# rmontanana/semcode

Hardware: AMD Instinct MI355X
Metric: chunks/sec embed (256-tok) + top-k QPS over 10M x 768 (higher is better)
Workload: dtype bf16; 1 GPU; encoder forward, 256 chunks x 256 tokens per GPU per step, BERT-base shape (12x768, 12 heads, FFN 3072), bf16 MFMA / f32 accumulate, random-init weights; global_batch=256, seq_len=256, parallelism=dp1 (replicated weights, no collective), device=AMD Radeon Graphics (gfx950:sramecc+:xnack-)

## Files before the change

include/semcode_hip.h:

```cpp
#ifndef SEMCODE_HIP_H
#define SEMCODE_HIP_H

#include <stddef.h>
#include <stdint.h>

#ifdef __cplusplus
extern "C" {
#endif

typedef int32_t sc_status;

enum {
    SC_OK = 0,
    SC_ERR_INVALID = -1,
    SC_ERR_HIP = -2,
    SC_ERR_STATE = -3,
    SC_ERR_UNSUPPORTED = -4,
    SC_ERR_NOMEM = -5
};

typedef enum { SC_METRIC_IP = 0, SC_METRIC_L2 = 1, SC_METRIC_COSINE = 2 } sc_metric;
typedef enum { SC_INDEX_FLAT = 0, SC_INDEX_IVF_FLAT = 1 } sc_index_kind;

typedef struct sc_runtime sc_runtime;
typedef struct sc_index sc_index;
typedef struct sc_encoder sc_encoder;


typedef struct sc_runtime_cfg {
    int32_t device;
    void* stream;
    int32_t flags;
} sc_runtime_cfg;

const char* sc_version(void);
sc_status sc_last_error(char* buf, size_t n);

sc_status sc_runtime_create(const sc_runtime_cfg* cfg, sc_runtime** out);
sc_status sc_runtime_destroy(sc_runtime* rt);
sc_status sc_runtime_set_stream(sc_runtime* rt, void* stream);
sc_status sc_runtime_synchronize(sc_runtime* rt);
sc_status sc_runtime_device_info(sc_runtime* rt, char* name, size_t n, int32_t* cus, int64_t* hbm_bytes);
sc_status sc_runtime_set_profiling(sc_runtime* rt, int32_t enabled);
sc_status sc_runtime_profile_read(sc_runtime* rt, int32_t which, double* total_ms, int64_t* launches);
sc_status sc_runtime_profile_reset(sc_runtime* rt);

sc_status sc_synth_fill_dev(sc_runtime* rt, float* out, int64_t rows, int32_t dim, int32_t ld,
                            uint64_t seed, int64_t first_row);


typedef struct sc_encoder_cfg {
    int32_t vocab, hidden, layers, heads, ffn, max_pos, type_vocab;
    float ln_eps;
    int32_t normalize;
    uint64_t synth_seed;
    int32_t pos_type;
    int32_t ffn_type;
    float rope_theta;
    int32_t arch;
    int32_t local_window;
    int32_t global_every;
    float rope_theta_local;
    int32_t kv_heads;
    int32_t head_dim;
    int32_t qk_norm;
    int32_t rel_buckets;
    int32_t rel_max_distance;
} sc_encoder_cfg;

sc_status sc_encoder_blob_bytes(const sc_encoder_cfg* cfg, int64_t* out);
sc_status sc_encoder_create(sc_runtime* rt, const sc_encoder_cfg* cfg, const void* weights_blob, size_t nbytes, sc_encoder** out);
sc_status sc_encoder_destroy(sc_encoder* enc);
sc_status sc_encoder_info(sc_encoder* enc, sc_encoder_cfg* cfg_out);
sc_status sc_encoder_set_path(sc_encoder* enc, int32_t path);
sc_status sc_encoder_set_pooling(sc_encoder* enc, int32_t pooling);
sc_status sc_encoder_get_pooling(sc_encoder* enc, int32_t* out);
sc_status sc_encoder_set_output_proj(sc_encoder* enc, const float* W, const float* b, int32_t E);
sc_status sc_encoder_out_dim(sc_encoder* enc, int32_t* out);
sc_status sc_encoder_embed_ids(sc_encoder* enc, const int32_t* ids, const int32_t* lens, int32_t B, int32_t S, float* out);
sc_status sc_encoder_embed_ids_dev(sc_encoder* enc, const int32_t* ids_dev, const int32_t* lens_dev, int32_t B, int32_t S,
                                   float* out_dev);

sc_status sc_encoder_embed_ids_into(sc_encoder* enc, const int32_t* ids, const int32_t* lens, int32_t B, int32_t S, sc_index* ix,
                                    const int64_t* rows, float* out);

sc_status sc_encoder_embed_ids_into_async(sc_encoder* enc, const int32_t* ids, const int32_t* lens, int32_t B, int32_t S, sc_index* ix,
                                          const int64_t* rows);
sc_status sc_encoder_wait(sc_encoder* enc);

#define SC_ENCODER_PACKED_MAX_ROWS 524288
sc_status sc_encoder_packed_rows(sc_encoder* enc, const int64_t* offsets, int32_t B, int64_t* rows);
sc_status sc_encoder_embed_packed(sc_encoder* enc, const int32_t* ids, const int64_t* offsets, int32_t B, float* out);
sc_status sc_encoder_embed_packed_into(sc_encoder* enc, const int32_t* ids, const int64_t* offsets, int32_t B, sc_index* ix, const int64_t* rows,
                                       float* out);
sc_status sc_encoder_embed_packed_into_async(sc_encoder* enc, const int32_t* ids, const int64_t* offsets, int32_t B, sc_index* ix,
                                             const int64_t* rows);

sc_status sc_encoder_set_pair_head(sc_encoder* enc, const float* pooler_w , const float* pooler_b ,
                                   const float* cls_w , const float* cls_b , int32_t num_labels);
sc_status sc_encoder_score_pairs(sc_encoder* enc, const int32_t* ids, const int64_t* offsets, const int32_t* first_lens, int32_t B,
                                 float* out_logits, float* out_cls);

typedef struct sc_score_head {
    int32_t kind;
    int32_t pooling;
    int32_t num_labels;
    float   norm_eps;
    const float *dense_w , *dense_b , *norm_g , *norm_b ;
    const float *cls_w , *cls_b ;
} sc_score_head;
sc_status sc_encoder_set_score_head(sc_encoder* enc, const sc_score_head* head );
sc_status sc_encoder_score_seqs(sc_encoder* enc, const int32_t* ids, const int64_t* offsets, int32_t B, float* out_logits ,
                                float* out_rows );

sc_status sc_encoder_set_token_head(sc_encoder* enc, const float* w , int32_t W);
sc_status sc_encoder_embed_tokens(sc_encoder* enc, const int32_t* ids, const int64_t* offsets, int32_t B, int32_t expand_id, float* out ,
                                  int32_t* out_counts );
sc_status sc_encoder_score_late(sc_encoder* enc, const int32_t* q_ids, const int64_t* q_offsets, int32_t Bq, int32_t expand_id, const int32_t* d_ids,
                                const int64_t* d_offsets, int32_t Bd, const uint8_t* d_keep , const int32_t* pair_q, const int32_t* pair_d, int32_t P,
                                float* out_scores );
sc_status sc_diag_maxsim(sc_runtime* rt, const float* Q, const int32_t* q_off, int32_t Bq, const float* D, const int32_t* d_off, int32_t Bd, const uint8_t* keep,
                         const int32_t* pair_q, const int32_t* pair_d, int32_t P, int32_t W, float* out);
sc_status sc_diag_maxsim_host(const float* Q, const int32_t* q_off, int32_t Bq, const float* D, const int32_t* d_off, int32_t Bd, const uint8_t* keep,
                              const int32_t* pair_q, const int32_t* pair_d, int32_t P, int32_t W, float* out);

typedef struct sc_tokenizer sc_tokenizer;
sc_status sc_tokenizer_create(const char* vocab_utf8, size_t nbytes, int32_t lowercase, sc_tokenizer** out);
sc_status sc_tokenizer_destroy(sc_tokenizer* tok);
sc_status sc_tokenizer_info(sc_tokenizer* tok, int32_t* vocab_size, int32_t* pad, int32_t* unk, int32_t* cls, int32_t* sep);
sc_status sc_tokenizer_encode(sc_tokenizer* tok, const char* bytes, const int64_t* offsets, int32_t n, int32_t max_tokens, int32_t S,
                              int32_t* ids, int32_t* lens, uint8_t* needs_fallback, int32_t threads);

sc_status sc_diag_gemm_bf16(sc_runtime* rt, int32_t epi, const float* A, const float* W, const float* bias, const float* R,
                            int32_t M, int32_t N, int32_t K, float* out);
sc_status sc_diag_gemm_bench(sc_runtime* rt, int32_t epi, int32_t M, int32_t N, int32_t K, int32_t iters, int32_t variant,
                             double* ms_per_launch);
sc_status sc_diag_gemm_trace(sc_runtime* rt, int32_t epi, int32_t M, int32_t N, int32_t K, uint64_t* out, int64_t cap_words);
sc_status sc_diag_gemm_i8(sc_runtime* rt, const int8_t* A, const int8_t* W, int32_t M, int32_t N, int32_t K, int32_t* out);
sc_status sc_diag_encoder_read(sc_encoder* enc, int32_t which, void* out, size_t nbytes);
sc_status sc_diag_set_option(const char* name, int32_t value);
sc_status sc_diag_rope(sc_runtime* rt, float* qk, int32_t rows, int32_t S, int32_t heads, float theta);
sc_status sc_diag_rel_buckets(int32_t rel_buckets, int32_t max_distance, int32_t span, int32_t* out);
sc_status sc_diag_attention_bias(sc_runtime* rt, const float* qkv, const int32_t* lens, int32_t B, int32_t S, int32_t heads, int32_t blocked_rows,
                                 const float* rel_bias, int32_t buckets, int32_t max_distance, float* out);
sc_status sc_diag_attention_bias_packed(sc_runtime* rt, const float* qkv, const int32_t* starts, const int32_t* lens, int32_t B, int32_t heads,
                                        int32_t blocked_rows, const float* rel_bias, int32_t buckets, int32_t max_distance, float* out);
sc_status sc_diag_ffn_act(sc_runtime* rt, int32_t kind, const float* h, int32_t rows, int32_t F, float* out);
sc_status sc_diag_output_proj(sc_runtime* rt, const float* x, int32_t B, int32_t H, const float* W, const float* bias, int32_t E, int32_t normalize,
                              float* out);
sc_status sc_diag_swiglu(sc_runtime* rt, const float* h, int32_t rows, int32_t F, float* out);
sc_status sc_diag_attention(sc_runtime* rt, const float* qkv, const int32_t* lens, int32_t B, int32_t S, int32_t heads, float* out);

sc_status sc_diag_fold_ln(sc_runtime* rt, const float* W, const float* gamma, const float* beta, const float* bias, int32_t N, int32_t K,
                          float* Wf, float* c1, float* c2);
sc_status sc_diag_gemm_lna(sc_runtime* rt, int32_t epi, int32_t flags, const float* A, const float* Wf, const float* c1, const float* c2,
                           const float* stats_in, float eps, int32_t M, int32_t N, int32_t K, int32_t rope_S, float rope_theta,
                           int32_t rope_ncols, float* C, float* fin);
int32_t sc_diag_gemm_strip(int32_t M, int32_t N, int32_t K, int32_t cus);
sc_status sc_diag_gemm_resln(sc_runtime* rt, int32_t flags, const float* A, const float* W, const float* bias, const float* gam, const float* R,
                             const float* fin, float eps, int32_t M, int32_t N, int32_t K, float* C, float* stats_out);
sc_status sc_diag_attention_ex(sc_runtime* rt, const float* qkv, const int32_t* lens, int32_t B, int32_t S, int32_t heads, int32_t blocked_rows,
                               const float* slopes, float* out);
sc_status sc_diag_attention_packed(sc_runtime* rt, const float* qkv, const int32_t* starts, const int32_t* lens, int32_t B, int32_t heads,
                                   int32_t blocked_rows, const float* slopes, float* out);
sc_status sc_diag_attention_hd(sc_runtime* rt, const float* qkv, const int32_t* lens, int32_t B, int32_t S, int32_t heads, int32_t head_dim,
                               int32_t blocked_rows, const float* slopes, float* out);
sc_status sc_diag_attention_packed_hd(sc_runtime* rt, const float* qkv, const int32_t* starts, const int32_t* lens, int32_t B, int32_t heads,
                                      int32_t head_dim, int32_t blocked_rows, const float* slopes, float* out);
sc_status sc_diag_attention_cls(sc_runtime* rt, const float* qkv, const int32_t* lens, int32_t B, int32_t S, int32_t heads, int32_t head_dim,
                                const float* alibi, float* out);
sc_status sc_diag_attention_window(sc_runtime* rt, const float* qkv, const int32_t* starts, const int32_t* lens, int32_t B, int32_t S, int32_t heads,
                                   int32_t local_window, int32_t blocked_rows, float* out);
sc_status sc_diag_attention_causal(sc_runtime* rt, const float* qkv, const int32_t* starts, const int32_t* lens, int32_t B, int32_t S, int32_t heads,
                                   int32_t kv_heads, int32_t blocked_rows, float* out);
sc_status sc_diag_attention_causal_hd(sc_runtime* rt, const float* qkv, const int32_t* starts, const int32_t* lens, int32_t B, int32_t S, int32_t heads,
                                      int32_t kv_heads, int32_t head_dim, int32_t blocked_rows, float* out);
sc_status sc_diag_qknorm_rope(sc_runtime* rt, float* x, int32_t rows, int32_t S, const int32_t* pos, int32_t heads, int32_t kv_heads, int32_t head_dim,
                              float theta, const float* gamma_q, const float* gamma_k, float eps);
sc_status sc_diag_layernorm(sc_runtime* rt, const float* x, int32_t tokens, int32_t H, const float* gamma, const float* beta, float eps, float* out);
sc_status sc_diag_rmsnorm(sc_runtime* rt, const float* x, int32_t tokens, int32_t H, const float* gamma, float eps, float* out);
sc_status sc_diag_mean_pool(sc_runtime* rt, const float* x, const int32_t* lens, int32_t B, int32_t S, int32_t H, int32_t normalize, float* out);
sc_status sc_diag_mean_pool_ln(sc_runtime* rt, const float* y, const float* stats, int32_t slots, int32_t tokens_pad, const float* gamma,
                               const float* beta, float eps, const int32_t* lens, int32_t B, int32_t S, int32_t H, float* out);
sc_status sc_diag_geglu(sc_runtime* rt, const float* h, int32_t rows, int32_t F, float* out);
sc_status sc_diag_embed(sc_runtime* rt, int32_t ln, const int32_t* ids, int32_t tokens, int32_t S, int32_t H, int32_t vocab, int32_t max_pos,
                        const float* wemb, const float* pemb, const float* temb, const float* gamma, const float* beta, float eps,
                        int32_t tokens_pad, int32_t slots, float* rows, float* stats);
sc_status sc_diag_embed_pairs(sc_runtime* rt, int32_t ln, const int32_t* ids, const int32_t* pos, const int32_t* types, int32_t tokens, int32_t H,
                              int32_t vocab, int32_t max_pos, int32_t type_vocab, const float* wemb, const float* pemb, const float* temb,
                              const float* gamma, const float* beta, float eps, int32_t tokens_pad, int32_t slots, float* rows, float* stats);
sc_status sc_diag_pair_head(sc_runtime* rt, const float* cls, int32_t B, int32_t H, const float* pooler_w, const float* pooler_b,
                            const float* cls_w, const float* cls_b, int32_t num_labels, float* out_logits);
sc_status sc_diag_score_head(sc_runtime* rt, const float* rows, int32_t B, int32_t H, const sc_score_head* head, float* out_logits);


sc_status sc_index_create(sc_runtime* rt, int32_t dim, sc_metric metric, sc_index_kind kind,
                          int32_t nlist, int64_t row_base, sc_index** out);
sc_status sc_index_destroy(sc_index* ix);
sc_status sc_index_info(sc_index* ix, int64_t* rows, int32_t* dim, int32_t* ld);
sc_status sc_index_reserve(sc_index* ix, int64_t rows);
sc_status sc_index_add(sc_index* ix, const float* vecs, int64_t n);
sc_status sc_index_overwrite(sc_index* ix, const float* vecs, const int64_t* rows, int64_t n);
sc_status sc_index_put_rows(sc_index* ix, const float* vecs, const int64_t* rows, int64_t n);
sc_status sc_index_put_rows_dev(sc_index* ix, const float* vecs_dev, const int64_t* rows, int64_t n);
sc_status sc_index_delete_rows(sc_index* ix, const int64_t* rows, int64_t n);
sc_status sc_index_last_delete_stats(sc_index* ix, int64_t* rows_moved, int64_t* bytes_moved, int32_t* shadows_kept, int32_t* shadows_dropped);
sc_status sc_index_get_rows(sc_index* ix, int64_t first, int64_t n, float* out);
sc_status sc_index_fill_synthetic(sc_index* ix, int64_t n, uint64_t seed, int64_t first_row);

sc_status sc_index_fill_synthetic_clustered(sc_index* ix, int64_t n, uint64_t seed, int64_t first_row, int32_t nclusters, float spread);
sc_status sc_index_release_scratch(sc_index* ix);

sc_status sc_index_search(sc_index* ix, const float* q, int32_t Q, int32_t k, int32_t nprobe,
                          float* out_dist, int64_t* out_rows);
sc_status sc_index_search_dev(sc_index* ix, const float* q_dev, int32_t Q, int32_t k, int32_t nprobe,
                              float* out_dist_dev, int64_t* out_rows_dev);

sc_status sc_index_search_masked(sc_index* ix, const float* q, int32_t Q, int32_t k, const uint32_t* allow, int64_t allow_words,
                                 float* out_dist, int64_t* out_rows);
sc_status sc_index_search_masked_dev(sc_index* ix, const float* q_dev, int32_t Q, int32_t k, const uint32_t* allow_dev,
                                     int64_t allow_words, float* out_dist_dev, int64_t* out_rows_dev);
sc_status sc_index_last_mask_stats(sc_index* ix, int64_t* allowed_rows, int64_t* scanned_rows, int32_t* gathered);

sc_status sc_index_set_groups(sc_index* ix, const int32_t* labels, int64_t n);
sc_status sc_index_search_grouped(sc_index* ix, const float* q, int32_t Q, int32_t k, const uint32_t* allow, int64_t allow_words,
                                  float* out_dist, int64_t* out_rows);
sc_status sc_index_search_grouped_dev(sc_index* ix, const float* q_dev, int32_t Q, int32_t k, const uint32_t* allow_dev,
                                      int64_t allow_words, float* out_dist_dev, int64_t* out_rows_dev);
sc_status sc_index_last_group_stats(sc_index* ix, int32_t* first_width, int32_t* queries_continued, int32_t* rounds, int64_t* rows_scanned);

sc_status sc_index_search_mmr(sc_index* ix, const float* q, int32_t Q, int32_t k, int32_t fetch_k, float lambda, const uint32_t* allow,
                              int64_t allow_words, float* out_dist, int64_t* out_rows);
sc_status sc_index_search_mmr_dev(sc_index* ix, const float* q_dev, int32_t Q, int32_t k, int32_t fetch_k, float lambda,
                                  const uint32_t* allow_dev, int64_t allow_words, float* out_dist_dev, int64_t* out_rows_dev);
sc_status sc_index_last_mmr_stats(sc_index* ix, int32_t* fetch_k, int32_t* min_candidates, int64_t* rows_scanned);
sc_status sc_diag_mmr_select_host(const float* rel, const float* G, int32_t C, int32_t ldg, int32_t k, float lambda, int32_t* picked);

sc_status sc_lex_terms(const uint8_t* bytes, const int64_t* offsets, int64_t n, int32_t T, uint16_t* out_terms, int32_t* out_counts);
sc_status sc_index_set_terms(sc_index* ix, int64_t first_row, int64_t n, int32_t T, const uint16_t* terms);
sc_status sc_index_drop_terms(sc_index* ix);
sc_status sc_index_lex_stats(sc_index* ix, int64_t* rows, int64_t* sum_dl, uint32_t* df);
sc_status sc_index_search_lexical(sc_index* ix, int32_t Q, int32_t k, const uint16_t* qterms, const float* qweights, const int32_t* nterms, float k1, float b,
                                  float avgdl, const uint32_t* allow, int64_t allow_words, float* out_score, int64_t* out_rows);
sc_status sc_index_search_lexical_dev(sc_index* ix, int32_t Q, int32_t k, const uint16_t* qterms_dev, const float* qweights_dev, const int32_t* nterms_dev,
                                      float k1, float b, float avgdl, const uint32_t* allow_dev, int64_t allow_words, float* out_score_dev,
                                      int64_t* out_rows_dev);
sc_status sc_index_search_hybrid(sc_index* ix, const float* q, int32_t Q, int32_t k, int32_t fetch_k, const uint16_t* qterms, const float* qweights,
                                 const int32_t* nterms, float k1, float b, float avgdl, int32_t c, float wd, float wl, const uint32_t* allow,
                                 int64_t allow_words, float* out_score, int64_t* out_rows);
sc_status sc_index_search_hybrid_dev(sc_index* ix, const float* q_dev, int32_t Q, int32_t k, int32_t fetch_k, const uint16_t* qterms_dev,
                                     const float* qweights_dev, const int32_t* nterms_dev, float k1, float b, float avgdl, int32_t c, float wd, float wl,
                                     const uint32_t* allow_dev, int64_t allow_words, float* out_score_dev, int64_t* out_rows_dev);
sc_status sc_index_last_lex_stats(sc_index* ix, int64_t* rows_scanned, int64_t* bytes_per_pass, int32_t* passes);
sc_status sc_diag_lex_score_host(const uint16_t* terms, int64_t n, int32_t T, const uint16_t* qterms, const float* qweights, int32_t m, float k1, float b,
                                 float avgdl, float* out_score, uint8_t* out_hit);
sc_status sc_diag_rrf_host(const int64_t* dense_rows, const int64_t* lex_rows, int32_t F, int32_t k, int32_t c, float wd, float wl, float* out_score,
                           int64_t* out_rows);

sc_status sc_index_train(sc_index* ix, int32_t niter, uint64_t seed);
sc_status sc_index_ivf_assignments(sc_index* ix, int32_t* out);
sc_status sc_index_set_ivf(sc_index* ix, const float* centroids, const int32_t* assign, int32_t nlist);
sc_status sc_index_assign_lists(sc_index* ix, const float* centroids, int32_t nlist);
sc_status sc_index_ivf_info(sc_index* ix, int32_t* nlist, float* centroids, int64_t* list_sizes);

sc_status sc_index_set_search_mode(sc_index* ix, int32_t mode);
sc_status sc_index_last_search_stats(sc_index* ix, int32_t* path, int32_t* uncertified);

sc_status sc_index_set_coarse_stage(sc_index* ix, int32_t bits);
sc_status sc_index_last_coarse_stats(sc_index* ix, int32_t* first_stage_bits, int32_t* handed_to_bf16);
sc_status sc_index_last_collect_stats(sc_index* ix, int32_t* tried, int32_t* resolved);
sc_status sc_index_last_wide(sc_index* ix, int32_t* wide);
sc_status sc_index_last_tail_rows(sc_index* ix, int64_t* rows);

sc_status sc_index_last_probe_stats(sc_index* ix, int64_t* unique_rows, int64_t* streamed_rows, int32_t* groups);
sc_status sc_diag_ivf_plan(const char* path, const int64_t* probes, int32_t Q, int32_t nprobe, const int64_t* list_off, int32_t nlist,
                           int32_t k, int32_t ld, int32_t cus, int32_t wide, void* out, int64_t cap_bytes, int64_t* need_bytes);
sc_status sc_diag_ivf_exact_path(int32_t ld, int32_t R, int32_t k, int32_t nprobe, int32_t cus, int32_t* path);
sc_status sc_diag_encoder_plan(const int32_t* ids, const int64_t* offsets, int32_t B, int32_t kind, const int32_t* first_lens, int32_t expand_id,
                               int32_t query, int32_t max_pos, int32_t pos_type, int32_t vocab, int32_t type_vocab, int32_t arch, int32_t global_every,
                               int32_t local_window, void* out, int64_t cap_bytes, int64_t* need_bytes);

sc_status sc_topk_merge_host(sc_metric metric, int32_t lists, int32_t Q, int32_t k,
                             const float* dist, const int64_t* rows, float* out_dist, int64_t* out_rows);


typedef struct sc_comm sc_comm;
#define SC_COMM_ID_BYTES 128
sc_status sc_comm_unique_id(void* id_out, size_t nbytes);
sc_status sc_comm_create(sc_runtime* rt, int32_t rank, int32_t world, const void* unique_id, size_t nbytes, sc_comm** out);
sc_status sc_comm_destroy(sc_comm* comm);
sc_status sc_comm_info(sc_comm* comm, int32_t* rank, int32_t* world);
sc_status sc_comm_rccl_version(int32_t* version);
sc_status sc_comm_allgather_topk(sc_comm* comm, const float* dist_dev, const int64_t* rows_dev, int32_t Q, int32_t k,
                                 float* all_dist_dev, int64_t* all_rows_dev);
sc_status sc_comm_broadcast(sc_comm* comm, void* buf_dev, size_t nbytes, int32_t root);
sc_status sc_index_search_sharded(sc_index* ix, sc_comm* comm, const float* q, int32_t Q, int32_t k, int32_t nprobe,
                                  float* out_dist, int64_t* out_rows);
sc_status sc_index_search_sharded_dev(sc_index* ix, sc_comm* comm, const float* q_dev, int32_t Q, int32_t k, int32_t nprobe,
                                      float* all_dist_dev, int64_t* all_rows_dev);
sc_status sc_index_train_sharded(sc_index* ix, sc_comm* comm, int32_t niter, int32_t root);
sc_status sc_comm_allreduce_max(sc_comm* comm, double* value);

#ifdef __cplusplus
}
#endif
#endif
```

semcode_amd/_native.py:

```python
from __future__ import annotations

import ctypes as C
import sys
import threading
from pathlib import Path

import numpy as np

LIB_PATH = Path(__file__).resolve().parent / "_lib" / "libsemcode_hip.so"

METRICS = {"IP": 0, "L2": 1, "COSINE": 2}
KINDS = {"FLAT": 0, "IVF_FLAT": 1}


class ScError(RuntimeError):

    def __init__(self, status: int, message: str):
        super().__init__(f"libsemcode_hip error {status}: {message}")
        self.status = status


class _Cfg(C.Structure):
    _fields_ = [("device", C.c_int32), ("stream", C.c_void_p), ("flags", C.c_int32)]


class EncoderCfg(C.Structure):
    _fields_ = [("vocab", C.c_int32), ("hidden", C.c_int32), ("layers", C.c_int32), ("heads", C.c_int32), ("ffn", C.c_int32),
                ("max_pos", C.c_int32), ("type_vocab", C.c_int32), ("ln_eps", C.c_float), ("normalize", C.c_int32),
                ("synth_seed", C.c_uint64), ("pos_type", C.c_int32), ("ffn_type", C.c_int32), ("rope_theta", C.c_float),
                ("arch", C.c_int32), ("local_window", C.c_int32), ("global_every", C.c_int32), ("rope_theta_local", C.c_float),
                ("kv_heads", C.c_int32)]

    def __new__(cls, *args, **kw):
        real = EncoderCfgFull if cls is EncoderCfg else cls
        return real.from_buffer(bytearray(real.CFG_BYTES))


class EncoderCfgFull(EncoderCfg):
    _fields_ = [("head_dim", C.c_int32), ("qk_norm", C.c_int32)]
    TAIL_FIELDS = ("rel_buckets", "rel_max_distance")
    CFG_BYTES = 88 + 4 * len(TAIL_FIELDS)

    def _tail(self, name):
        return C.c_int32.from_address(C.addressof(self) + 88 + 4 * self.TAIL_FIELDS.index(name))

    rel_buckets = property(lambda self: self._tail("rel_buckets").value, lambda self, v: setattr(self._tail("rel_buckets"), "value", int(v)))
    rel_max_distance = property(lambda self: self._tail("rel_max_distance").value, lambda self, v: setattr(self._tail("rel_max_distance"), "value", int(v)))


class ScoreHead(C.Structure):
    _fields_ = [("kind", C.c_int32), ("pooling", C.c_int32), ("num_labels", C.c_int32), ("norm_eps", C.c_float),
                ("dense_w", C.c_void_p), ("dense_b", C.c_void_p), ("norm_g", C.c_void_p), ("norm_b", C.c_void_p), ("cls_w", C.c_void_p), ("cls_b", C.c_void_p)]


_lib = None
_lib_lock = threading.Lock()

_f32p = C.POINTER(C.c_float)
_i64p = C.POINTER(C.c_int64)

SIGNATURES = {
    "sc_version": (C.c_char_p, []),
    "sc_last_error": (C.c_int32, [C.c_char_p, C.c_size_t]),
    "sc_runtime_create": (C.c_int32, [C.POINTER(_Cfg), C.POINTER(C.c_void_p)]),
    "sc_runtime_destroy": (C.c_int32, [C.c_void_p]),
    "sc_runtime_set_stream": (C.c_int32, [C.c_void_p, C.c_void_p]),
    "sc_runtime_synchronize": (C.c_int32, [C.c_void_p]),
    "sc_runtime_device_info": (C.c_int32, [C.c_void_p, C.c_char_p, C.c_size_t, C.POINTER(C.c_int32), C.POINTER(C.c_int64)]),
    "sc_runtime_set_profiling": (C.c_int32, [C.c_void_p, C.c_int32]),
    "sc_runtime_profile_read": (C.c_int32, [C.c_void_p, C.c_int32, C.POINTER(C.c_double), C.POINTER(C.c_int64)]),
    "sc_runtime_profile_reset": (C.c_int32, [C.c_void_p]),
    "sc_synth_fill_dev": (C.c_int32, [C.c_void_p, C.c_void_p, C.c_int64, C.c_int32, C.c_int32, C.c_uint64, C.c_int64]),
    "sc_encoder_blob_bytes": (C.c_int32, [C.POINTER(EncoderCfg), C.POINTER(C.c_int64)]),
    "sc_encoder_create": (C.c_int32, [C.c_void_p, C.POINTER(EncoderCfg), C.c_void_p, C.c_size_t, C.POINTER(C.c_void_p)]),
    "sc_encoder_destroy": (C.c_int32, [C.c_void_p]),
    "sc_encoder_set_path": (C.c_int32, [C.c_void_p, C.c_int32]),
    "sc_encoder_set_pooling": (C.c_int32, [C.c_void_p, C.c_int32]),
    "sc_encoder_get_pooling": (C.c_int32, [C.c_void_p, C.POINTER(C.c_int32)]),
    "sc_encoder_info": (C.c_int32, [C.c_void_p, C.POINTER(EncoderCfg)]),
    "sc_encoder_embed_ids": (C.c_int32, [C.c_void_p, C.c_void_p, C.c_void_p, C.c_int32, C.c_int32, C.c_void_p]),
    "sc_encoder_embed_ids_dev": (C.c_int32, [C.c_void_p, C.c_void_p, C.c_void_p, C.c_int32, C.c_int32, C.c_void_p]),
    "sc_encoder_embed_ids_into": (C.c_int32, [C.c_void_p, C.c_void_p, C.c_void_p, C.c_int32, C.c_int32, C.c_void_p, C.c_void_p, C.c_void_p]),
    "sc_encoder_embed_ids_into_async": (C.c_int32, [C.c_void_p, C.c_void_p, C.c_void_p, C.c_int32, C.c_int32, C.c_void_p, C.c_void_p]),
    "sc_encoder_wait": (C.c_int32, [C.c_void_p]),
    "sc_encoder_packed_rows": (C.c_int32, [C.c_void_p, C.c_void_p, C.c_int32, C.POINTER(C.c_int64)]),
    "sc_encoder_embed_packed": (C.c_int32, [C.c_void_p, C.c_void_p, C.c_void_p, C.c_int32, C.c_void_p]),
    "sc_encoder_set_output_proj": (C.c_int32, [C.c_void_p, C.c_void_p, C.c_void_p, C.c_int32]),
    "sc_encoder_out_dim": (C.c_int32, [C.c_void_p, C.POINTER(C.c_int32)]),
    "sc_diag_output_proj": (C.c_int32, [C.c_void_p, C.c_void_p, C.c_int32, C.c_int32, C.c_void_p, C.c_void_p, C.c_int32, C.c_int32, C.c_void_p]),
    "sc_encoder_set_pair_head": (C.c_int32, [C.c_void_p] * 5 + [C.c_int32]),
    "sc_encoder_score_pairs": (C.c_int32, [C.c_void_p] * 4 + [C.c_int32, C.c_void_p, C.c_void_p]),
    "sc_encoder_set_score_head": (C.c_int32, [C.c_void_p, C.POINTER(ScoreHead)]),
    "sc_encoder_score_seqs": (C.c_int32, [C.c_void_p, C.c_void_p, C.c_void_p, C.c_int32, C.c_void_p, C.c_void_p]),
    "sc_encoder_set_token_head": (C.c_int32, [C.c_void_p, C.c_void_p, C.c_int32]),
    "sc_encoder_embed_tokens": (C.c_int32, [C.c_void_p, C.c_void_p, C.c_void_p, C.c_int32, C.c_int32, C.c_void_p, C.c_void_p]),
    "sc_encoder_score_late": (C.c_int32, [C.c_void_p, C.c_void_p, C.c_void_p, C.c_int32, C.c_int32, C.c_void_p, C.c_void_p, C.c_int32] + [C.c_void_p] * 3
                              + [C.c_int32, C.c_void_p]),
    "sc_diag_maxsim": (C.c_int32, [C.c_void_p, C.c_void_p, C.c_void_p, C.c_int32, C.c_void_p, C.c_void_p, C.c_int32] + [C.c_void_p] * 3
                       + [C.c_int32, C.c_int32, C.c_void_p]),
    "sc_diag_maxsim_host": (C.c_int32, [C.c_void_p, C.c_void_p, C.c_int32, C.c_void_p, C.c_void_p, C.c_int32] + [C.c_void_p] * 3 + [C.c_int32, C.c_int32, C.c_void_p]),
    "sc_diag_score_head": (C.c_int32, [C.c_void_p, C.c_void_p, C.c_int32, C.c_int32, C.POINTER(ScoreHead), C.c_void_p]),
    "sc_diag_embed_pairs": (C.c_int32, [C.c_void_p, C.c_int32] + [C.c_void_p] * 3 + [C.c_int32] * 5 + [C.c_void_p] * 5 + [C.c_float, C.c_int32, C.c_int32,
                                                                                                                       C.c_void_p, C.c_void_p]),
    "sc_diag_pair_head": (C.c_int32, [C.c_void_p, C.c_void_p, C.c_int32, C.c_int32] + [C.c_void_p] * 4 + [C.c_int32, C.c_void_p]),
    "sc_encoder_embed_packed_into": (C.c_int32, [C.c_void_p, C.c_void_p, C.c_void_p, C.c_int32, C.c_void_p, C.c_void_p, C.c_void_p]),
    "sc_encoder_embed_packed_into_async": (C.c_int32, [C.c_void_p, C.c_void_p, C.c_void_p, C.c_int32, C.c_void_p, C.c_void_p]),
    "sc_tokenizer_create": (C.c_int32, [C.c_char_p, C.c_size_t, C.c_int32, C.POINTER(C.c_void_p)]),
    "sc_tokenizer_destroy": (C.c_int32, [C.c_void_p]),
    "sc_tokenizer_info": (C.c_int32, [C.c_void_p] + [C.POINTER(C.c_int32)] * 5),
    "sc_tokenizer_encode": (C.c_int32, [C.c_void_p, C.c_char_p, C.c_void_p, C.c_int32, C.c_int32, C.c_int32, C.c_void_p, C.c_void_p, C.c_void_p, C.c_int32]),
    "sc_diag_gemm_bf16": (C.c_int32, [C.c_void_p, C.c_int32, C.c_void_p, C.c_void_p, C.c_void_p, C.c_void_p, C.c_int32, C.c_int32, C.c_int32, C.c_void_p]),
    "sc_diag_gemm_bench": (C.c_int32, [C.c_void_p, C.c_int32, C.c_int32, C.c_int32, C.c_int32, C.c_int32, C.c_int32, C.POINTER(C.c_double)]),
    "sc_diag_gemm_trace": (C.c_int32, [C.c_void_p, C.c_int32, C.c_int32, C.c_int32, C.c_int32, C.c_void_p, C.c_int64]),
    "sc_diag_set_option": (C.c_int32, [C.c_char_p, C.c_int32]),
    "sc_diag_gemm_i8": (C.c_int32, [C.c_void_p, C.c_void_p, C.c_void_p, C.c_int32, C.c_int32, C.c_int32, C.c_void_p]),
    "sc_diag_encoder_read": (C.c_int32, [C.c_void_p, C.c_int32, C.c_void_p, C.c_size_t]),
    "sc_diag_attention": (C.c_int32, [C.c_void_p, C.c_void_p, C.c_void_p, C.c_int32, C.c_int32, C.c_int32, C.c_void_p]),
    "sc_diag_rope": (C.c_int32, [C.c_void_p, C.c_void_p, C.c_int32, C.c_int32, C.c_int32, C.c_float]),
    "sc_diag_swiglu": (C.c_int32, [C.c_void_p, C.c_void_p, C.c_int32, C.c_int32, C.c_void_p]),
    "sc_diag_rel_buckets": (C.c_int32, [C.c_int32, C.c_int32, C.c_int32, C.c_void_p]),
    "sc_diag_attention_bias": (C.c_int32, [C.c_void_p, C.c_void_p, C.c_void_p, C.c_int32, C.c_int32, C.c_int32, C.c_int32, C.c_void_p, C.c_int32, C.c_int32, C.c_void_p]),
    "sc_diag_attention_bias_packed": (C.c_int32, [C.c_void_p, C.c_void_p, C.c_void_p, C.c_void_p, C.c_int32, C.c_int32, C.c_int32, C.c_void_p, C.c_int32, C.c_int32,
                                                  C.c_void_p]),
    "sc_diag_ffn_act": (C.c_int32, [C.c_void_p, C.c_int32, C.c_void_p, C.c_int32, C.c_int32, C.c_void_p]),
    "sc_diag_fold_ln": (C.c_int32, [C.c_void_p] * 5 + [C.c_int32, C.c_int32] + [C.c_void_p] * 3),
    "sc_diag_gemm_strip": (C.c_int32, [C.c_int32] * 4),
    "sc_diag_gemm_lna": (C.c_int32, [C.c_void_p, C.c_int32, C.c_int32] + [C.c_void_p] * 5 + [C.c_float, C.c_int32, C.c_int32, C.c_int32, C.c_int32,
                                     C.c_float, C.c_int32, C.c_void_p, C.c_void_p]),
    "sc_diag_gemm_resln": (C.c_int32, [C.c_void_p, C.c_int32] + [C.c_void_p] * 6 + [C.c_float, C.c_int32, C.c_int32, C.c_int32, C.c_void_p, C.c_void_p]),
    "sc_diag_attention_ex": (C.c_int32, [C.c_void_p, C.c_void_p, C.c_void_p, C.c_int32, C.c_int32, C.c_int32, C.c_int32, C.c_void_p, C.c_void_p]),
    "sc_diag_attention_packed": (C.c_int32, [C.c_void_p, C.c_void_p, C.c_void_p, C.c_void_p, C.c_int32, C.c_int32, C.c_int32, C.c_void_p, C.c_void_p]),
    "sc_diag_attention_hd": (C.c_int32, [C.c_void_p, C.c_void_p, C.c_void_p, C.c_int32, C.c_int32, C.c_int32, C.c_int32, C.c_int32, C.c_void_p, C.c_void_p]),
    "sc_diag_attention_cls": (C.c_int32, [C.c_void_p, C.c_void_p, C.c_void_p, C.c_int32, C.c_int32, C.c_int32, C.c_int32, C.c_void_p, C.c_void_p]),
    "sc_diag_attention_window": (C.c_int32, [C.c_void_p, C.c_void_p, C.c_void_p, C.c_void_p, C.c_int32, C.c_int32, C.c_int32, C.c_int32, C.c_int32, C.c_void_p]),
    "sc_diag_attention_packed_hd": (C.c_int32, [C.c_void_p, C.c_void_p, C.c_void_p, C.c_void_p, C.c_int32, C.c_int32, C.c_int32, C.c_int32, C.c_void_p, C.c_void_p]),
    "sc_diag_layernorm": (C.c_int32, [C.c_void_p, C.c_void_p, C.c_int32, C.c_int32, C.c_void_p, C.c_void_p, C.c_float, C.c_void_p]),
    "sc_diag_attention_causal": (C.c_int32, [C.c_void_p, C.c_void_p, C.c_void_p, C.c_void_p, C.c_int32, C.c_int32, C.c_int32, C.c_int32, C.c_int32, C.c_void_p]),
    "sc_diag_attention_causal_hd": (C.c_int32, [C.c_void_p, C.c_void_p, C.c_void_p, C.c_void_p, C.c_int32, C.c_int32, C.c_int32, C.c_int32, C.c_int32, C.c_int32,
                                                 C.c_void_p]),
    "sc_diag_qknorm_rope": (C.c_int32, [C.c_void_p, C.c_void_p, C.c_int32, C.c_int32, C.c_void_p, C.c_int32, C.c_int32, C.c_int32, C.c_float, C.c_void_p, C.c_void_p,
                                         C.c_float]),
    "sc_diag_rmsnorm": (C.c_int32, [C.c_void_p, C.c_void_p, C.c_int32, C.c_int32, C.c_void_p, C.c_float, C.c_void_p]),
    "sc_diag_mean_pool": (C.c_int32, [C.c_void_p, C.c_void_p, C.c_void_p, C.c_int32, C.c_int32, C.c_int32, C.c_int32, C.c_void_p]),
    "sc_diag_mean_pool_ln": (C.c_int32, [C.c_void_p, C.c_void_p, C.c_void_p, C.c_int32, C.c_int32, C.c_void_p, C.c_void_p, C.c_float, C.c_void_p,
                                         C.c_int32, C.c_int32, C.c_int32, C.c_void_p]),
    "sc_diag_geglu": (C.c_int32, [C.c_void_p, C.c_void_p, C.c_int32, C.c_int32, C.c_void_p]),
    "sc_diag_embed": (C.c_int32, [C.c_void_p, C.c_int32, C.c_void_p, C.c_int32, C.c_int32, C.c_int32, C.c_int32, C.c_int32] + [C.c_void_p] * 5 +
                                 [C.c_float, C.c_int32, C.c_int32, C.c_void_p, C.c_void_p]),
    "sc_index_create": (C.c_int32, [C.c_void_p, C.c_int32, C.c_int32, C.c_int32, C.c_int32, C.c_int64, C.POINTER(C.c_void_p)]),
    "sc_index_destroy": (C.c_int32, [C.c_void_p]),
    "sc_index_info": (C.c_int32, [C.c_void_p, C.POINTER(C.c_int64), C.POINTER(C.c_int32), C.POINTER(C.c_int32)]),
    "sc_index_reserve": (C.c_int32, [C.c_void_p, C.c_int64]),
    "sc_index_add": (C.c_int32, [C.c_void_p, C.c_void_p, C.c_int64]),
    "sc_index_overwrite": (C.c_int32, [C.c_void_p, C.c_void_p, C.c_void_p, C.c_int64]),
    "sc_index_put_rows": (C.c_int32, [C.c_void_p, C.c_void_p, C.c_void_p, C.c_int64]),
    "sc_index_put_rows_dev": (C.c_int32, [C.c_void_p, C.c_void_p, C.c_void_p, C.c_int64]),
    "sc_index_delete_rows": (C.c_int32, [C.c_void_p, C.c_void_p, C.c_int64]),
    "sc_index_last_delete_stats": (C.c_int32, [C.c_void_p, C.POINTER(C.c_int64), C.POINTER(C.c_int64), C.POINTER(C.c_int32), C.POINTER(C.c_int32)]),
    "sc_index_get_rows": (C.c_int32, [C.c_void_p, C.c_int64, C.c_int64, C.c_void_p]),
    "sc_index_fill_synthetic": (C.c_int32, [C.c_void_p, C.c_int64, C.c_uint64, C.c_int64]),
    "sc_index_fill_synthetic_clustered": (C.c_int32, [C.c_void_p, C.c_int64, C.c_uint64, C.c_int64, C.c_int32, C.c_float]),
    "sc_index_release_scratch": (C.c_int32, [C.c_void_p]),
    "sc_index_search": (C.c_int32, [C.c_void_p, C.c_void_p, C.c_int32, C.c_int32, C.c_int32, C.c_void_p, C.c_void_p]),
    "sc_index_search_dev": (C.c_int32, [C.c_void_p, C.c_void_p, C.c_int32, C.c_int32, C.c_int32, C.c_void_p, C.c_void_p]),
    "sc_index_search_masked": (C.c_int32, [C.c_void_p, C.c_void_p, C.c_int32, C.c_int32, C.c_void_p, C.c_int64, C.c_void_p, C.c_void_p]),
    "sc_index_search_masked_dev": (C.c_int32, [C.c_void_p, C.c_void_p, C.c_int32, C.c_int32, C.c_void_p, C.c_int64, C.c_void_p, C.c_void_p]),
    "sc_index_last_mask_stats": (C.c_int32, [C.c_void_p, C.POINTER(C.c_int64), C.POINTER(C.c_int64), C.POINTER(C.c_int32)]),
    "sc_index_set_groups": (C.c_int32, [C.c_void_p, C.c_void_p, C.c_int64]),
    "sc_index_search_grouped": (C.c_int32, [C.c_void_p, C.c_void_p, C.c_int32, C.c_int32, C.c_void_p, C.c_int64, C.c_void_p, C.c_void_p]),
    "sc_index_search_grouped_dev": (C.c_int32, [C.c_void_p, C.c_void_p, C.c_int32, C.c_int32, C.c_void_p, C.c_int64, C.c_void_p, C.c_void_p]),
    "sc_index_last_group_stats": (C.c_int32, [C.c_void_p, C.POINTER(C.c_int32), C.POINTER(C.c_int32), C.POINTER(C.c_int32), C.POINTER(C.c_int64)]),
    "sc_index_search_mmr": (C.c_int32, [C.c_void_p, C.c_void_p, C.c_int32, C.c_int32, C.c_int32, C.c_float, C.c_void_p, C.c_int64, C.c_void_p, C.c_void_p]),
    "sc_index_search_mmr_dev": (C.c_int32, [C.c_void_p, C.c_void_p, C.c_int32, C.c_int32, C.c_int32, C.c_float, C.c_void_p, C.c_int64, C.c_void_p, C.c_void_p]),
    "sc_index_last_mmr_stats": (C.c_int32, [C.c_void_p, C.POINTER(C.c_int32), C.POINTER(C.c_int32), C.POINTER(C.c_int64)]),
    "sc_diag_mmr_select_host": (C.c_int32, [C.c_void_p, C.c_void_p, C.c_int32, C.c_int32, C.c_int32, C.c_float, C.c_void_p]),
    "sc_lex_terms": (C.c_int32, [C.c_void_p, C.c_void_p, C.c_int64, C.c_int32, C.c_void_p, C.c_void_p]),
    "sc_index_set_terms": (C.c_int32, [C.c_void_p, C.c_int64, C.c_int64, C.c_int32, C.c_void_p]),
    "sc_index_drop_terms": (C.c_int32, [C.c_void_p]),
    "sc_index_lex_stats": (C.c_int32, [C.c_void_p, C.POINTER(C.c_int64), C.POINTER(C.c_int64), C.c_void_p]),
    "sc_index_search_lexical": (C.c_int32, [C.c_void_p, C.c_int32, C.c_int32, C.c_void_p, C.c_void_p, C.c_void_p, C.c_float, C.c_float, C.c_float, C.c_void_p, C.c_int64,
                                            C.c_void_p, C.c_void_p]),
    "sc_index_search_lexical_dev": (C.c_int32, [C.c_void_p, C.c_int32, C.c_int32, C.c_void_p, C.c_void_p, C.c_void_p, C.c_float, C.c_float, C.c_float, C.c_void_p, C.c_int64,
                                                C.c_void_p, C.c_void_p]),
    "sc_index_search_hybrid": (C.c_int32, [C.c_void_p, C.c_void_p, C.c_int32, C.c_int32, C.c_int32, C.c_void_p, C.c_void_p, C.c_void_p, C.c_float, C.c_float, C.c_float,
                                           C.c_int32, C.c_float, C.c_float, C.c_void_p, C.c_int64, C.c_void_p, C.c_void_p]),
    "sc_index_search_hybrid_dev": (C.c_int32, [C.c_void_p, C.c_void_p, C.c_int32, C.c_int32, C.c_int32, C.c_void_p, C.c_void_p, C.c_void_p, C.c_float, C.c_float, C.c_float,
                                               C.c_int32, C.c_float, C.c_float, C.c_void_p, C.c_int64, C.c_void_p, C.c_void_p]),
    "sc_index_last_lex_stats": (C.c_int32, [C.c_void_p, C.POINTER(C.c_int64), C.POINTER(C.c_int64), C.POINTER(C.c_int32)]),
    "sc_diag_lex_score_host": (C.c_int32, [C.c_void_p, C.c_int64, C.c_int32, C.c_void_p, C.c_void_p, C.c_int32, C.c_float, C.c_float, C.c_float, C.c_void_p, C.c_void_p]),
    "sc_diag_rrf_host": (C.c_int32, [C.c_void_p, C.c_void_p, C.c_int32, C.c_int32, C.c_int32, C.c_float, C.c_float, C.c_void_p, C.c_void_p]),
    "sc_index_train": (C.c_int32, [C.c_void_p, C.c_int32, C.c_uint64]),
    "sc_index_ivf_assignments": (C.c_int32, [C.c_void_p, C.c_void_p]),
    "sc_index_set_ivf": (C.c_int32, [C.c_void_p, C.c_void_p, C.c_void_p, C.c_int32]),
    "sc_index_assign_lists": (C.c_int32, [C.c_void_p, C.c_void_p, C.c_int32]),
    "sc_index_ivf_info": (C.c_int32, [C.c_void_p, C.POINTER(C.c_int32), C.c_void_p, C.c_void_p]),
    "sc_index_set_search_mode": (C.c_int32, [C.c_void_p, C.c_int32]),
    "sc_index_last_search_stats": (C.c_int32, [C.c_void_p, C.POINTER(C.c_int32), C.POINTER(C.c_int32)]),
    "sc_index_set_coarse_stage": (C.c_int32, [C.c_void_p, C.c_int32]),
    "sc_index_last_coarse_stats": (C.c_int32, [C.c_void_p, C.POINTER(C.c_int32), C.POINTER(C.c_int32)]),
    "sc_index_last_collect_stats": (C.c_int32, [C.c_void_p, C.POINTER(C.c_int32), C.POINTER(C.c_int32)]),
    "sc_index_last_wide": (C.c_int32, [C.c_void_p, C.POINTER(C.c_int32)]),
    "sc_index_last_tail_rows": (C.c_int32, [C.c_void_p, C.POINTER(C.c_int64)]),
    "sc_index_last_probe_stats": (C.c_int32, [C.c_void_p, C.POINTER(C.c_int64), C.POINTER(C.c_int64), C.POINTER(C.c_int32)]),
    "sc_diag_ivf_plan": (C.c_int32, [C.c_char_p, C.c_void_p, C.c_int32, C.c_int32, C.c_void_p, C.c_int32, C.c_int32, C.c_int32, C.c_int32, C.c_int32, C.c_void_p,
                                     C.c_int64, C.POINTER(C.c_int64)]),
    "sc_diag_ivf_exact_path": (C.c_int32, [C.c_int32, C.c_int32, C.c_int32, C.c_int32, C.c_int32, C.POINTER(C.c_int32)]),
    "sc_diag_encoder_plan": (C.c_int32, [C.c_void_p, C.c_void_p, C.c_int32, C.c_int32, C.c_void_p, C.c_int32] + [C.c_int32] * 8 + [C.c_void_p, C.c_int64,
                                         C.POINTER(C.c_int64)]),
    "sc_comm_unique_id": (C.c_int32, [C.c_void_p, C.c_size_t]),
    "sc_comm_create": (C.c_int32, [C.c_void_p, C.c_int32, C.c_int32, C.c_void_p, C.c_size_t, C.POINTER(C.c_void_p)]),
    "sc_comm_destroy": (C.c_int32, [C.c_void_p]),
    "sc_comm_info": (C.c_int32, [C.c_void_p, C.POINTER(C.c_int32), C.POINTER(C.c_int32)]),
    "sc_comm_rccl_version": (C.c_int32, [C.POINTER(C.c_int32)]),
    "sc_comm_allgather_topk": (C.c_int32, [C.c_void_p, C.c_void_p, C.c_void_p, C.c_int32, C.c_int32, C.c_void_p, C.c_void_p]),
    "sc_comm_broadcast": (C.c_int32, [C.c_void_p, C.c_void_p, C.c_size_t, C.c_int32]),
    "sc_index_search_sharded": (C.c_int32, [C.c_void_p, C.c_void_p, C.c_void_p, C.c_int32, C.c_int32, C.c_int32, C.c_void_p, C.c_void_p]),
    "sc_index_search_sharded_dev": (C.c_int32, [C.c_void_p, C.c_void_p, C.c_void_p, C.c_int32, C.c_int32, C.c_int32, C.c_void_p, C.c_void_p]),
    "sc_index_train_sharded": (C.c_int32, [C.c_void_p, C.c_void_p, C.c_int32, C.c_int32]),
    "sc_comm_allreduce_max": (C.c_int32, [C.c_void_p, C.POINTER(C.c_double)]),
    "sc_topk_merge_host": (C.c_int32, [C.c_int32, C.c_int32, C.c_int32, C.c_int32, C.c_void_p, C.c_void_p, C.c_void_p, C.c_void_p]),
}


def lib() -> C.CDLL:
    global _lib
    with _lib_lock:
        if _lib is None:
            if not LIB_PATH.exists():
                raise RuntimeError(
                    f"{LIB_PATH} is missing: build it with `python -m semcode_amd.csrc.build` "
                    "(needs hipcc); semcode_amd has no CPU fallback."
                )
            try:
                import torch
            except Exception:
                pass
            handle = C.CDLL(str(LIB_PATH))
            for name, (res, args) in SIGNATURES.items():
                fn = getattr(handle, name)
                fn.restype = res
                fn.argtypes = args
            _lib = handle
    return _lib


def _check(status: int) -> None:
    if status != 0:
        buf = C.create_string_buffer(512)
        lib().sc_last_error(buf, 512)
        raise ScError(status, buf.value.decode("utf-8", "replace"))


def pack_allow(allow, rows: int) -> np.ndarray:
    a = np.asarray(allow)
    if a.dtype == np.bool_:
        if a.shape != (rows,):
            raise ValueError(f"a boolean mask must have one entry per row ({rows}), got shape {a.shape}")
        bits = np.packbits(a, bitorder="little")
        words = np.zeros((rows + 31) // 32 * 4, dtype=np.uint8)
        words[: bits.size] = bits
        return words.view("<u4")
    if a.dtype != np.uint32 or a.ndim != 1:
        raise ValueError("allow must be a 1-d uint32 word array or a boolean array with one entry per row")
    return np.ascontiguousarray(a)


def _result_arrays(Q: int, k: int) -> "tuple[np.ndarray, np.ndarray]":
    return np.empty((Q, k), dtype=np.float32), np.empty((Q, k), dtype=np.int64)


LEX_MAX_QTERMS = 32
LEX_DF_SIZE = 65536
LEX_PAD = 0xFFFF


def lex_terms(texts, T: int = 128) -> "tuple[np.ndarray, np.ndarray]":
    raw = [t.encode("utf-8") if isinstance(t, str) else bytes(t) for t in texts]
    n = len(raw)
    offsets = np.zeros(n + 1, dtype=np.int64)
# ... 824 lines not shown
def diag_gemm_bench(rt: Runtime, M: int, N: int, K: int, epi: int = 0, iters: int = 20, variant: int = 0) -> float:
    ms = C.c_double()
    _check(lib().sc_diag_gemm_bench(rt.handle, epi, M, N, K, iters, variant, C.byref(ms)))
    return ms.value


def diag_gemm_trace(rt: Runtime, M: int, N: int, K: int, epi: int = 0, launches: int = 1) -> np.ndarray:
    nt = (M // 256) * (N // 256)
    out = np.zeros((launches, nt, 8), np.uint64)
    _check(lib().sc_diag_gemm_trace(rt.handle, epi, M, N, K, out.ctypes.data_as(C.c_void_p), out.size))
    return out


def diag_gemm_i8(rt: Runtime, A, W) -> np.ndarray:
    A = np.ascontiguousarray(A, np.int8)
    W = np.ascontiguousarray(W, np.int8)
    M, K = A.shape
    N = W.shape[0]
    out = np.empty((M, N), np.int32)
    _check(lib().sc_diag_gemm_i8(rt.handle, A.ctypes.data_as(C.c_void_p), W.ctypes.data_as(C.c_void_p), M, N, K, out.ctypes.data_as(C.c_void_p)))
    return out


def diag_attention(rt: Runtime, qkv, lens, B: int, S: int, heads: int, head_dim: int = 64, blocked_rows: int = 0) -> np.ndarray:
    if head_dim != 64 or blocked_rows:
        return diag_attention_ex(rt, qkv, lens, B, S, heads, blocked_rows=blocked_rows, head_dim=head_dim)
    qkv = np.ascontiguousarray(qkv, np.float32)
    lens = np.ascontiguousarray(lens, np.int32)
    out = np.empty((B * S, heads * 64), np.float32)
    _check(lib().sc_diag_attention(rt.handle, qkv.ctypes.data_as(C.c_void_p), lens.ctypes.data_as(C.c_void_p), B, S, heads,
                                   out.ctypes.data_as(C.c_void_p)))
    return out


def diag_rope(rt: Runtime, qk, S: int, heads: int, theta: float) -> np.ndarray:
    out = np.array(qk, dtype=np.float32, order="C")
    rows = out.shape[0]
    if out.shape != (rows, heads * 64):
        raise ValueError("qk must be [rows, heads * 64]")
    _check(lib().sc_diag_rope(rt.handle, out.ctypes.data_as(C.c_void_p), rows, int(S), int(heads), float(theta)))
    return out


def diag_rel_buckets(rel_buckets: int, max_distance: int, span: int) -> np.ndarray:
    out = np.empty(max(2 * int(span) - 1, 1), np.int32)
    _check(lib().sc_diag_rel_buckets(int(rel_buckets), int(max_distance), int(span), out.ctypes.data_as(C.c_void_p)))
    return out


def diag_ffn_act(rt: Runtime, kind: int, h) -> np.ndarray:
    h = np.ascontiguousarray(h, np.float32)
    rows, F = h.shape[0], h.shape[1] // (2 if kind == 4 else 1)
    out = np.empty((rows, F), np.float32)
    _check(lib().sc_diag_ffn_act(rt.handle, int(kind), h.ctypes.data_as(C.c_void_p), rows, F, out.ctypes.data_as(C.c_void_p)))
    return out


def diag_attention_bias(rt: Runtime, qkv, lens, B: int, S: int, heads: int, rel_bias, max_distance: int, blocked_rows: int = 0) -> np.ndarray:
    qkv = np.ascontiguousarray(qkv, np.float32)
    lens = np.ascontiguousarray(lens, np.int32)
    rb = np.ascontiguousarray(rel_bias, np.float32)
    H = heads * 64
    if blocked_rows:
        pad = np.zeros((blocked_rows, 3 * H), np.float32)
        pad[: B * S] = qkv
        qkv = block64(pad)
    out = np.empty((B * S, H), np.float32)
    _check(lib().sc_diag_attention_bias(rt.handle, qkv.ctypes.data_as(C.c_void_p), lens.ctypes.data_as(C.c_void_p), B, S, heads, int(blocked_rows),
                                        rb.ctypes.data_as(C.c_void_p), rb.shape[0], int(max_distance), out.ctypes.data_as(C.c_void_p)))
    return out


def diag_attention_bias_packed(rt: Runtime, qkv, starts, lens, heads: int, rel_bias, max_distance: int, blocked_rows: int = 0) -> np.ndarray:
    qkv = np.ascontiguousarray(qkv, np.float32)
    starts = np.ascontiguousarray(starts, np.int32)
    lens = np.ascontiguousarray(lens, np.int32)
    rb = np.ascontiguousarray(rel_bias, np.float32)
    H = heads * 64
    R = int(blocked_rows) if blocked_rows else (int((starts + (lens + 31) // 32 * 32).max()) + 255) // 256 * 256
    if qkv.shape != (R, 3 * H) or starts.shape != lens.shape:
        raise ValueError(f"diag_attention_bias_packed: qkv must be [{R}, {3 * H}], starts and lens [B]")
    if blocked_rows:
        qkv = block64(qkv)
    out = np.empty((R, H), np.float32)
    _check(lib().sc_diag_attention_bias_packed(rt.handle, qkv.ctypes.data_as(C.c_void_p), starts.ctypes.data_as(C.c_void_p), lens.ctypes.data_as(C.c_void_p),
                                               len(lens), heads, int(blocked_rows), rb.ctypes.data_as(C.c_void_p), rb.shape[0], int(max_distance),
                                               out.ctypes.data_as(C.c_void_p)))
    return out


def diag_output_proj(rt: Runtime, x, W, b=None, normalize: bool = True) -> np.ndarray:
    x, W = np.ascontiguousarray(x, np.float32), np.ascontiguousarray(W, np.float32)
    b = None if b is None else np.ascontiguousarray(b, np.float32)
    out = np.empty((x.shape[0], W.shape[0]), np.float32)
    _check(lib().sc_diag_output_proj(rt.handle, x.ctypes.data_as(C.c_void_p), x.shape[0], x.shape[1], W.ctypes.data_as(C.c_void_p),
                                     None if b is None else b.ctypes.data_as(C.c_void_p), W.shape[0], 1 if normalize else 0, out.ctypes.data_as(C.c_void_p)))
    return out


def diag_swiglu(rt: Runtime, h) -> np.ndarray:
    h = np.ascontiguousarray(h, np.float32)
    rows, F = h.shape[0], h.shape[1] // 2
    out = np.empty((rows, F), np.float32)
    _check(lib().sc_diag_swiglu(rt.handle, h.ctypes.data_as(C.c_void_p), rows, F, out.ctypes.data_as(C.c_void_p)))
    return out


EPI_LNA_BIAS, EPI_LNA_GELU, EPI_RESLN_STATS, EPI_LNA_BIAS_ROPE = 3, 4, 5, 6


def _f32(a):
    return np.ascontiguousarray(a, np.float32)


def _ptr(a):
    return None if a is None else a.ctypes.data_as(C.c_void_p)


def block64(a: np.ndarray) -> np.ndarray:
    M, N = a.shape
    return np.ascontiguousarray(a.reshape(M, N // 64, 64).transpose(1, 0, 2))


def unblock64(a: np.ndarray, M: int, N: int) -> np.ndarray:
    return np.ascontiguousarray(np.asarray(a).reshape(N // 64, M, 64).transpose(1, 0, 2).reshape(M, N))


def diag_fold_ln(rt: Runtime, W, gamma, beta, bias=None):
    W, gamma, beta = _f32(W), _f32(gamma), _f32(beta)
    bias = None if bias is None else _f32(bias)
    N, K = W.shape
    Wf, c1, c2 = np.empty((N, K), np.float32), np.empty(N, np.float32), np.empty(N, np.float32)
    _check(lib().sc_diag_fold_ln(rt.handle, _ptr(W), _ptr(gamma), _ptr(beta), _ptr(bias), N, K, _ptr(Wf), _ptr(c1), _ptr(c2)))
    return Wf, c1, c2


def diag_gemm_lna(rt: Runtime, epi: int, A, Wf, c1, c2, stats_in, eps: float, blocked: bool = False, rope_S: int = 0, rope_theta: float = 0.0,
                  rope_ncols: int = 0):
    A, Wf, c1, c2, stats_in = _f32(A), _f32(Wf), _f32(c1), _f32(c2), _f32(stats_in)
    M, K = A.shape
    N = Wf.shape[0]
    if stats_in.shape != (K // 256, M, 2) or Wf.shape != (N, K) or c1.shape != (N,) or c2.shape != (N,):
        raise ValueError("diag_gemm_lna: shapes")
    Cc, fin = np.empty((M, N), np.float32), np.empty((M, 2), np.float32)
    _check(lib().sc_diag_gemm_lna(rt.handle, epi, 1 if blocked else 0, _ptr(A), _ptr(Wf), _ptr(c1), _ptr(c2), _ptr(stats_in), float(eps), M, N, K,
                                  int(rope_S), float(rope_theta), int(rope_ncols), _ptr(Cc), _ptr(fin)))
    return (unblock64(Cc, M, N) if blocked else Cc), fin


def diag_gemm_strip(M: int = 0, N: int = 0, K: int = 0, cus: int = 0) -> int:
    return int(lib().sc_diag_gemm_strip(int(M), int(N), int(K), int(cus)))


def diag_gemm_resln(rt: Runtime, A, W, bias, gam, R, fin, eps: float, a_blocked: bool = False):
    A, W, bias, gam, R, fin = _f32(A), _f32(W), _f32(bias), _f32(gam), _f32(R), _f32(fin)
    M, K = A.shape
    N = W.shape[0]
    if W.shape != (N, K) or R.shape != (M, N) or fin.shape != (M, 2) or bias.shape != (N,) or gam.shape != (N,):
        raise ValueError("diag_gemm_resln: shapes")
    Ad = block64(A) if a_blocked else A
    Cc, st = np.empty((M, N), np.float32), np.empty((N // 256, M, 2), np.float32)
    _check(lib().sc_diag_gemm_resln(rt.handle, 1 if a_blocked else 0, _ptr(Ad), _ptr(W), _ptr(bias), _ptr(gam), _ptr(R), _ptr(fin), float(eps), M, N, K,
                                    _ptr(Cc), _ptr(st)))
    return Cc, st


def diag_attention_ex(rt: Runtime, qkv, lens, B: int, S: int, heads: int, blocked_rows: int = 0, slopes=None, head_dim: int = 64) -> np.ndarray:
    qkv = _f32(qkv)
    lens = np.ascontiguousarray(lens, np.int32)
    H = heads * head_dim
    if blocked_rows:
        pad = np.zeros((blocked_rows, 3 * H), np.float32)
        pad[: B * S] = qkv
        qkv = block64(pad)
    sl = None if slopes is None else _f32(slopes)
    out = np.empty((B * S, H), np.float32)
    if head_dim != 64:
        _check(lib().sc_diag_attention_hd(rt.handle, _ptr(qkv), _ptr(lens), B, S, heads, int(head_dim), int(blocked_rows), _ptr(sl), _ptr(out)))
    else:
        _check(lib().sc_diag_attention_ex(rt.handle, _ptr(qkv), _ptr(lens), B, S, heads, int(blocked_rows), _ptr(sl), _ptr(out)))
    return out


def diag_attention_cls(rt: Runtime, qkv, lens, B: int, S: int, heads: int, head_dim: int = 64, slopes=None) -> np.ndarray:
    qkv = _f32(qkv)
    lens = np.ascontiguousarray(lens, np.int32)
    H = heads * head_dim
    if qkv.shape != (B * S, 3 * H) or lens.shape != (B,):
        raise ValueError("qkv must be [B*S, 3*heads*head_dim] and lens [B]")
    sl = None if slopes is None else _f32(slopes)
    out = np.full((B, H), np.nan, np.float32)
    _check(lib().sc_diag_attention_cls(rt.handle, _ptr(qkv), _ptr(lens), B, S, heads, int(head_dim), _ptr(sl), _ptr(out)))
    return out


def diag_attention_packed(rt: Runtime, qkv, starts, lens, heads: int, blocked_rows: int = 0, slopes=None, head_dim: int = 64) -> np.ndarray:
    qkv = _f32(qkv)
    starts = np.ascontiguousarray(starts, np.int32)
    lens = np.ascontiguousarray(lens, np.int32)
    H = heads * head_dim
    R = int(blocked_rows) if blocked_rows else (int((starts + (lens + 31) // 32 * 32).max()) + 255) // 256 * 256
    if qkv.shape != (R, 3 * H) or starts.shape != lens.shape:
        raise ValueError(f"diag_attention_packed: qkv must be [{R}, {3 * H}], starts and lens [B]")
    if blocked_rows:
        qkv = block64(qkv)
    sl = None if slopes is None else _f32(slopes)
    out = np.empty((R, H), np.float32)
    if head_dim != 64:
        _check(lib().sc_diag_attention_packed_hd(rt.handle, _ptr(qkv), _ptr(starts), _ptr(lens), len(lens), heads, int(head_dim), int(blocked_rows), _ptr(sl),
                                                 _ptr(out)))
    else:
        _check(lib().sc_diag_attention_packed(rt.handle, _ptr(qkv), _ptr(starts), _ptr(lens), len(lens), heads, int(blocked_rows), _ptr(sl), _ptr(out)))
    return out


def diag_attention_window(rt: Runtime, qkv, lens, heads: int, local_window: int, S: int = 0, starts=None, blocked_rows: int = 0) -> np.ndarray:
    qkv = _f32(qkv)
    lens = np.ascontiguousarray(lens, np.int32)
    H = heads * 64
    if starts is None:
        rows = len(lens) * int(S)
        R = int(blocked_rows) if blocked_rows else rows
    else:
        starts = np.ascontiguousarray(starts, np.int32)
        R = rows = int(blocked_rows) if blocked_rows else (int((starts + (lens + 31) // 32 * 32).max()) + 255) // 256 * 256
    if qkv.shape != (R, 3 * H) or (starts is not None and starts.shape != lens.shape):
        raise ValueError(f"diag_attention_window: qkv must be [{R}, {3 * H}], starts (if given) and lens [B]")
    if blocked_rows:
        qkv = block64(qkv)
    out = np.empty((rows, H), np.float32)
    _check(lib().sc_diag_attention_window(rt.handle, _ptr(qkv), None if starts is None else _ptr(starts), _ptr(lens), len(lens), int(S), heads,
                                          int(local_window), int(blocked_rows), _ptr(out)))
    return out


def diag_attention_causal(rt: Runtime, qkv, lens, heads: int, kv_heads: int, S: int = 0, starts=None, blocked_rows: int = 0, head_dim: int = 64) -> np.ndarray:
    qkv = _f32(qkv)
    lens = np.ascontiguousarray(lens, np.int32)
    head_dim = int(head_dim)
    H, QN = heads * head_dim, (heads + 2 * kv_heads) * head_dim
    if starts is None:
        rows = len(lens) * int(S)
        R = int(blocked_rows) if blocked_rows else rows
    else:
        starts = np.ascontiguousarray(starts, np.int32)
        R = rows = int(blocked_rows) if blocked_rows else (int((starts + (lens + 31) // 32 * 32).max()) + 255) // 256 * 256
    if qkv.shape != (R, QN) or (starts is not None and starts.shape != lens.shape):
        raise ValueError(f"diag_attention_causal: qkv must be [{R}, {QN}], starts (if given) and lens [B]")
    if blocked_rows:
        qkv = block64(qkv)
    out = np.empty((rows, H), np.float32)
    if head_dim != 64:
        _check(lib().sc_diag_attention_causal_hd(rt.handle, _ptr(qkv), None if starts is None else _ptr(starts), _ptr(lens), len(lens), int(S), heads,
                                                 int(kv_heads), head_dim, int(blocked_rows), _ptr(out)))
        return out
    _check(lib().sc_diag_attention_causal(rt.handle, _ptr(qkv), None if starts is None else _ptr(starts), _ptr(lens), len(lens), int(S), heads,
                                          int(kv_heads), int(blocked_rows), _ptr(out)))
    return out


def diag_qknorm_rope(rt: Runtime, x, heads: int, kv_heads: int, head_dim: int, S: int, theta: float, pos=None, gamma_q=None, gamma_k=None,
                     eps: float = 1e-6) -> np.ndarray:
    out = np.array(x, dtype=np.float32, order="C")
    rows = out.shape[0]
    if out.shape != (rows, (heads + 2 * kv_heads) * head_dim):
        raise ValueError("x must be [rows, (heads + 2 kv_heads) * head_dim]")
    if pos is not None:
        pos = np.ascontiguousarray(pos, np.int32)
        if pos.shape != (rows,):
            raise ValueError("pos must be [rows]")
    gq = None if gamma_q is None else _f32(gamma_q)
    gk = None if gamma_k is None else _f32(gamma_k)
    _check(lib().sc_diag_qknorm_rope(rt.handle, _ptr(out), rows, int(S), None if pos is None else _ptr(pos), int(heads), int(kv_heads), int(head_dim),
                                     float(theta), None if gq is None else _ptr(gq), None if gk is None else _ptr(gk), float(eps)))
    return out


def diag_rmsnorm(rt: Runtime, x, gamma, eps: float) -> np.ndarray:
    x, gamma = _f32(x), _f32(gamma)
    out = np.empty_like(x)
    _check(lib().sc_diag_rmsnorm(rt.handle, _ptr(x), x.shape[0], x.shape[1], _ptr(gamma), float(eps), _ptr(out)))
    return out


def diag_layernorm(rt: Runtime, x, gamma, beta, eps: float) -> np.ndarray:
    x, gamma, beta = _f32(x), _f32(gamma), _f32(beta)
    out = np.empty_like(x)
    _check(lib().sc_diag_layernorm(rt.handle, _ptr(x), x.shape[0], x.shape[1], _ptr(gamma), _ptr(beta), float(eps), _ptr(out)))
    return out


def diag_mean_pool(rt: Runtime, x, lens, S: int, normalize: bool) -> np.ndarray:
    x = _f32(x)
    lens = np.ascontiguousarray(lens, np.int32)
    B, H = lens.size, x.shape[1]
    out = np.empty((B, H), np.float32)
    _check(lib().sc_diag_mean_pool(rt.handle, _ptr(x), _ptr(lens), B, int(S), H, 1 if normalize else 0, _ptr(out)))
    return out


def diag_mean_pool_ln(rt: Runtime, y, stats, gamma, beta, eps: float, lens, S: int) -> np.ndarray:
    y, stats, gamma, beta = _f32(y), _f32(stats), _f32(gamma), _f32(beta)
    lens = np.ascontiguousarray(lens, np.int32)
    B, (tp, H) = lens.size, y.shape
    if stats.shape[1:] != (tp, 2):
        raise ValueError("diag_mean_pool_ln: stats must be [slots, tokens_pad, 2]")
# ... 104 lines not shown
```

semcode_amd/csrc/sc_api.cpp:

```cpp
#include <algorithm>
#include <cmath>
#include <cstdarg>
#include <cstdio>
#include <cstring>
#include <mutex>
#include <new>
#include <string>
#include <vector>

#include "encoder_ops.h"
#include "sc_internal.h"

static thread_local std::string g_err;

sc_status sc_fail(sc_status code, const char* fmt, ...) {
    char buf[512];
    va_list ap;
    va_start(ap, fmt);
    vsnprintf(buf, sizeof buf, fmt, ap);
    va_end(ap);
    g_err = buf;
    return code;
}

extern "C" const char* sc_version(void) { return "semcode_hip 0.1 (gfx950)"; }

extern "C" sc_status sc_last_error(char* buf, size_t n) {
    if (!buf || n == 0) return SC_ERR_INVALID;
    snprintf(buf, n, "%s", g_err.c_str());
    return SC_OK;
}


extern "C" sc_status sc_runtime_create(const sc_runtime_cfg* cfg, sc_runtime** out) {
    if (!out) return sc_fail(SC_ERR_INVALID, "sc_runtime_create: out is NULL");
    *out = nullptr;
    int ndev = 0;
    hipError_t e = hipGetDeviceCount(&ndev);
    if (e != hipSuccess || ndev <= 0)
        return sc_fail(SC_ERR_HIP, "sc_runtime_create: no HIP device available (%s)", e == hipSuccess ? "count = 0" : hipGetErrorString(e));
    const int dev = cfg ? cfg->device : 0;
    if (dev < 0 || dev >= ndev) return sc_fail(SC_ERR_INVALID, "sc_runtime_create: device %d out of range [0,%d)", dev, ndev);
    SC_HIP(hipSetDevice(dev));
    sc_runtime* rt = new (std::nothrow) sc_runtime();
    if (!rt) return sc_fail(SC_ERR_NOMEM, "sc_runtime_create: out of host memory");
    rt->device = dev;
    if (cfg && cfg->stream) {
        rt->stream = (hipStream_t)cfg->stream;
        rt->own_stream = false;
    } else {
        e = hipStreamCreateWithFlags(&rt->stream, hipStreamNonBlocking);
        if (e != hipSuccess) {
            delete rt;
            return sc_fail(SC_ERR_HIP, "hipStreamCreate: %s", hipGetErrorString(e));
        }
        rt->own_stream = true;
    }
    hipDeviceProp_t prop;
    if (hipGetDeviceProperties(&prop, dev) == hipSuccess) {
        snprintf(rt->name, sizeof rt->name, "%s (%s)", prop.name, prop.gcnArchName);
        rt->cus = prop.multiProcessorCount;
        rt->hbm = (int64_t)prop.totalGlobalMem;
    }
    *out = rt;
    return SC_OK;
}

static void prof_clear(sc_runtime* rt) {
    for (int c = 0; c < SC_PROF_CLASSES; ++c) {
        for (auto& p : rt->prof[c]) {
            hipEventDestroy(p.first);
            hipEventDestroy(p.second);
        }
        rt->prof[c].clear();
    }
}

void sc_runtime_retain(sc_runtime* rt) { rt->refs.fetch_add(1, std::memory_order_relaxed); }

void sc_runtime_release(sc_runtime* rt) {
    if (rt->refs.fetch_sub(1, std::memory_order_acq_rel) != 1) return;
    hipSetDevice(rt->device);
    hipStreamSynchronize(rt->stream);
    prof_clear(rt);
    if (rt->own_stream) hipStreamDestroy(rt->stream);
    delete rt;
}

extern "C" sc_status sc_runtime_destroy(sc_runtime* rt) {
    if (!rt) return SC_OK;
    sc_runtime_release(rt);
    return SC_OK;
}

extern "C" sc_status sc_runtime_set_stream(sc_runtime* rt, void* stream) {
    if (!rt) return sc_fail(SC_ERR_INVALID, "runtime is NULL");
    std::lock_guard<std::mutex> g(rt->mu);
    if (rt->own_stream) {
        hipStreamSynchronize(rt->stream);
        hipStreamDestroy(rt->stream);
        rt->own_stream = false;
    }
    rt->stream = (hipStream_t)stream;
    return SC_OK;
}

extern "C" sc_status sc_runtime_synchronize(sc_runtime* rt) {
    if (!rt) return sc_fail(SC_ERR_INVALID, "runtime is NULL");
    SC_HIP(hipSetDevice(rt->device));
    SC_HIP(hipStreamSynchronize(rt->stream));
    return SC_OK;
}

extern "C" sc_status sc_runtime_device_info(sc_runtime* rt, char* name, size_t n, int32_t* cus, int64_t* hbm_bytes) {
    if (!rt) return sc_fail(SC_ERR_INVALID, "runtime is NULL");
    if (name && n) snprintf(name, n, "%s", rt->name);
    if (cus) *cus = rt->cus;
    if (hbm_bytes) *hbm_bytes = rt->hbm;
    return SC_OK;
}

extern "C" sc_status sc_runtime_set_profiling(sc_runtime* rt, int32_t enabled) {
    if (!rt) return sc_fail(SC_ERR_INVALID, "runtime is NULL");
    rt->profiling = enabled < 0 ? 0 : enabled;
    return SC_OK;
}

void sc_prof_begin(sc_runtime* rt, int which, hipEvent_t* a, hipEvent_t* b) {
    *a = *b = nullptr;
    if (!rt->profiling || rt->prof[which].size() >= 8192) return;
    if (which >= SC_PROF_GEMM && rt->profiling > 1 && (rt->prof_seen[which]++ % (unsigned)rt->profiling) != 0) return;
    if (hipEventCreate(a) != hipSuccess) { *a = nullptr; return; }
    if (hipEventCreate(b) != hipSuccess) { hipEventDestroy(*a); *a = *b = nullptr; return; }
    hipEventRecord(*a, rt->stream);
}
void sc_prof_end(sc_runtime* rt, int which, hipEvent_t a, hipEvent_t b) {
    if (!a) return;
    hipEventRecord(b, rt->stream);
    std::lock_guard<std::mutex> g(rt->mu);
    rt->prof[which].push_back({a, b});
}

extern "C" sc_status sc_runtime_profile_read(sc_runtime* rt, int32_t which, double* total_ms, int64_t* launches) {
    if (!rt || which < 0 || which >= SC_PROF_CLASSES) return sc_fail(SC_ERR_INVALID, "bad profile class");
    SC_HIP(hipSetDevice(rt->device));
    SC_HIP(hipStreamSynchronize(rt->stream));
    double t = 0;
    std::lock_guard<std::mutex> g(rt->mu);
    for (auto& p : rt->prof[which]) {
        float ms = 0;
        if (hipEventElapsedTime(&ms, p.first, p.second) == hipSuccess) t += ms;
    }
    if (total_ms) *total_ms = t;
    if (launches) *launches = (int64_t)rt->prof[which].size();
    return SC_OK;
}

extern "C" sc_status sc_runtime_profile_reset(sc_runtime* rt) {
    if (!rt) return sc_fail(SC_ERR_INVALID, "runtime is NULL");
    SC_HIP(hipSetDevice(rt->device));
    SC_HIP(hipStreamSynchronize(rt->stream));
    std::lock_guard<std::mutex> g(rt->mu);
    prof_clear(rt);
    for (unsigned& c : rt->prof_seen) c = 0;
    return SC_OK;
}

extern "C" sc_status sc_synth_fill_dev(sc_runtime* rt, float* out, int64_t rows, int32_t dim, int32_t ld, uint64_t seed,
                                       int64_t first_row) {
    if (!rt || !out) return sc_fail(SC_ERR_INVALID, "sc_synth_fill_dev: NULL argument");
    if (rows < 0 || dim <= 0 || ld < dim || (ld & 3)) return sc_fail(SC_ERR_INVALID, "sc_synth_fill_dev: need rows>=0, 0<dim<=ld, ld%%4==0");
    SC_HIP(hipSetDevice(rt->device));
    sc_launch_synth_fill(out, rows, dim, ld, seed, first_row, nullptr, rt->stream);
    SC_HIP(hipGetLastError());
    return SC_OK;
}

extern "C" sc_status sc_diag_set_option(const char* name, int32_t value) {
    if (!name) return sc_fail(SC_ERR_INVALID, "sc_diag_set_option: NULL name");
    static const struct { const char* name; void (*set)(int); } options[] = {
        {"coarse_workgroups", sc_scan_set_coarse_workgroups}, {"coarse_persistent", sc_scan_set_coarse_persistent},
        {"gemm_pp", sc_gemm_set_pp},                          {"gemm_nt", sc_gemm_set_nt},
        {"ivf_refresh_nomem", sc_ivf_set_refresh_nomem},      {"ivf_refine_cap", sc_ivf_set_refine_cap},
        {"ivf_coarse_nomem", sc_ivf_set_coarse_nomem},        {"collect_pass", sc_set_collect_pass},
        {"tighten", sc_set_tighten},                          {"wide_candidates", sc_set_wide_force},
        {"ivf_tail_rows", sc_set_ivf_tail_rows},              {"delete_chunk_rows", sc_set_delete_chunk_rows},
        {"rope_fused", sc_encoder_set_rope_fused},            {"mask_gather", sc_set_mask_gather},
        {"group_width0", sc_set_group_width0},                {"group_width1", sc_set_group_width1},
        {"mmr_chunk_q", sc_set_mmr_chunk_q},                  {"lex_chunk_q", sc_set_lex_chunk_q},
        {"gemm_strip", sc_gemm_set_strip},                    {"gemm_strip_n", sc_gemm_set_strip_n},
        {"cls_prune", sc_encoder_set_cls_prune},
    };
    for (const auto& o : options)
        if (!strcmp(name, o.name)) {
            o.set(value);
            return SC_OK;
        }
    return sc_fail(SC_ERR_INVALID, "sc_diag_set_option: unknown option '%s'", name);
}


static inline int round_up(int v, int a) { return (v + a - 1) / a * a; }

extern "C" sc_status sc_index_create(sc_runtime* rt, int32_t dim, sc_metric metric, sc_index_kind kind, int32_t nlist,
                                     int64_t row_base, sc_index** out) {
    if (!rt || !out) return sc_fail(SC_ERR_INVALID, "sc_index_create: NULL argument");
    *out = nullptr;
    if (dim <= 0 || dim > 65536) return sc_fail(SC_ERR_INVALID, "sc_index_create: dim %d out of range", dim);
    if (metric != SC_METRIC_IP && metric != SC_METRIC_L2 && metric != SC_METRIC_COSINE)
        return sc_fail(SC_ERR_INVALID, "sc_index_create: unknown metric %d", (int)metric);
    if (kind != SC_INDEX_FLAT && kind != SC_INDEX_IVF_FLAT) return sc_fail(SC_ERR_INVALID, "sc_index_create: unknown kind %d", (int)kind);
    if (kind == SC_INDEX_IVF_FLAT && nlist < 1) return sc_fail(SC_ERR_INVALID, "sc_index_create: IVF_FLAT needs nlist >= 1");
    sc_index* ix = new (std::nothrow) sc_index();
    if (!ix) return sc_fail(SC_ERR_NOMEM, "out of host memory");
    ix->rt = rt;
    sc_runtime_retain(rt);
    ix->dim = dim;
    ix->ld = round_up(dim, SC_LD_ALIGN);
    ix->metric = metric;
    ix->kind = kind;
    ix->nlist = nlist;
    ix->row_base = row_base;
    const size_t ld8 = (size_t)sc_ld8(ix);
    ix->sh_b16.row_bytes[0] = (size_t)ix->ld * 2;
    ix->sh_b16.stat_bit = 1;
    ix->sh_i8.row_bytes[0] = ix->sh_c8.row_bytes[0] = ld8;
    ix->sh_i8.row_bytes[1] = 4;
    ix->sh_i8.stat_bit = 2;
    ix->sh_c8.row_bytes[1] = 16;
    ix->sh_c8.tail_pad = 256;
    ix->sh_c8.stat_bit = 4;
    *out = ix;
    return SC_OK;
}

extern "C" sc_status sc_index_destroy(sc_index* ix) {
    if (!ix) return SC_OK;
    hipSetDevice(ix->rt->device);
    hipStreamSynchronize(ix->rt->stream);
    hipFree(ix->X);
    hipFree(ix->xnorm);
    hipFree(ix->perm);
    hipFree(ix->list_off);
    for (const sc_index_buf& b : SC_INDEX_BUFS) sc_buf_free(ix->*b.buf);
    for (sc_shadow* sh : ix->shadows) sc_shadow_release(*sh);
    if (ix->quant) sc_index_destroy(ix->quant);
    sc_runtime* rt = ix->rt;
    delete ix;
    sc_runtime_release(rt);
    return SC_OK;
}

extern "C" sc_status sc_index_info(sc_index* ix, int64_t* rows, int32_t* dim, int32_t* ld) {
    if (!ix) return sc_fail(SC_ERR_INVALID, "index is NULL");
    std::lock_guard<std::mutex> g(ix->mu);
    if (rows) *rows = ix->n;
    if (dim) *dim = ix->dim;
    if (ld) *ld = ix->ld;
    return SC_OK;
}

static sc_status ensure_rows(sc_index* ix, int64_t rows, bool exact) {
    if (rows <= ix->capacity) return SC_OK;
    int64_t cap = rows;
    if (!exact) cap = std::max<int64_t>(rows, std::max<int64_t>(ix->capacity * 2, 4096));
    float *nx = nullptr, *nn = nullptr;
    hipError_t e = hipMalloc((void**)&nx, (size_t)cap * ix->ld * sizeof(float));
    if (e != hipSuccess) return sc_fail(SC_ERR_NOMEM, "hipMalloc corpus (%lld rows x %d) failed: %s", (long long)cap, ix->ld, hipGetErrorString(e));
    e = hipMalloc((void**)&nn, (size_t)cap * sizeof(float));
    if (e != hipSuccess) {
        hipFree(nx);
        return sc_fail(SC_ERR_NOMEM, "hipMalloc norms failed: %s", hipGetErrorString(e));
    }
    hipStream_t s = ix->rt->stream;
    if (ix->n > 0) {
        SC_HIP(hipMemcpyAsync(nx, ix->X, (size_t)ix->n * ix->ld * sizeof(float), hipMemcpyDeviceToDevice, s));
        SC_HIP(hipMemcpyAsync(nn, ix->xnorm, (size_t)ix->n * sizeof(float), hipMemcpyDeviceToDevice, s));
    }
    SC_HIP(hipStreamSynchronize(s));
    hipFree(ix->X);
    hipFree(ix->xnorm);
    ix->X = nx;
    ix->xnorm = nn;
    ix->capacity = cap;
    return SC_OK;
}

extern "C" sc_status sc_index_reserve(sc_index* ix, int64_t rows) {
    if (!ix || rows < 0) return sc_fail(SC_ERR_INVALID, "sc_index_reserve: bad argument");
    std::lock_guard<std::mutex> g(ix->mu);
    SC_HIP(hipSetDevice(ix->rt->device));
    return ensure_rows(ix, rows, true);
}

static const int64_t STAGE_ROWS_BYTES = 64ll << 20;

extern "C" sc_status sc_index_add(sc_index* ix, const float* vecs, int64_t n) {
    if (!ix || n < 0 || (n > 0 && !vecs)) return sc_fail(SC_ERR_INVALID, "sc_index_add: bad argument");
    if (n == 0) return SC_OK;
    std::lock_guard<std::mutex> g(ix->mu);
    SC_HIP(hipSetDevice(ix->rt->device));
    if (ix->n + n > 0xFFFFFFF0ll) return sc_fail(SC_ERR_UNSUPPORTED, "sc_index_add: more than 2^32 rows per shard");
    sc_status st = ensure_rows(ix, ix->n + n, false);
    if (st) return st;
    const int64_t chunk = std::max<int64_t>(1, STAGE_ROWS_BYTES / ((int64_t)ix->dim * 4));
    hipStream_t s = ix->rt->stream;
    for (int64_t off = 0; off < n; off += chunk) {
        const int64_t m = std::min(chunk, n - off);
        st = sc_grow(ix, ix->stage, (size_t)m * ix->dim * 4);
        if (st) return st;
        SC_HIP(hipMemcpyAsync(ix->stage.p, vecs + off * ix->dim, (size_t)m * ix->dim * 4, hipMemcpyHostToDevice, s));
        sc_launch_ingest_rows(ix->stage.as<float>(), nullptr, ix->n + off, m, ix->dim, ix->X, ix->ld, ix->xnorm, s);
        SC_HIP(hipGetLastError());
        SC_HIP(hipStreamSynchronize(s));
    }
    ix->n += n;
    if (!ix->perm) ix->trained = false;
    return SC_OK;
}

extern "C" sc_status sc_index_overwrite(sc_index* ix, const float* vecs, const int64_t* rows, int64_t n) {
    if (!ix || n < 0 || (n > 0 && (!vecs || !rows))) return sc_fail(SC_ERR_INVALID, "sc_index_overwrite: bad argument");
    if (n == 0) return SC_OK;
    std::lock_guard<std::mutex> g(ix->mu);
    SC_HIP(hipSetDevice(ix->rt->device));
    for (int64_t i = 0; i < n; ++i)
        if (rows[i] < 0 || rows[i] >= ix->n) return sc_fail(SC_ERR_INVALID, "sc_index_overwrite: row %lld out of range [0,%lld)", (long long)rows[i], (long long)ix->n);
    return sc_index_put_rows_locked(ix, vecs, false, rows, n, "sc_index_overwrite");
}

sc_status sc_index_put_rows_locked(sc_index* ix, const float* vecs, bool vecs_on_device, const int64_t* rows, int64_t n, const char* who) {
    int64_t next = ix->n, min_old = INT64_MAX;
    const int64_t old_n = ix->n;
    for (int64_t i = 0; i < n; ++i) {
        const int64_t r = rows[i];
        if (r == next) ++next;
        else if (r >= 0 && r < ix->n) min_old = std::min(min_old, r);
        else return sc_fail(SC_ERR_INVALID, "%s: rows[%lld] = %lld is neither an existing row [0,%lld) nor the next free row %lld", who, (long long)i,
                            (long long)r, (long long)ix->n, (long long)next);
    }
    if (next > 0xFFFFFFF0ll) return sc_fail(SC_ERR_UNSUPPORTED, "%s: more than 2^32 rows per shard", who);
    {
        std::vector<int64_t> sorted(rows, rows + n);
        std::sort(sorted.begin(), sorted.end());
// ... 257 lines not shown
```

semcode_amd/csrc/sc_encoder_diag.cpp:

```cpp
#include <cstring>
#include <vector>

#include "encoder_ops.h"
#include "maxsim_rule.h"
#include "rel_bucket_rule.h"
#include "sc_diag_blob.h"
#include "sc_encoder_plan.h"
#include "sc_internal.h"

namespace {
#define SC_TRY(expr)              \
    do {                          \
        sc_status st_ = (expr);   \
        if (st_) return st_;      \
    } while (0)

sc_status dev_alloc(sc_devbuf& out, size_t bytes) {
    if (out.alloc(bytes) != hipSuccess) return sc_fail(SC_ERR_NOMEM, "diag: hipMalloc failed");
    return SC_OK;
}
sc_status upload(const void* host, size_t bytes, sc_devbuf& out, hipStream_t s) {
    SC_TRY(dev_alloc(out, bytes));
    if (host && bytes) SC_HIP(hipMemcpyAsync(out.p, host, bytes, hipMemcpyHostToDevice, s));
    return SC_OK;
// ... 73 lines not shown
    sc_launch_gemm_i8_diag(da.p, dw.p, dc.p, M, N, K, s);
    return download(dc.p, (size_t)M * N * 4, out, s);
}

namespace {
struct SynthGemm {
    int epi, M, N, K;
    sc_devbuf fa, da, fw, dw, db, dr, dc;
    sc_status init(hipStream_t s) {
        const int64_t na = (int64_t)M * K, nw = (int64_t)N * K, nc = (int64_t)M * N;
        SC_TRY(dev_alloc(fa, na * 4));
        SC_TRY(dev_alloc(da, na * 2));
        SC_TRY(dev_alloc(fw, nw * 4));
        SC_TRY(dev_alloc(dw, nw * 2));
        SC_TRY(dev_alloc(db, (size_t)N * 4));
        SC_TRY(dev_alloc(dr, nc * 2));
        SC_TRY(dev_alloc(dc, nc * 2));
        sc_launch_synth_scaled((float*)fa.p, na, 1, 1.0f, 0.0f, s);
        sc_launch_synth_scaled((float*)fw.p, nw, 2, 0.05f, 0.0f, s);
        sc_launch_f32_to_bf16((const float*)fa.p, da.p, na, s);
        sc_launch_f32_to_bf16((const float*)fw.p, dw.p, nw, s);
        SC_HIP(hipMemsetAsync(db.p, 0, (size_t)N * 4, s));
        SC_HIP(hipMemsetAsync(dr.p, 0, (size_t)nc * 2, s));
        return SC_OK;
    }
    void launch(hipStream_t s) const { sc_launch_gemm_bf16(epi, da.p, K, dw.p, K, (const float*)db.p, dr.p, N, dc.p, N, M, N, K, s); }
};
}

extern "C" sc_status sc_diag_gemm_trace(sc_runtime* rt, int32_t epi, int32_t M, int32_t N, int32_t K, uint64_t* out, int64_t cap_words) {
    if (!rt || !out) return sc_fail(SC_ERR_INVALID, "sc_diag_gemm_trace: bad argument");
    if (M <= 0 || N <= 0 || K <= 0 || (M % 256) || (N % 256) || (K % 64)) return sc_fail(SC_ERR_UNSUPPORTED, "sc_diag_gemm_trace: need M%%256==0, N%%256==0, K%%64==0");
    const int64_t ntiles = (int64_t)(M / 256) * (N / 256);
    const int64_t launches = cap_words / (ntiles * 8);
    if (launches < 1) return sc_fail(SC_ERR_INVALID, "sc_diag_gemm_trace: out too small (need 8 words per tile)");
    SC_HIP(hipSetDevice(rt->device));
    hipStream_t s = rt->stream;
    SynthGemm g{epi, M, N, K};
    sc_devbuf tr;
    const size_t trace_bytes = (size_t)launches * ntiles * 64;
    SC_TRY(dev_alloc(tr, trace_bytes));
    SC_TRY(g.init(s));
    SC_HIP(hipMemsetAsync(tr.p, 0, trace_bytes, s));
    static const int dbg = (int)sc_env_i64("SC_GEMM_TRACE_DBG", 0);
    sc_gemm_set_debug(dbg);
    for (int i = 0; i < 2; ++i) g.launch(s);
    for (int64_t l = 0; l < launches; ++l) {
        sc_gemm_set_trace((unsigned long long*)tr.p + l * ntiles * 8);
        g.launch(s);
    }
    sc_gemm_set_trace(nullptr);
    sc_gemm_set_debug(0);
    hipError_t he = hipStreamSynchronize(s);
    if (he != hipSuccess) return sc_fail(SC_ERR_HIP, "diag gemm trace failed: %s", hipGetErrorString(he));
    SC_HIP(hipMemcpy(out, tr.p, trace_bytes, hipMemcpyDeviceToHost));
    return SC_OK;
}

extern "C" sc_status sc_diag_gemm_bench(sc_runtime* rt, int32_t epi, int32_t M, int32_t N, int32_t K, int32_t iters, int32_t variant,
                                        double* ms_per_launch) {
    if (!rt || !ms_per_launch || iters < 1) return sc_fail(SC_ERR_INVALID, "sc_diag_gemm_bench: bad argument");
    if (!sc_gemm_bf16_supported(M, N, K)) return sc_fail(SC_ERR_UNSUPPORTED, "sc_diag_gemm_bench: need M%%128==0, N%%128==0, K%%64==0");
    SC_HIP(hipSetDevice(rt->device));
    hipStream_t s = rt->stream;
    SynthGemm g{epi, M, N, K};
    SC_TRY(g.init(s));
    const int pp = variant / 100000;
    variant %= 100000;
    sc_gemm_set_pp(pp == 0 ? -1 : pp == 1 ? 0 : pp);
    sc_gemm_force_tile128(variant == 128);
    sc_gemm_set_debug((variant == 128 || variant >= 1000) ? 0 : variant);
    sc_gemm_set_order(variant >= 1000 ? variant - 1000 : 16);
    hipEvent_t e0, e1;
    SC_HIP(hipEventCreate(&e0));
    SC_HIP(hipEventCreate(&e1));
    for (int i = 0; i < 2; ++i) g.launch(s);
    hipEventRecord(e0, s);
    for (int i = 0; i < iters; ++i) g.launch(s);
    hipEventRecord(e1, s);
    hipError_t he = hipStreamSynchronize(s);
    sc_gemm_force_tile128(false);
    sc_gemm_set_debug(0);
    sc_gemm_set_order(16);
    sc_gemm_set_pp(-1);
    float ms = 0;
    hipEventElapsedTime(&ms, e0, e1);
    hipEventDestroy(e0);
    hipEventDestroy(e1);
    if (he != hipSuccess) return sc_fail(SC_ERR_HIP, "diag gemm bench failed: %s", hipGetErrorString(he));
    *ms_per_launch = ms / iters;
    return SC_OK;
}


extern "C" sc_status sc_diag_fold_ln(sc_runtime* rt, const float* W, const float* gamma, const float* beta, const float* bias, int32_t N, int32_t K,
                                     float* Wf, float* c1, float* c2) {
    if (!rt || !W || !gamma || !beta || !Wf || !c1 || !c2) return sc_fail(SC_ERR_INVALID, "sc_diag_fold_ln: NULL argument");
    if (N < 1 || K < 4 || (K % 4)) return sc_fail(SC_ERR_UNSUPPORTED, "sc_diag_fold_ln: need N >= 1 and K a multiple of 4");
    SC_HIP(hipSetDevice(rt->device));
    hipStream_t s = rt->stream;
    sc_devbuf dw, dg, db, dbias, dwf, dc1, dc2;
    SC_TRY(upload(W, (size_t)N * K * 4, dw, s));
    SC_TRY(upload(gamma, (size_t)K * 4, dg, s));
    SC_TRY(upload(beta, (size_t)K * 4, db, s));
    if (bias) SC_TRY(upload(bias, (size_t)N * 4, dbias, s));
    SC_TRY(alloc_nan(dwf, (size_t)N * K * 2, s));
    SC_TRY(alloc_nan(dc1, (size_t)N * 4, s));
    SC_TRY(alloc_nan(dc2, (size_t)N * 4, s));
    sc_launch_fold_ln_weights((const float*)dw.p, (const float*)dg.p, (const float*)db.p, bias ? (const float*)dbias.p : nullptr, N, K, dwf.p, (float*)dc1.p,
                              (float*)dc2.p, s);
    SC_TRY(download(dc1.p, (size_t)N * 4, c1, s));
    SC_TRY(download(dc2.p, (size_t)N * 4, c2, s));
    return download_bf16(dwf.p, (int64_t)N * K, Wf, s);
}

extern "C" sc_status sc_diag_gemm_lna(sc_runtime* rt, int32_t epi, int32_t flags, const float* A, const float* Wf, const float* c1, const float* c2,
                                      const float* stats_in, float eps, int32_t M, int32_t N, int32_t K, int32_t rope_S, float rope_theta,
                                      int32_t rope_ncols, float* C, float* fin) {
    if (!rt || !A || !Wf || !c1 || !c2 || !stats_in || !C || !fin) return sc_fail(SC_ERR_INVALID, "sc_diag_gemm_lna: NULL argument");
    if (epi != EPI_LNA_BIAS && epi != EPI_LNA_GELU && epi != EPI_LNA_BIAS_ROPE) return sc_fail(SC_ERR_INVALID, "sc_diag_gemm_lna: epilogue must be 3, 4 or 6");
    if ((flags & ~1) || !(eps > 0.f)) return sc_fail(SC_ERR_INVALID, "sc_diag_gemm_lna: bad flags / eps");
    if (!sc_gemm_ln_supported(M, N, K) || K > 4096) return sc_fail(SC_ERR_UNSUPPORTED, "sc_diag_gemm_lna: need M%%256==0, N%%256==0, K%%256==0, K<=4096");
    const bool rope = epi == EPI_LNA_BIAS_ROPE;
    if (rope && (rope_S < 1 || rope_S > 65536 || (rope_S & (rope_S - 1)) || rope_ncols < 0 || rope_ncols > N || (rope_ncols % 64)))
        return sc_fail(SC_ERR_INVALID, "sc_diag_gemm_lna: rope_S must be a power of two, rope_ncols a multiple of 64 within N");
    SC_HIP(hipSetDevice(rt->device));
    hipStream_t s = rt->stream;
    sc_devbuf fa, da, fw, dw, dc1, dc2, dst, dfin, dc, dt;
    SC_TRY(upload_bf16(A, (int64_t)M * K, fa, da, s));
    SC_TRY(upload_bf16(Wf, (int64_t)N * K, fw, dw, s));
    SC_TRY(upload(c1, (size_t)N * 4, dc1, s));
    SC_TRY(upload(c2, (size_t)N * 4, dc2, s));
    SC_TRY(upload(stats_in, (size_t)(K / 256) * M * 8, dst, s));
    SC_TRY(alloc_nan(dfin, (size_t)M * 8, s));
    SC_TRY(alloc_nan(dc, (size_t)M * N * 2, s));
    const float *cos_t = nullptr, *sin_t = nullptr;
    std::vector<float> tab;
    if (rope) {
        tab = sc_rope_table(rope_S, rope_theta);
        SC_TRY(upload(tab.data(), tab.size() * 4, dt, s));
        cos_t = (const float*)dt.p;
        sin_t = cos_t + tab.size() / 2;
    }
    sc_launch_gemm_bf16_ln(epi, da.p, K, dw.p, K, (const float*)dc2.p, nullptr, 0, dc.p, (flags & 1) ? SC_LDC_BLOCKED64 : N, M, N, K, s, (const float*)dc1.p,
                           (const float*)dst.p, (float*)dfin.p, nullptr, nullptr, eps, cos_t, sin_t, rope ? rope_S : 0, rope ? rope_ncols : 0);
    SC_TRY(download(dfin.p, (size_t)M * 8, fin, s));
    return download_bf16(dc.p, (int64_t)M * N, C, s);
}

extern "C" int32_t sc_diag_gemm_strip(int32_t M, int32_t N, int32_t K, int32_t cus) {
    if (M == 0) return sc_gemm_last_strip();
    return sc_gemm_strip_tiles(M, N, K, cus > 0 ? cus : sc_device_cus());
}

extern "C" sc_status sc_diag_gemm_resln(sc_runtime* rt, int32_t flags, const float* A, const float* W, const float* bias, const float* gam, const float* R,
                                        const float* fin, float eps, int32_t M, int32_t N, int32_t K, float* C, float* stats_out) {
    if (!rt || !A || !W || !bias || !gam || !R || !fin || !C || !stats_out) return sc_fail(SC_ERR_INVALID, "sc_diag_gemm_resln: NULL argument");
    if ((flags & ~1) || !(eps > 0.f)) return sc_fail(SC_ERR_INVALID, "sc_diag_gemm_resln: bad flags / eps");
    if (!sc_gemm_ln_supported(M, N, K)) return sc_fail(SC_ERR_UNSUPPORTED, "sc_diag_gemm_resln: need M%%256==0, N%%256==0, K%%256==0");
    SC_HIP(hipSetDevice(rt->device));
    hipStream_t s = rt->stream;
    sc_devbuf fa, da, fw, dw, fr, dr, db, dg, dfin, dc, dso;
    SC_TRY(upload_bf16(A, (int64_t)M * K, fa, da, s));
    SC_TRY(upload_bf16(W, (int64_t)N * K, fw, dw, s));
    SC_TRY(upload_bf16(R, (int64_t)M * N, fr, dr, s));
    SC_TRY(upload(bias, (size_t)N * 4, db, s));
    SC_TRY(upload(gam, (size_t)N * 4, dg, s));
    SC_TRY(upload(fin, (size_t)M * 8, dfin, s));
    SC_TRY(alloc_nan(dc, (size_t)M * N * 2, s));
    SC_TRY(alloc_nan(dso, (size_t)(N / 256) * M * 8, s));
    sc_launch_gemm_bf16_ln(EPI_RESLN_STATS, da.p, (flags & 1) ? SC_LDC_BLOCKED64 : K, dw.p, K, (const float*)db.p, dr.p, N, dc.p, N, M, N, K, s, nullptr, nullptr,
                           (float*)dfin.p, (const float*)dg.p, (float*)dso.p, eps);
    SC_TRY(download(dso.p, (size_t)(N / 256) * M * 8, stats_out, s));
    return download_bf16(dc.p, (int64_t)M * N, C, s);
}

static sc_status diag_attention(const char* who, sc_runtime* rt, const float* qkv, const int32_t* lens, int32_t B, int32_t S, int32_t heads, int32_t blocked_rows,
                                const float* slopes, float* out, int32_t head_dim = 64, RelBiasArg rb = RelBiasArg()) {
    if (!rt || !qkv || !lens || !out || B < 1 || blocked_rows < 0) return sc_fail(SC_ERR_INVALID, "%s: bad argument", who);
    const int H = heads * head_dim;
    if (!sc_attention_supported(S, H, heads, head_dim))
        return sc_fail(SC_ERR_UNSUPPORTED, "%s: S must be one of 32,64,128,256,512,1024,2048, head_dim 64 or 32 (an even number of heads)", who);
    if (head_dim != 64 && slopes) return sc_fail(SC_ERR_UNSUPPORTED, "%s: head dimension %d has no ALiBi kernel", who, head_dim);
    const int64_t tokens = (int64_t)B * S;
    if (blocked_rows && blocked_rows < tokens) return sc_fail(SC_ERR_INVALID, "%s: blocked_rows < B*S", who);
    SC_HIP(hipSetDevice(rt->device));
    hipStream_t s = rt->stream;
    sc_devbuf fq, dq, dl, dsl, dc;
    SC_TRY(upload_bf16(qkv, (blocked_rows ? (int64_t)blocked_rows : tokens) * 3 * H, fq, dq, s));
    SC_TRY(upload(lens, (size_t)B * 4, dl, s));
    if (slopes) SC_TRY(upload(slopes, (size_t)heads * 4, dsl, s));
    SC_TRY(alloc_nan(dc, (size_t)tokens * H * 2, s));
    if (rb.rel_bias) {
        SC_TRY(upload_rel_table(who, rb, heads, dsl, s));
        sc_launch_attention_rel(dq.p, (const int32_t*)dl.p, B, S, H, (const float*)dsl.p, DIAG_REL_SPAN, dc.p, s, blocked_rows);
    } else {
        sc_launch_attention(dq.p, (const int32_t*)dl.p, B, S, H, slopes ? (const float*)dsl.p : nullptr, dc.p, s, blocked_rows, head_dim);
    }
    return download_bf16(dc.p, tokens * H, out, s);
}
extern "C" sc_status sc_diag_attention_bias(sc_runtime* rt, const float* qkv, const int32_t* lens, int32_t B, int32_t S, int32_t heads, int32_t blocked_rows,
                                            const float* rel_bias, int32_t buckets, int32_t max_distance, float* out) {
    if (!rel_bias) return sc_fail(SC_ERR_INVALID, "sc_diag_attention_bias: rel_bias is NULL");
    return diag_attention("sc_diag_attention_bias", rt, qkv, lens, B, S, heads, blocked_rows, nullptr, out, 64, RelBiasArg{rel_bias, buckets, max_distance});
}
extern "C" sc_status sc_diag_attention_hd(sc_runtime* rt, const float* qkv, const int32_t* lens, int32_t B, int32_t S, int32_t heads, int32_t head_dim,
                                          int32_t blocked_rows, const float* slopes, float* out) {
    return diag_attention("sc_diag_attention_hd", rt, qkv, lens, B, S, heads, blocked_rows, slopes, out, head_dim);
}
extern "C" sc_status sc_diag_attention_ex(sc_runtime* rt, const float* qkv, const int32_t* lens, int32_t B, int32_t S, int32_t heads, int32_t blocked_rows,
                                          const float* slopes, float* out) {
    return diag_attention("sc_diag_attention_ex", rt, qkv, lens, B, S, heads, blocked_rows, slopes, out);
}
extern "C" sc_status sc_diag_attention(sc_runtime* rt, const float* qkv, const int32_t* lens, int32_t B, int32_t S, int32_t heads, float* out) {
    return diag_attention("sc_diag_attention", rt, qkv, lens, B, S, heads, 0, nullptr, out);
}

extern "C" sc_status sc_diag_attention_cls(sc_runtime* rt, const float* qkv, const int32_t* lens, int32_t B, int32_t S, int32_t heads, int32_t head_dim,
                                           const float* alibi, float* out) {
    const char* who = "sc_diag_attention_cls";
    if (!rt || !qkv || !lens || !out || B < 1 || B > 65536 || heads < 1) return sc_fail(SC_ERR_INVALID, "%s: bad argument", who);
    if (head_dim != 64 && !(head_dim == 32 && heads % 2 == 0)) return sc_fail(SC_ERR_UNSUPPORTED, "%s: head_dim must be 64, or 32 with an even number of heads", who);
    const int H = heads * head_dim;
    if (S < 1 || S > 2048 || H > 2048) return sc_fail(SC_ERR_INVALID, "%s: S and heads*head_dim must be at most 2048", who);
    const int64_t tokens = (int64_t)B * S, M = (tokens + 255) / 256 * 256, nblk = 3 * H / 64;
    std::vector<float> blocked((size_t)nblk * M * 64, 0.f);
    for (int64_t r = 0; r < tokens; ++r)
        for (int64_t cb = 0; cb < nblk; ++cb) memcpy(&blocked[(size_t)(cb * M + r) * 64], qkv + r * 3 * H + cb * 64, 64 * sizeof(float));
    SC_HIP(hipSetDevice(rt->device));
    hipStream_t s = rt->stream;
    sc_devbuf fq, dq, dl, dsl, dc;
    SC_TRY(upload_bf16(blocked.data(), nblk * M * 64, fq, dq, s));
    SC_TRY(upload(lens, (size_t)B * 4, dl, s));
    if (alibi) SC_TRY(upload(alibi, (size_t)heads * 4, dsl, s));
    SC_TRY(alloc_nan(dc, (size_t)B * H * 2, s));
    sc_launch_attention_cls(dq.p, nullptr, (const int32_t*)dl.p, B, S, (int)M, H, head_dim, alibi ? (const float*)dsl.p : nullptr, dc.p, B, s);
    return download_bf16(dc.p, (int64_t)B * H, out, s);
}

static sc_status diag_attention_packed(const char* who, sc_runtime* rt, const float* qkv, const int32_t* starts, const int32_t* lens, int32_t B, int32_t heads,
                                       int32_t head_dim, int32_t blocked_rows, const float* slopes, float* out, RelBiasArg rb = RelBiasArg()) {
    if (!rt || !qkv || !starts || !lens || !out || B < 1 || B > 65536 || blocked_rows < 0 || heads < 1) return sc_fail(SC_ERR_INVALID, "%s: bad argument", who);
    if (head_dim != 64 && !(head_dim == 32 && heads % 2 == 0 && !slopes))
        return sc_fail(SC_ERR_UNSUPPORTED, "%s: head_dim must be 64, or 32 with an even number of heads and no ALiBi slopes (got %d, %d heads)", who, head_dim, heads);
    if (heads * head_dim > 2048) return sc_fail(SC_ERR_INVALID, "%s: bad argument", who);
    const int H = heads * head_dim;
    int64_t end = 0;
    for (int32_t b = 0; b < B; ++b) {
        if (lens[b] < 1 || lens[b] > 2048 || starts[b] < 0 || (starts[b] % 32) || starts[b] > (1 << 24))
            return sc_fail(SC_ERR_INVALID, "%s: sequence %d: start %d (multiple of 32) / length %d (1..2048) out of range", who, b, starts[b], lens[b]);
        const int64_t e = (int64_t)starts[b] + (lens[b] + 31) / 32 * 32;
        if (e > end) end = e;
    }
    const int64_t R = blocked_rows ? (int64_t)blocked_rows : (end + 255) / 256 * 256;
    if (R < end) return sc_fail(SC_ERR_INVALID, "%s: blocked_rows %d < the last sequence's end %lld", who, blocked_rows, (long long)end);
    SC_HIP(hipSetDevice(rt->device));
    hipStream_t s = rt->stream;
    std::vector<int32_t> items((size_t)B * 8 * 4);
    int nitems[3];
    sc_packed_items(starts, lens, B, items.data(), nitems);
    sc_devbuf fq, dq, di, dsl, dc;
    SC_TRY(upload_bf16(qkv, R * 3 * H, fq, dq, s));
    SC_TRY(upload(items.data(), items.size() * 4, di, s));
    if (slopes) SC_TRY(upload(slopes, (size_t)heads * 4, dsl, s));
    SC_TRY(alloc_nan(dc, (size_t)R * H * 2, s));
    if (rb.rel_bias) {
        SC_TRY(upload_rel_table(who, rb, heads, dsl, s));
        sc_launch_attention_rel_packed(dq.p, (const int32_t*)di.p, nitems, H, (const float*)dsl.p, DIAG_REL_SPAN, dc.p, s, blocked_rows);
    } else {
        sc_launch_attention_packed(dq.p, (const int32_t*)di.p, nitems, H, slopes ? (const float*)dsl.p : nullptr, dc.p, s, blocked_rows, head_dim);
    }
    return download_bf16(dc.p, R * H, out, s);
}
extern "C" sc_status sc_diag_attention_bias_packed(sc_runtime* rt, const float* qkv, const int32_t* starts, const int32_t* lens, int32_t B, int32_t heads,
                                                   int32_t blocked_rows, const float* rel_bias, int32_t buckets, int32_t max_distance, float* out) {
    if (!rel_bias) return sc_fail(SC_ERR_INVALID, "sc_diag_attention_bias_packed: rel_bias is NULL");
    return diag_attention_packed("sc_diag_attention_bias_packed", rt, qkv, starts, lens, B, heads, 64, blocked_rows, nullptr, out,
                                 RelBiasArg{rel_bias, buckets, max_distance});
}
extern "C" sc_status sc_diag_rel_buckets(int32_t rel_buckets, int32_t max_distance, int32_t span, int32_t* out) {
    if (!out || span < 1 || span > (1 << 20)) return sc_fail(SC_ERR_INVALID, "sc_diag_rel_buckets: bad argument (span 1 .. 2^20)");
    if (!sc_rel_buckets_valid(rel_buckets, max_distance))
        return sc_fail(SC_ERR_INVALID, "sc_diag_rel_buckets: rel_buckets must be even, 4 .. 256, and max_distance beyond rel_buckets / 4, got %d / %d", rel_buckets,
                       max_distance);
    sc_rel_buckets(rel_buckets, max_distance, span, out);
    return SC_OK;
}
extern "C" sc_status sc_diag_attention_packed(sc_runtime* rt, const float* qkv, const int32_t* starts, const int32_t* lens, int32_t B, int32_t heads,
                                              int32_t blocked_rows, const float* slopes, float* out) {
    return diag_attention_packed("sc_diag_attention_packed", rt, qkv, starts, lens, B, heads, 64, blocked_rows, slopes, out);
}
extern "C" sc_status sc_diag_attention_packed_hd(sc_runtime* rt, const float* qkv, const int32_t* starts, const int32_t* lens, int32_t B, int32_t heads,
                                                 int32_t head_dim, int32_t blocked_rows, const float* slopes, float* out) {
    return diag_attention_packed("sc_diag_attention_packed_hd", rt, qkv, starts, lens, B, heads, head_dim, blocked_rows, slopes, out);
}

extern "C" sc_status sc_diag_attention_window(sc_runtime* rt, const float* qkv, const int32_t* starts, const int32_t* lens, int32_t B, int32_t S, int32_t heads,
                                              int32_t local_window, int32_t blocked_rows, float* out) {
    const char* who = "sc_diag_attention_window";
    if (!rt || !qkv || !lens || !out || B < 1 || B > 65536 || blocked_rows < 0 || heads < 1 || heads * 64 > 2048) return sc_fail(SC_ERR_INVALID, "%s: bad argument", who);
    if (!sc_attention_window_supported(local_window)) return sc_fail(SC_ERR_UNSUPPORTED, "%s: local_window must be even and within 2 .. 128, got %d", who, local_window);
    const int H = heads * 64;
    int64_t R = 0, rows_out = 0;
    std::vector<int32_t> items;
    int nitems[3] = {0, 0, 0};
    if (starts) {
// ... 424 lines not shown
```

semcode_amd/csrc/sc_encoder_forward.cpp:

```cpp
#include "sc_encoder_state.h"

static void launch_gate(const sc_encoder_cfg& c, const void* h, int64_t tokens, int F, void* out, hipStream_t s) {
    if (c.ffn_type == 2) sc_launch_swiglu(h, tokens, F, out, s);
    else if (c.ffn_type == 4) sc_launch_geglu_tanh(h, tokens, F, out, s);
    else sc_launch_geglu(h, tokens, F, out, s);
}
static int g_rope_fused = -1;
static const int ROPE_FUSED_DEFAULT = 1;
void sc_encoder_set_rope_fused(int v) { g_rope_fused = v < 0 ? -1 : (v ? 1 : 0); }
static int g_cls_prune = -1;
static const int CLS_PRUNE_DEFAULT = 1;
void sc_encoder_set_cls_prune(int v) { g_cls_prune = v < 0 ? -1 : (v ? 1 : 0); }
static bool cls_prune_enabled() { return (g_cls_prune < 0 ? CLS_PRUNE_DEFAULT : g_cls_prune) != 0; }
static bool ffn_blocked_enabled() { static const bool on = sc_env_flag("SC_FFN_BLOCKED", true); return on; }

static void launch_rope(sc_encoder* e, int M, int S, const PackedLayout* pk, hipStream_t s, bool local = false) {
    const float *cos_t = local ? e->rope_cos_l : e->rope_cos, *sin_t = local ? e->rope_sin_l : e->rope_sin;
    const int nblocks = e->cfg.arch == 2 ? e->cfg.heads + e->cfg.kv_heads : 2 * e->cfg.heads;
    if (pk) sc_launch_rope_qk_packed(e->qkv, M, nblocks, pk->pos, e->cfg.max_pos, cos_t, sin_t, s);
    else sc_launch_rope_qk(e->qkv, M, nblocks, S, cos_t, sin_t, s);
}
static void launch_attention(sc_encoder* e, const int32_t* lens_dev, int B, int S, int M, const PackedLayout* pk, hipStream_t s) {
    const int hd = e->cfg.hidden / e->cfg.heads;
    if (pk) sc_launch_attention_packed(e->qkv, pk->items, pk->nitems, e->cfg.hidden, e->slopes, e->ctx, s, M, hd);
    else sc_launch_attention(e->qkv, lens_dev, B, S, e->cfg.hidden, e->slopes, e->ctx, s, M, hd);
}
static void launch_norm(const sc_encoder_cfg& c, const void* in, int tokens, const float* g, const float* b, void* out, hipStream_t s) {
    if (c.arch >= 2) sc_launch_rmsnorm(in, tokens, c.hidden, g, c.ln_eps, out, s);
    else sc_launch_layernorm(in, tokens, c.hidden, g, b, c.ln_eps, out, s);
}
static void launch_layer_rotation(sc_encoder* e, const LayerW& w, int l, int M, int S, const PackedLayout* pk, hipStream_t s) {
    const sc_encoder_cfg& c = e->cfg;
    if (c.arch == 3) return;
    if (c.arch == 2 && (head_width(c) == 128 || c.qk_norm))
        sc_launch_qknorm_rope(e->qkv, M, c.heads, c.kv_heads, head_width(c), S, pk ? pk->pos : nullptr, c.max_pos, e->rope_cos, e->rope_sin, w.qng, w.kng, c.ln_eps, s);
    else launch_rope(e, M, S, pk, s, layer_is_local(c, l));
}
static void launch_layer_attention(sc_encoder* e, int l, const int32_t* lens_dev, int B, int S, int M, const PackedLayout* pk, hipStream_t s) {
    const sc_encoder_cfg& c = e->cfg;
    if (c.arch == 2) {
        if (pk) sc_launch_attention_causal_packed(e->qkv, pk->items, pk->nitems, c.heads, c.kv_heads, head_width(c), e->ctx, s, M);
        else sc_launch_attention_causal(e->qkv, lens_dev, B, S, c.heads, c.kv_heads, head_width(c), e->ctx, s, M);
    } else if (c.arch == 3) {
        if (pk) sc_launch_attention_rel_packed(e->qkv, pk->items, pk->nitems, (int)attn_width(c), e->rel_tbl, c.max_pos, e->ctx, s, M);
        else sc_launch_attention_rel(e->qkv, lens_dev, B, S, (int)attn_width(c), e->rel_tbl, c.max_pos, e->ctx, s, M);
    } else if (layer_is_local(c, l)) {
        if (pk) sc_launch_attention_window_packed(e->qkv, pk->items, pk->nitems, c.hidden, c.local_window, e->ctx, s, M);
        else sc_launch_attention_window(e->qkv, lens_dev, B, S, c.hidden, c.local_window, e->ctx, s, M);
    } else {
        launch_attention(e, lens_dev, B, S, M, pk, s);
    }
}
static sc_status launch_token_head(sc_encoder* e, const void* x, const PackedLayout* pk, hipStream_t s) {
    sc_launch_token_head(x, pk->rows, e->cfg.hidden, e->token.w, e->token.W, pk->per_row, pk->call.tok_out, s);
    SC_HIP(hipGetLastError());
    return SC_OK;
}
static sc_status splitk_scratch(sc_encoder* e, int M, bool batch_invariant, void** sk, size_t* bytes) {
    *sk = nullptr;
    *bytes = 0;
    if (M > 1024 || e->path == 1 || batch_invariant) return SC_OK;
    if (!e->splitk) SC_HIP(hipMalloc(&e->splitk, sc_encoder::SPLITK_BYTES));
    *sk = e->splitk;
    *bytes = sc_encoder::SPLITK_BYTES;
    return SC_OK;
}
static sc_status cls_last_layer(sc_encoder* e, const LayerW& w, const int32_t* lens_dev, int B, int S, int M, const PackedLayout* pk, const float* res_g,
                                const float* res_b, float* out_dev) {
    const sc_encoder_cfg& c = e->cfg;
    sc_runtime* rt = e->rt;
    hipStream_t s = rt->stream;
    const int H = c.hidden, F = c.ffn, Mc = (int)ceil256(B);
    const int32_t* starts = pk ? pk->starts : nullptr;
    void* sk;
    size_t skb;
    if (sc_status st = splitk_scratch(e, Mc, false, &sk, &skb)) return st;
    sc_with_prof(rt, SC_PROF_ATTN, [&] { sc_launch_attention_cls(e->qkv, starts, lens_dev, B, S, M, H, H / c.heads, e->slopes, e->ctx, Mc, s); });
    sc_launch_cls_gather(e->x, starts, B, S, H, res_g, res_b, c.ln_eps, e->x1, Mc, s);
    sc_with_prof(rt, SC_PROF_GEMM, [&] { sc_launch_gemm_bf16(EPI_BIAS_RES, e->ctx, H, w.wo, H, w.bo, e->x1, H, e->y, H, Mc, H, H, s, sk, skb); });
    sc_launch_layernorm(e->y, Mc, H, w.ln1g, w.ln1b, c.ln_eps, e->x1, s);
    const void* ffn_in = e->hm;
    sc_with_prof(rt, SC_PROF_GEMM, [&] {
        if (ffn_gated(c)) sc_launch_gemm_bf16(EPI_BIAS, e->x1, H, w.w1, H, w.b1, nullptr, 0, e->hm, 2 * F, Mc, 2 * F, H, s, sk, skb);
        else sc_launch_gemm_bf16(EPI_BIAS_GELU, e->x1, H, w.w1, H, w.b1, nullptr, 0, e->hm, F, Mc, F, H, s, sk, skb);
    });
    if (ffn_gated(c)) {
        launch_gate(c, e->hm, Mc, F, e->hg, s);
        ffn_in = e->hg;
    }
    sc_with_prof(rt, SC_PROF_GEMM, [&] { sc_launch_gemm_bf16(EPI_BIAS_RES, ffn_in, F, w.w2, F, w.b2, e->x1, H, e->y, H, Mc, H, F, s, sk, skb); });
    sc_launch_cls_pool(e->y, nullptr, B, 1, H, w.ln2g, w.ln2b, c.ln_eps, out_normalize(e, pk), out_dev, s);
    SC_HIP(hipGetLastError());
    return SC_OK;
}
static void launch_mean_pool(sc_encoder* e, const void* x, const int32_t* lens_dev, int B, int S, const PackedLayout* pk, float* out_dev, hipStream_t s) {
    if (pk) sc_launch_mean_pool_packed(x, pk->starts, lens_dev, B, e->cfg.hidden, out_normalize(e, pk), out_dev, s);
    else sc_launch_mean_pool(x, lens_dev, B, S, e->cfg.hidden, out_normalize(e, pk), out_dev, s);
}

static sc_status forward_folded_locked(sc_encoder* e, const int32_t* ids_dev, const int32_t* lens_dev, int32_t B, int32_t S, float* out_dev,
                                       const PackedLayout* pk) {
    const sc_encoder_cfg& c = e->cfg;
    sc_runtime* rt = e->rt;
    hipStream_t s = rt->stream;
    const int H = c.hidden, F = c.ffn;
    const int tokens = pk ? pk->rows : B * S;
    const int M = (int)ceil256(tokens);
    const int slots = H / 256;
    const bool gated = ffn_gated(c);
    const bool ffn_blocked = !gated && ffn_blocked_enabled();
    const bool rope = c.pos_type == 2, rope_fused = rope && !pk && (g_rope_fused < 0 ? ROPE_FUSED_DEFAULT : g_rope_fused) != 0;
    const bool cls = cls_pooling(e, pk), prune = cls && cls_prune_enabled();
    if (pair_call(pk))
        sc_launch_embed_raw_pairs(ids_dev, pk->pos, pk->per_row, tokens, M, H, c.vocab, c.max_pos, c.type_vocab, e->wemb, e->pemb, e->temb, e->x, e->stat_b, slots, s);
    else if (pk) sc_launch_embed_raw_packed(ids_dev, pk->pos, tokens, M, H, c.vocab, c.max_pos, e->wemb, e->pemb, e->temb, e->x, e->stat_b, slots, s);
    else sc_launch_embed_raw(ids_dev, tokens, M, S, H, c.vocab, c.max_pos, e->wemb, e->pemb, e->temb, e->x, e->stat_b, slots, s);
    for (int l = 0; l < c.layers; ++l) {
        const LayerW& w = e->layers[l];
        sc_with_prof(rt, SC_PROF_GEMM, [&] {
            if (rope_fused)
                sc_launch_gemm_bf16_ln(EPI_LNA_BIAS_ROPE, e->x, H, w.wqkv_f, H, w.c2q, nullptr, 0, e->qkv, SC_LDC_BLOCKED64, M, 3 * H, H, s, w.c1q, e->stat_b, e->fin_b,
                                       nullptr, nullptr, c.ln_eps, e->rope_cos, e->rope_sin, S, 2 * H);
            else
                sc_launch_gemm_bf16_ln(EPI_LNA_BIAS, e->x, H, w.wqkv_f, H, w.c2q, nullptr, 0, e->qkv, SC_LDC_BLOCKED64, M, 3 * H, H, s, w.c1q, e->stat_b, e->fin_b, nullptr,
                                       nullptr, c.ln_eps);
        });
        if (rope && !rope_fused) launch_rope(e, M, S, pk, s);
        if (prune && l == c.layers - 1)
            return cls_last_layer(e, w, lens_dev, B, S, M, pk, w.g_prev, l == 0 ? e->embb : e->layers[l - 1].ln2b, out_dev);
        sc_with_prof(rt, SC_PROF_ATTN, [&] { launch_attention(e, lens_dev, B, S, M, pk, s); });
        sc_with_prof(rt, SC_PROF_GEMM, [&] {
            sc_launch_gemm_bf16_ln(EPI_RESLN_STATS, e->ctx, H, w.wo, H, w.bb_o, e->x, H, e->y, H, M, H, H, s, nullptr, nullptr, e->fin_b, w.g_prev, e->stat_a, c.ln_eps);
        });
        const void* ffn_in = e->hm;
        sc_with_prof(rt, SC_PROF_GEMM, [&] {
            if (gated)
                sc_launch_gemm_bf16_ln(EPI_LNA_BIAS, e->y, H, w.w1_f, H, w.c2f, nullptr, 0, e->hm, 2 * F, M, 2 * F, H, s, w.c1f, e->stat_a, e->fin_a, nullptr, nullptr, c.ln_eps);
            else
                sc_launch_gemm_bf16_ln(EPI_LNA_GELU, e->y, H, w.w1_f, H, w.c2f, nullptr, 0, e->hm, ffn_blocked ? SC_LDC_BLOCKED64 : F, M, F, H, s, w.c1f, e->stat_a,
                                       e->fin_a, nullptr, nullptr, c.ln_eps);
        });
        if (gated) {
            launch_gate(c, e->hm, M, F, e->hg, s);
            ffn_in = e->hg;
        }
        sc_with_prof(rt, SC_PROF_GEMM, [&] {
            sc_launch_gemm_bf16_ln(EPI_RESLN_STATS, ffn_in, ffn_blocked ? SC_LDC_BLOCKED64 : F, w.w2, F, w.bb_2, e->y, H, e->x, H, M, H, F, s, nullptr,
                                   nullptr, e->fin_a, w.ln1g, e->stat_b, c.ln_eps);
        });
    }
    const LayerW& last = e->layers[c.layers - 1];
    if (token_call(pk)) {
        sc_launch_layernorm(e->x, tokens, H, last.ln2g, last.ln2b, c.ln_eps, e->x1, s);
        return launch_token_head(e, e->x1, pk, s);
    }
    if (cls) {
        sc_launch_cls_pool(e->x, pk ? pk->starts : nullptr, B, S, H, last.ln2g, last.ln2b, c.ln_eps, out_normalize(e, pk), out_dev, s);
    } else if (out_normalize(e, pk)) {
        sc_launch_layernorm(e->x, tokens, H, last.ln2g, last.ln2b, c.ln_eps, e->x1, s);
        launch_mean_pool(e, e->x1, lens_dev, B, S, pk, out_dev, s);
    } else if (pk) {
        sc_launch_mean_pool_ln_packed(e->x, e->stat_b, slots, M, last.ln2g, last.ln2b, c.ln_eps, pk->starts, lens_dev, B, H, out_dev, s);
    } else {
        sc_launch_mean_pool_ln(e->x, e->stat_b, slots, M, last.ln2g, last.ln2b, c.ln_eps, lens_dev, B, S, H, out_dev, s);
    }
    SC_HIP(hipGetLastError());
    return SC_OK;
}

static sc_status forward_raw_locked(sc_encoder* e, const int32_t* ids_dev, const int32_t* lens_dev, int32_t B, int32_t S, float* out_dev,
                                    const PackedLayout* pk) {
    const sc_encoder_cfg& c = e->cfg;
    sc_runtime* rt = e->rt;
    hipStream_t s = rt->stream;
    const bool causal = c.arch == 2, raw_emb = c.arch >= 2;
    const int H = c.hidden, F = c.ffn, AW = (int)attn_width(c), QN = AW + 2 * (int)kv_width(c);
    const int tokens = pk ? pk->rows : B * S;
    const int M = (int)ceil256(tokens);
    const bool scored = scored_call(pk);
    void* sk;
    size_t skb;
    if (sc_status st = splitk_scratch(e, M, scored || token_call(pk), &sk, &skb)) return st;
    if (raw_emb && pk) sc_launch_embed_raw_packed(ids_dev, pk->pos, tokens, M, H, c.vocab, c.max_pos, e->wemb, nullptr, e->temb, e->x, nullptr, 0, s);
    else if (raw_emb) sc_launch_embed_raw(ids_dev, tokens, M, S, H, c.vocab, c.max_pos, e->wemb, nullptr, e->temb, e->x, nullptr, 0, s);
    else if (pk) sc_launch_embed_ln_packed(ids_dev, pk->pos, tokens, H, c.vocab, c.max_pos, e->wemb, nullptr, e->temb, e->embg, e->embb, c.ln_eps, e->x, s);
    else sc_launch_embed_ln(ids_dev, tokens, S, H, c.vocab, c.max_pos, e->wemb, nullptr, e->temb, e->embg, e->embb, c.ln_eps, e->x, s);
    for (int l = 0; l < c.layers; ++l) {
        const LayerW& w = e->layers[l];
        const void* a = e->x;
        if (raw_emb || l > 0) {
            launch_norm(c, e->x, tokens, w.ln1g, w.ln1b, e->x1, s);
            a = e->x1;
        }
        sc_with_prof(rt, SC_PROF_GEMM, [&] { sc_launch_gemm_bf16(EPI_BIAS, a, H, w.wqkv, H, w.bqkv, nullptr, 0, e->qkv, SC_LDC_BLOCKED64, M, QN, H, s, sk, skb); });
        launch_layer_rotation(e, w, l, M, S, pk, s);
        sc_with_prof(rt, SC_PROF_ATTN, [&] { launch_layer_attention(e, l, lens_dev, B, S, M, pk, s); });
        sc_with_prof(rt, SC_PROF_GEMM, [&] { sc_launch_gemm_bf16(EPI_BIAS_RES, e->ctx, AW, w.wo, AW, w.bo, e->x, H, e->y, H, M, H, AW, s, sk, skb); });
        launch_norm(c, e->y, tokens, w.ln2g, w.ln2b, e->x1, s);
        const void* ffn_in = e->hg;
        if (c.ffn_type == 3) {
            sc_with_prof(rt, SC_PROF_GEMM, [&] { sc_launch_gemm_bf16(EPI_BIAS, e->x1, H, w.w1, H, w.b1, nullptr, 0, e->hm, F, M, F, H, s, sk, skb); });
            sc_launch_relu(e->hm, (int64_t)M * F, s);
            ffn_in = e->hm;
        } else {
            sc_with_prof(rt, SC_PROF_GEMM, [&] { sc_launch_gemm_bf16(EPI_BIAS, e->x1, H, w.w1, H, w.b1, nullptr, 0, e->hm, 2 * F, M, 2 * F, H, s, sk, skb); });
            launch_gate(c, e->hm, M, F, e->hg, s);
        }
        sc_with_prof(rt, SC_PROF_GEMM, [&] { sc_launch_gemm_bf16(EPI_BIAS_RES, ffn_in, F, w.w2, F, w.b2, e->y, H, e->x, H, M, H, F, s, sk, skb); });
    }
    const int32_t* starts = pk ? pk->starts : nullptr;
    if (causal && (scored || e->pooling == 2)) {
        sc_launch_last_pool(e->x, starts, lens_dev, B, S, H, e->fing, c.ln_eps, out_normalize(e, pk), out_dev, s);
    } else if (c.arch == 3 && cls_pooling(e, pk)) {
        sc_launch_last_pool(e->x, starts, e->ones, B, S, H, e->fing, c.ln_eps, out_normalize(e, pk), out_dev, s);
    } else if (!causal && (scored ? pk->call.head_pool == 1 : cls_pooling(e, pk))) {
        sc_launch_cls_pool(e->x, starts, B, S, H, e->fing, e->finb, c.ln_eps, out_normalize(e, pk), out_dev, s);
    } else {
        launch_norm(c, e->x, tokens, e->fing, e->finb, e->x1, s);
        if (token_call(pk)) return launch_token_head(e, e->x1, pk, s);
        launch_mean_pool(e, e->x1, lens_dev, B, S, pk, out_dev, s);
    }
    SC_HIP(hipGetLastError());
    return SC_OK;
}

sc_status forward_locked(sc_encoder* e, const int32_t* ids_dev, const int32_t* lens_dev, int32_t B, int32_t S, float* out_dev, const PackedLayout* pk) {
    const sc_encoder_cfg& c = e->cfg;
    sc_runtime* rt = e->rt;
    hipStream_t s = rt->stream;
    const int H = c.hidden, F = c.ffn;
    const int tokens = pk ? pk->rows : B * S;
    const int M = (int)ceil256(tokens);
    if (c.arch != 0) return forward_raw_locked(e, ids_dev, lens_dev, B, S, out_dev, pk);
    static const bool env_fold = sc_env_flag("SC_ENC_FOLD", true);
    const bool tok = token_call(pk);
    if (e->foldable && e->path != 2 && (M > 1024 || e->path == 1 || tok) && env_fold) return forward_folded_locked(e, ids_dev, lens_dev, B, S, out_dev, pk);
    void* sk;
    size_t skb;
    if (sc_status st = splitk_scratch(e, M, tok, &sk, &skb)) return st;
    const bool gated = ffn_gated(c);
    const bool ffn_blocked = !sk && !gated && (F % 256) == 0 && (H % 256) == 0 && ffn_blocked_enabled();
    const bool cls = cls_pooling(e, pk), prune = cls && cls_prune_enabled();
    if (pair_call(pk))
        sc_launch_embed_ln_pairs(ids_dev, pk->pos, pk->per_row, tokens, H, c.vocab, c.max_pos, c.type_vocab, e->wemb, e->pemb, e->temb, e->embg, e->embb, c.ln_eps, e->x, s);
    else if (pk) sc_launch_embed_ln_packed(ids_dev, pk->pos, tokens, H, c.vocab, c.max_pos, e->wemb, e->pemb, e->temb, e->embg, e->embb, c.ln_eps, e->x, s);
    else sc_launch_embed_ln(ids_dev, tokens, S, H, c.vocab, c.max_pos, e->wemb, e->pemb, e->temb, e->embg, e->embb, c.ln_eps, e->x, s);
    for (int l = 0; l < c.layers; ++l) {
        const LayerW& w = e->layers[l];
        sc_with_prof(rt, SC_PROF_GEMM, [&] {
            sc_launch_gemm_bf16(EPI_BIAS, e->x, H, w.wqkv, H, w.bqkv, nullptr, 0, e->qkv, SC_LDC_BLOCKED64, M, 3 * H, H, s, sk, skb);
        });
        if (c.pos_type == 2) launch_rope(e, M, S, pk, s);
        if (prune && l == c.layers - 1) return cls_last_layer(e, w, lens_dev, B, S, M, pk, nullptr, nullptr, out_dev);
        sc_with_prof(rt, SC_PROF_ATTN, [&] { launch_attention(e, lens_dev, B, S, M, pk, s); });
        sc_with_prof(rt, SC_PROF_GEMM, [&] { sc_launch_gemm_bf16(EPI_BIAS_RES, e->ctx, H, w.wo, H, w.bo, e->x, H, e->y, H, M, H, H, s, sk, skb); });
        sc_launch_layernorm(e->y, tokens, H, w.ln1g, w.ln1b, c.ln_eps, e->x1, s);
        const void* ffn_in = e->hm;
        sc_with_prof(rt, SC_PROF_GEMM, [&] {
            if (gated) sc_launch_gemm_bf16(EPI_BIAS, e->x1, H, w.w1, H, w.b1, nullptr, 0, e->hm, 2 * F, M, 2 * F, H, s, sk, skb);
            else sc_launch_gemm_bf16(EPI_BIAS_GELU, e->x1, H, w.w1, H, w.b1, nullptr, 0, e->hm, ffn_blocked ? SC_LDC_BLOCKED64 : F, M, F, H, s, sk, skb);
        });
        if (gated) {
            launch_gate(c, e->hm, M, F, e->hg, s);
            ffn_in = e->hg;
        }
        sc_with_prof(rt, SC_PROF_GEMM, [&] { sc_launch_gemm_bf16(EPI_BIAS_RES, ffn_in, ffn_blocked ? SC_LDC_BLOCKED64 : F, w.w2, F, w.b2, e->x1, H, e->y, H, M, H, F, s, sk, skb); });
        sc_launch_layernorm(e->y, tokens, H, w.ln2g, w.ln2b, c.ln_eps, e->x, s);
    }
    if (tok) return launch_token_head(e, e->x, pk, s);
    if (cls) sc_launch_cls_pool(e->x, pk ? pk->starts : nullptr, B, S, H, nullptr, nullptr, c.ln_eps, out_normalize(e, pk), out_dev, s);
    else launch_mean_pool(e, e->x, lens_dev, B, S, pk, out_dev, s);
    SC_HIP(hipGetLastError());
    return SC_OK;
}
```

semcode_amd/csrc/sc_encoder_model.cpp:

```cpp
#include <cmath>
#include <new>

#include "rel_bucket_rule.h"
#include "sc_encoder_state.h"

static int64_t blob_floats(const sc_encoder_cfg& c) {
    const int64_t H = c.hidden, F = c.ffn, F1 = ffn_gated(c) ? 2 * F : F;
    const int64_t KV = kv_width(c), AW = attn_width(c);
    int64_t n = (int64_t)c.vocab * H + (c.pos_type != 0 ? 0 : (int64_t)c.max_pos * H) + (c.arch != 0 ? 0 : (int64_t)c.type_vocab * H) + (c.arch >= 2 ? 0 : 2 * H);
    if (c.pos_type == 3) n += (int64_t)c.rel_buckets * c.heads;
    n += (int64_t)c.layers * ((AW * H + AW) + (H * AW + H) + 2 * (KV * H + KV) + 2 * H + (F1 * H + F1) + (H * F + H) + 2 * H);
    if (c.arch == 2 && c.qk_norm) n += (int64_t)c.layers * 2 * head_width(c);
    if (c.arch != 0) n += 2 * H;
    return n;
}
extern "C" sc_status sc_encoder_blob_bytes(const sc_encoder_cfg* cfg, int64_t* out) {
    if (!cfg || !out) return sc_fail(SC_ERR_INVALID, "sc_encoder_blob_bytes: NULL argument");
    *out = blob_floats(*cfg) * 4;
    return SC_OK;
}

static sc_status check_cfg(const sc_encoder_cfg& c) {
    if (c.vocab < 1 || c.hidden < 1 || c.layers < 1 || c.heads < 1 || c.ffn < 1 || c.max_pos < 1 || c.type_vocab < 1)
        return sc_fail(SC_ERR_INVALID, "sc_encoder_create: non-positive model dimension");
// ... 121 lines not shown
    e->rel_tbl = c.pos_type == 3 ? a.f32((size_t)c.heads * (2 * (size_t)c.max_pos - 1)) : nullptr;
    e->temb = a.f32(c.arch != 0 ? H : (size_t)c.type_vocab * H);
    e->fing = c.arch != 0 ? a.f32(H) : nullptr;
    e->finb = c.arch != 0 ? a.f32(H) : nullptr;
    e->embg = a.f32(H);
    e->embb = a.f32(H);
    for (LayerW& w : e->layers) {
        w.wqkv = a.bf16(QN * H);    w.bqkv = a.f32(QN);
        w.wo = a.bf16(H * AW);      w.bo = a.f32(H);
        w.qng = c.arch == 2 && c.qk_norm ? a.f32((size_t)head_width(c)) : nullptr;
        w.kng = c.arch == 2 && c.qk_norm ? a.f32((size_t)head_width(c)) : nullptr;
        w.ln1g = a.f32(H);          w.ln1b = a.f32(H);
        w.w1 = a.bf16(F1 * H);      w.b1 = a.f32(F1);
        w.w2 = a.bf16(H * F);       w.b2 = a.f32(H);
        w.ln2g = a.f32(H);          w.ln2b = a.f32(H);
        if (!e->foldable) continue;
        w.wqkv_f = a.bf16(3 * H * H); w.c1q = a.f32(3 * H); w.c2q = a.f32(3 * H);
        w.w1_f = a.bf16(F1 * H);      w.c1f = a.f32(F1);    w.c2f = a.f32(F1);
        w.bb_o = a.f32(H);            w.bb_2 = a.f32(H);
    }
}

extern "C" sc_status sc_encoder_create(sc_runtime* rt, const sc_encoder_cfg* cfg, const void* weights_blob, size_t nbytes, sc_encoder** out) {
    if (!rt || !cfg || !out) return sc_fail(SC_ERR_INVALID, "sc_encoder_create: NULL argument");
    *out = nullptr;
    sc_status st = check_cfg(*cfg);
    if (st) return st;
    const int64_t nfl = blob_floats(*cfg);
    if (weights_blob && (int64_t)nbytes != nfl * 4)
        return sc_fail(SC_ERR_INVALID, "sc_encoder_create: weight blob is %zu bytes, config needs %lld", nbytes, (long long)(nfl * 4));
    SC_HIP(hipSetDevice(rt->device));
    hipStream_t s = rt->stream;
    sc_encoder* e = new (std::nothrow) sc_encoder();
    if (!e) return sc_fail(SC_ERR_NOMEM, "out of host memory");
    e->rt = rt;
    sc_runtime_retain(rt);
    e->cfg = *cfg;
    if (e->cfg.arch == 2 && e->cfg.kv_heads == 0) e->cfg.kv_heads = e->cfg.heads;
    if (e->cfg.arch == 2) e->cfg.head_dim = head_width(*cfg);
    const int64_t H = cfg->hidden, F = cfg->ffn, L = cfg->layers, F1 = ffn_gated(*cfg) ? 2 * F : F, KV = kv_width(*cfg), AW = attn_width(*cfg), HD = head_width(*cfg);

    float* blob = nullptr;
    hipError_t he = hipMalloc((void**)&blob, (size_t)nfl * 4);
    if (he != hipSuccess) {
        delete e;
        sc_runtime_release(rt);
        return sc_fail(SC_ERR_NOMEM, "hipMalloc weight staging (%lld B) failed: %s", (long long)nfl * 4, hipGetErrorString(he));
    }
    auto fail = [&](sc_status code) {
        hipFree(blob);
        hipFree(e->params);
        delete e;
        sc_runtime_release(rt);
        return code;
    };
    e->foldable = cfg->arch == 0 && (H % 256) == 0 && (F % 256) == 0 && (F1 % 256) == 0 && ((3 * H) % 256) == 0;
    e->layers.resize(L);
    Arena arena;
    layout_params(e, arena);
    he = hipMalloc((void**)&e->params, arena.used);
    if (he != hipSuccess) return fail(sc_fail(SC_ERR_NOMEM, "hipMalloc parameters (%zu B) failed: %s", arena.used, hipGetErrorString(he)));
    arena = Arena{e->params};
    layout_params(e, arena);

    if (weights_blob) {
        he = hipMemcpyAsync(blob, weights_blob, (size_t)nfl * 4, hipMemcpyHostToDevice, s);
        if (he != hipSuccess) return fail(sc_fail(SC_ERR_HIP, "weight upload failed: %s", hipGetErrorString(he)));
    } else {
        sc_launch_synth_scaled(blob, nfl, cfg->synth_seed, 0.02f, 0.0f, s);
    }
    int64_t off = 0;
    auto take = [&](int64_t n) { float* p = blob + off; off += n; return p; };
    enum { COPY, ONES, ZEROS };
    auto put_f32 = [&](float* d, const float* src, int64_t n, int synth) {
        if (!weights_blob && synth == ONES) sc_launch_synth_scaled(d, n, 0, 0.0f, 1.0f, s);
        else if (!weights_blob && synth == ZEROS) hipMemsetAsync(d, 0, (size_t)n * 4, s);
        else hipMemcpyAsync(d, src, (size_t)n * 4, hipMemcpyDeviceToDevice, s);
    };
    auto put_bf16 = [&](void* d, const float* src, int64_t n) { sc_launch_f32_to_bf16(src, d, n, s); };
    auto put_host = [&](float* d, const std::vector<float>& v) {
        hipMemcpyAsync(d, v.data(), v.size() * 4, hipMemcpyHostToDevice, s);
        hipStreamSynchronize(s);
    };
    put_f32(e->wemb, take((int64_t)cfg->vocab * H), (int64_t)cfg->vocab * H, COPY);
    if (e->pemb) put_f32(e->pemb, take((int64_t)cfg->max_pos * H), (int64_t)cfg->max_pos * H, COPY);
    if (e->slopes) put_host(e->slopes, alibi_slopes(cfg->heads));
    if (e->rope_cos) put_host(e->rope_cos, sc_rope_table(cfg->max_pos, cfg->rope_theta, (int)HD));
    if (e->rope_cos_l) put_host(e->rope_cos_l, sc_rope_table(cfg->max_pos, cfg->rope_theta_local));
    if (e->rel_tbl) {
        const int64_t nb = (int64_t)cfg->rel_buckets * cfg->heads;
        std::vector<float> rb((size_t)nb);
        he = hipMemcpyAsync(rb.data(), take(nb), (size_t)nb * 4, hipMemcpyDeviceToHost, s);
        if (he == hipSuccess) he = hipStreamSynchronize(s);
        if (he != hipSuccess) return fail(sc_fail(SC_ERR_HIP, "relative bias download failed: %s", hipGetErrorString(he)));
        put_host(e->rel_tbl, sc_rel_bias_table(rb.data(), cfg->rel_buckets, cfg->heads, cfg->rel_max_distance, cfg->max_pos));
    }
    if (cfg->arch != 0) hipMemsetAsync(e->temb, 0, (size_t)H * 4, s);
    else put_f32(e->temb, take((int64_t)cfg->type_vocab * H), (int64_t)cfg->type_vocab * H, COPY);
    if (cfg->arch < 2) {
        put_f32(e->embg, take(H), H, ONES);
        put_f32(e->embb, take(H), H, ZEROS);
    }
    for (int64_t l = 0; l < L; ++l) {
        LayerW& w = e->layers[l];
        const float* wqkv_f32[3];
        for (int p = 0; p < 3; ++p) {
            const int64_t rows = p == 0 ? AW : KV, row0 = p == 0 ? 0 : AW + (p - 1) * KV;
            wqkv_f32[p] = take(rows * H);
            put_bf16((char*)w.wqkv + (size_t)row0 * H * 2, wqkv_f32[p], rows * H);
            put_f32(w.bqkv + row0, take(rows), rows, ZEROS);
        }
        put_bf16(w.wo, take(H * AW), H * AW);
        put_f32(w.bo, take(H), H, ZEROS);
        put_f32(w.ln1g, take(H), H, ONES);
        put_f32(w.ln1b, take(H), H, ZEROS);
        const float* w1_f32 = take(F1 * H);
        put_bf16(w.w1, w1_f32, F1 * H);
        put_f32(w.b1, take(F1), F1, ZEROS);
        put_bf16(w.w2, take(H * F), H * F);
        put_f32(w.b2, take(H), H, ZEROS);
        put_f32(w.ln2g, take(H), H, ONES);
        put_f32(w.ln2b, take(H), H, ZEROS);
        if (w.qng) {
            put_f32(w.qng, take(HD), HD, ONES);
            put_f32(w.kng, take(HD), HD, ONES);
        }
        if (e->foldable) {
            const float* gp = l == 0 ? e->embg : e->layers[l - 1].ln2g;
            const float* bp = l == 0 ? e->embb : e->layers[l - 1].ln2b;
            w.g_prev = gp;
            for (int p = 0; p < 3; ++p)
                sc_launch_fold_ln_weights(wqkv_f32[p], gp, bp, w.bqkv + p * H, (int)H, (int)H, (char*)w.wqkv_f + (size_t)p * H * H * 2, w.c1q + p * H, w.c2q + p * H, s);
            sc_launch_fold_ln_weights(w1_f32, w.ln1g, w.ln1b, w.b1, (int)F1, (int)H, w.w1_f, w.c1f, w.c2f, s);
            sc_launch_add_vectors(w.bo, bp, w.bb_o, (int)H, s);
            sc_launch_add_vectors(w.b2, w.ln1b, w.bb_2, (int)H, s);
        }
    }
    if (e->fing) {
        put_f32(e->fing, take(H), H, ONES);
        put_f32(e->finb, take(H), H, ZEROS);
    }
    he = hipStreamSynchronize(s);
    if (he == hipSuccess) he = hipGetLastError();
    if (he != hipSuccess) return fail(sc_fail(SC_ERR_HIP, "encoder parameter setup failed: %s", hipGetErrorString(he)));
    hipFree(blob);
    *out = e;
    return SC_OK;
}

extern "C" sc_status sc_encoder_destroy(sc_encoder* e) {
    if (!e) return SC_OK;
    hipSetDevice(e->rt->device);
    hipStreamSynchronize(e->rt->stream);
    hipFree(e->params);
    hipFree(e->ws);
    hipFree(e->splitk);
    hipFree(e->pair.mem);
    hipFree(e->proj.mem);
    hipFree(e->score.mem);
    hipFree(e->token.mem);
    hipFree(e->tok[0].p);
    hipFree(e->tok[1].p);
    hipFree(e->late_aux.p);
    for (auto& slot : e->pin) {
        if (slot.host) hipHostFree(slot.host);
        if (slot.done) hipEventDestroy(slot.done);
    }
    sc_runtime* rt = e->rt;
    delete e;
    sc_runtime_release(rt);
    return SC_OK;
}

static void layout_ws(sc_encoder* e, Arena& a, size_t tokens, size_t nb) {
    const size_t H = e->cfg.hidden, F = e->cfg.ffn, F1 = ffn_gated(e->cfg) ? 2 * F : F, slots = H / 256;
    const size_t AW = (size_t)attn_width(e->cfg), QN = AW + 2 * (size_t)kv_width(e->cfg);
    e->x = a.bf16(tokens * H);
    e->x1 = a.bf16(tokens * H);
    e->y = a.bf16(tokens * H);
    e->qkv = a.bf16(tokens * (QN > 3 * H ? QN : 3 * H));
    e->ctx = a.bf16(tokens * (AW > H ? AW : H));
    e->hm = a.bf16(tokens * F1);
    e->hg = ffn_gated(e->cfg) ? a.bf16(tokens * F) : nullptr;
    e->ids = (int32_t*)a.take(tokens * 4);
    e->lens = (int32_t*)a.take(nb * 4);
    e->ones = e->cfg.arch == 3 ? (int32_t*)a.take(nb * 4) : nullptr;
    e->plan = (char*)a.take(PlanOffsets(tokens, nb, PackedCall::PAIRS).total);
    e->pooled = a.f32(nb * H);
    e->projected = e->proj.mem ? a.f32(nb * (size_t)e->proj.E) : nullptr;
    e->logits = a.f32(nb * 2);
    e->stat_a = e->foldable ? a.f32(slots * tokens * 2) : nullptr;
    e->stat_b = e->foldable ? a.f32(slots * tokens * 2) : nullptr;
    e->fin_a = e->foldable ? a.f32(tokens * 2) : nullptr;
    e->fin_b = e->foldable ? a.f32(tokens * 2) : nullptr;
}

sc_status ensure_ws(sc_encoder* e, int64_t rows, int64_t B) {
    const int64_t tokens = ceil256(rows);
    if (tokens <= e->ws_tokens && B <= e->ws_batch) return SC_OK;
    SC_HIP(hipStreamSynchronize(e->rt->stream));
    hipFree(e->ws);
    e->ws = nullptr;
    e->ws_tokens = 0;
    e->ws_batch = 0;
    Arena arena;
    layout_ws(e, arena, (size_t)tokens, (size_t)B);
    hipError_t he = hipMalloc((void**)&e->ws, arena.used);
    if (he != hipSuccess) return sc_fail(SC_ERR_NOMEM, "hipMalloc encoder workspace (%zu B) failed: %s", arena.used, hipGetErrorString(he));
    SC_HIP(hipMemsetAsync(e->ws, 0, arena.used, e->rt->stream));
    arena = Arena{e->ws};
    layout_ws(e, arena, (size_t)tokens, (size_t)B);
    if (e->ones) SC_HIP(hipMemsetD32Async((hipDeviceptr_t)e->ones, 1, (size_t)B, e->rt->stream));
    e->ws_tokens = tokens;
    e->ws_batch = B;
    return SC_OK;
}

extern "C" sc_status sc_encoder_info(sc_encoder* e, sc_encoder_cfg* cfg_out) {
    if (!e || !cfg_out) return sc_fail(SC_ERR_INVALID, "sc_encoder_info: NULL argument");
    *cfg_out = e->cfg;
    return SC_OK;
}
```

semcode_amd/csrc/sc_encoder_plan.cpp:

```cpp
#include "sc_encoder_plan.h"

#include <cstring>

void sc_packed_items(const int32_t* starts, const int32_t* lens, int64_t B, int32_t* items, int nitems[3]) {
    int32_t* w = items;
    for (int cls = 0; cls < 3; ++cls) {
        const int32_t* w0 = w;
        for (int64_t i = 0; i < B; ++i) {
            if (sc_packed_attention_class(lens[i]) != cls) continue;
            const int nqb = (int)(ceil32(lens[i]) / 32);
            for (int qb = 0; qb < (cls == 0 ? nqb : 1); qb += 8, w += 4) { w[0] = starts[i]; w[1] = lens[i]; w[2] = qb; w[3] = 0; }
        }
        nitems[cls] = (int)((w - w0) / 4);
    }
}

sc_status sc_plan_check_offsets(const int64_t* offsets, int32_t B, const PlanBounds& mb, const char* who, int64_t* rows) {
    if (!offsets) return sc_fail(SC_ERR_INVALID, "%s: NULL argument", who);
    if (B < 1 || B > 65536) return sc_fail(SC_ERR_INVALID, "%s: batch %d out of range", who, B);
    if (offsets[0] != 0) return sc_fail(SC_ERR_INVALID, "%s: offsets[0] must be 0 (got %lld)", who, (long long)offsets[0]);
    const int64_t max_len = mb.pos_type != 1 && mb.max_pos < 2048 ? mb.max_pos : 2048;
    int64_t used = 0;
    for (int32_t i = 0; i < B; ++i) {
        const int64_t len = offsets[i + 1] - offsets[i];
        if (len < 1) return sc_fail(SC_ERR_INVALID, "%s: text %d has length %lld (every text needs at least one token)", who, i, (long long)len);
        if (len > max_len)
            return sc_fail(SC_ERR_INVALID, "%s: text %d has %lld tokens, more than %lld (the smaller of 2048 and the model's max_pos)", who, i, (long long)len, (long long)max_len);
        used += ceil32(len);
    }
    if (ceil256(used) > SC_ENCODER_PACKED_MAX_ROWS)
        return sc_fail(SC_ERR_UNSUPPORTED, "%s: %lld token rows, more than SC_ENCODER_PACKED_MAX_ROWS = %d (split the batch)", who, (long long)used, SC_ENCODER_PACKED_MAX_ROWS);
    *rows = used;
    return SC_OK;
}

sc_status sc_plan_check_pairs(const int64_t* offsets, const int32_t* first_lens, int32_t B, const PlanBounds& mb, const char* who) {
    for (int32_t i = 0; i < B; ++i) {
        const int64_t len = offsets[i + 1] - offsets[i];
        if (len < 2) return sc_fail(SC_ERR_INVALID, "%s: pair %d has %lld token(s) (a pair needs at least 2)", who, i, (long long)len);
        if (first_lens[i] < 1 || first_lens[i] > len)
            return sc_fail(SC_ERR_INVALID, "%s: first_lens[%d] = %d outside 1 .. %lld (the pair's length)", who, i, first_lens[i], (long long)len);
        if (first_lens[i] < len && mb.type_vocab < 2)
            return sc_fail(SC_ERR_INVALID, "%s: pair %d has a second segment, the model's type_vocab is %d (needs 2)", who, i, mb.type_vocab);
    }
    return SC_OK;
}

sc_status sc_plan_check_tokens(const int64_t* offsets, int32_t B, int32_t expand_id, bool query, const PlanBounds& mb, const char* who, int64_t* used,
                               int64_t* nrows) {
    sc_status st = sc_plan_check_offsets(offsets, B, mb, who, used);
    if (st) return st;
    if (expand_id >= mb.vocab) return sc_fail(SC_ERR_INVALID, "%s: expand_id %d outside the vocabulary (%d tokens)", who, expand_id, mb.vocab);
    *nrows = expand_id >= 0 ? *used : offsets[B];
    if (!query) return SC_OK;
    const bool local_layers = mb.arch == 1 && mb.global_every > 1;
    for (int32_t i = 0; i < B; ++i) {
        const int64_t len = offsets[i + 1] - offsets[i];
        if (len > mb.max_query) return sc_fail(SC_ERR_INVALID, "%s: query %d has %lld tokens, more than %d", who, i, (long long)len, mb.max_query);
        if (expand_id >= 0 && local_layers && ceil32(len) - len > mb.local_window / 2)
            return sc_fail(SC_ERR_INVALID, "%s: query %d has %lld tokens: its last expansion row would see no key within local_window %d", who, i, (long long)len,
                           mb.local_window);
    }
    return SC_OK;
}

int64_t sc_plan_fill(const int32_t* ids, const int64_t* offsets, int32_t B, const PackedCall& call, const PlanOffsets& po, int64_t M, char* buf, int nitems[3]) {
    int32_t* h_ids = (int32_t*)(buf + po.ids);
    int32_t* h_pos = (int32_t*)(buf + po.pos);
    int32_t* h_starts = (int32_t*)(buf + po.starts);
    int32_t* h_lens = (int32_t*)(buf + po.lens);
    memset(h_ids, 0, (size_t)M * 4);
    memset(h_pos, 0, (size_t)M * 4);
    int64_t row = 0;
    for (int32_t i = 0; i < B; ++i) {
        const int64_t len = offsets[i + 1] - offsets[i], span = ceil32(len);
        h_starts[i] = (int32_t)row;
        h_lens[i] = (int32_t)len;
        memcpy(h_ids + row, ids + offsets[i], (size_t)len * 4);
        for (int64_t j = 0; j < span; ++j) h_pos[row + j] = (int32_t)j;
        row += span;
    }
    if (call.kind == PackedCall::PAIRS) {
        int32_t* h_types = (int32_t*)(buf + po.types);
        int32_t* h_ones = (int32_t*)(buf + po.ones);
        memset(h_types, 0, (size_t)M * 4);
        for (int32_t i = 0; i < B; ++i) {
            for (int32_t j = call.first_lens[i]; j < h_lens[i]; ++j) h_types[h_starts[i] + j] = 1;
            h_ones[i] = 1;
        }
    }
    if (call.kind == PackedCall::TOKENS) {
        int32_t* h_dst = (int32_t*)(buf + po.dst);
        memset(h_dst, 0xFF, (size_t)M * 4);
        int32_t at = 0;
        for (int32_t i = 0; i < B; ++i) {
            const int32_t n = call.expand_id >= 0 ? (int32_t)ceil32(h_lens[i]) : h_lens[i];
            for (int32_t j = h_lens[i]; j < n; ++j) h_ids[h_starts[i] + j] = call.expand_id;
            for (int32_t j = 0; j < n; ++j) h_dst[h_starts[i] + j] = at++;
        }
    }
    sc_packed_items(h_starts, h_lens, B, (int32_t*)(buf + po.items), nitems);
    return row;
}
```

semcode_amd/csrc/sc_encoder_plan.h:

```cpp
#pragma once
#include <cstddef>
#include <cstdint>

#include "../../include/semcode_hip.h"

sc_status sc_fail(sc_status code, const char* fmt, ...);
int sc_packed_attention_class(int len);

static inline int64_t ceil32(int64_t v) { return (v + 31) & ~(int64_t)31; }
static inline int64_t ceil256(int64_t v) { return (v + 255) & ~(int64_t)255; }

struct PackedCall {
    enum Kind {
        TEXTS,
        PAIRS,
        SCORED,
        TOKENS
    } kind = TEXTS;
    const int32_t* first_lens = nullptr;
    int head_pool = -1;
    int32_t expand_id = -1;
    float* tok_out = nullptr;
    static PackedCall pairs(const int32_t* first_lens) { PackedCall c; c.kind = PAIRS; c.first_lens = first_lens; return c; }
    static PackedCall scored(int head_pool) { PackedCall c; c.kind = SCORED; c.head_pool = head_pool; return c; }
    static PackedCall tokens(int32_t expand_id, float* out) { PackedCall c; c.kind = TOKENS; c.expand_id = expand_id; c.tok_out = out; return c; }
};

inline int64_t sc_packed_items_cap(int64_t rows, int64_t B) { return B + rows / 256; }
void sc_packed_items(const int32_t* starts, const int32_t* lens, int64_t B, int32_t* items, int nitems[3]);

struct PlanOffsets {
    size_t ids, pos, starts, lens, items, types = 0, ones = 0, dst = 0, total;
    PlanOffsets(size_t M, size_t B, PackedCall::Kind kind = PackedCall::TEXTS) {
        size_t u = 0;
        auto take = [&](size_t bytes) { const size_t at = u; u += (size_t)ceil256((int64_t)bytes); return at; };
        ids = take(M * 4);
        pos = take(M * 4);
        starts = take(B * 4);
        lens = take(B * 4);
        items = take((size_t)sc_packed_items_cap((int64_t)M, (int64_t)B) * 16);
        if (kind == PackedCall::PAIRS) {
            types = take(M * 4);
            ones = take(B * 4);
        }
        if (kind == PackedCall::TOKENS) dst = take(M * 4);
        total = u;
    }
};

struct PlanBounds {
    int max_pos, pos_type, vocab, type_vocab, arch, global_every, local_window;
    int max_query;
};

sc_status sc_plan_check_offsets(const int64_t* offsets, int32_t B, const PlanBounds& mb, const char* who, int64_t* rows);
sc_status sc_plan_check_pairs(const int64_t* offsets, const int32_t* first_lens, int32_t B, const PlanBounds& mb, const char* who);
sc_status sc_plan_check_tokens(const int64_t* offsets, int32_t B, int32_t expand_id, bool query, const PlanBounds& mb, const char* who, int64_t* used,
                               int64_t* nrows);

int64_t sc_plan_fill(const int32_t* ids, const int64_t* offsets, int32_t B, const PackedCall& call, const PlanOffsets& po, int64_t M, char* buf, int nitems[3]);
```

semcode_amd/csrc/sc_encoder_state.h:

```cpp
#pragma once
#include <vector>

#include "encoder_ops.h"
#include "maxsim_rule.h"
#include "sc_encoder_plan.h"
#include "sc_internal.h"

struct LayerW {
    void* wqkv;
    float* bqkv;
    void* wo;
    float* bo;
    float *qng = nullptr, *kng = nullptr;
    float *ln1g, *ln1b;
    void* w1;
    float* b1;
    void* w2;
    float* b2;
    float *ln2g, *ln2b;
    void *wqkv_f = nullptr, *w1_f = nullptr;
    float *c1q = nullptr, *c2q = nullptr, *c1f = nullptr, *c2f = nullptr;
    const float* g_prev = nullptr;
    float *bb_o = nullptr, *bb_2 = nullptr;
};

struct PairHead {
    char* mem = nullptr;
    float *wp = nullptr, *bp = nullptr, *wc = nullptr, *bc = nullptr;
    int labels = 0;
};
struct ScoreHead {
    char* mem = nullptr;
    float *wd = nullptr, *bd = nullptr, *g = nullptr, *b = nullptr, *wc = nullptr, *bc = nullptr;
    int kind = 0, pooling = 0, labels = 0;
    float eps = 0.f;
};
struct TokenHead {
    char* mem = nullptr;
    void* w = nullptr;
    int W = 0;
};

struct OutProj {
    char* mem = nullptr;
    float *w = nullptr, *b = nullptr;
    int E = 0;
};

struct sc_encoder {
    sc_runtime* rt = nullptr;
    sc_encoder_cfg cfg{};
    char* params = nullptr;
    float *wemb = nullptr, *pemb = nullptr, *temb = nullptr, *embg = nullptr, *embb = nullptr;
    float* slopes = nullptr;
    float *rope_cos = nullptr, *rope_sin = nullptr;
    float *rope_cos_l = nullptr, *rope_sin_l = nullptr;
    float *fing = nullptr, *finb = nullptr;
    float* rel_tbl = nullptr;
    std::vector<LayerW> layers;
    int64_t ws_tokens = 0;
    char* ws = nullptr;
    void *x = nullptr, *x1 = nullptr, *y = nullptr, *qkv = nullptr, *ctx = nullptr, *hm = nullptr, *hg = nullptr;
    int32_t* ids = nullptr;
    int32_t* lens = nullptr;
    int32_t* ones = nullptr;
    char* plan = nullptr;
    float* pooled = nullptr;
    float* logits = nullptr;
    int64_t ws_batch = 0;
    float *stat_a = nullptr, *stat_b = nullptr;
    float *fin_a = nullptr, *fin_b = nullptr;
    bool foldable = false;
    int path = 0;
    int pooling = 0;
    void* splitk = nullptr;
    static constexpr size_t SPLITK_BYTES = 64u << 20;
    struct PinSlot {
        char* host = nullptr;
        size_t cap = 0;
        hipEvent_t done = nullptr;
        bool busy = false;
    } pin[2];
    int pin_next = 0;
    PairHead pair;
    OutProj proj;
    float* projected = nullptr;
    ScoreHead score;
    TokenHead token;
    struct Grown {
        char* p = nullptr;
        size_t cap = 0;
    } tok[2], late_aux;
    std::mutex mu;
};

struct PackedLayout {
    const int32_t *pos, *starts, *items;
    int nitems[3];
    int rows;
    PackedCall call;
    const int32_t* per_row;
};
static inline bool pair_call(const PackedLayout* pk) { return pk && pk->call.kind == PackedCall::PAIRS; }
static inline bool scored_call(const PackedLayout* pk) { return pk && pk->call.kind == PackedCall::SCORED; }
static inline bool token_call(const PackedLayout* pk) { return pk && pk->call.kind == PackedCall::TOKENS; }
static inline bool cls_pooling(const sc_encoder* e, const PackedLayout* pk) { return e->pooling == 1 && (!pk || pk->call.kind == PackedCall::TEXTS); }
static inline int out_normalize(const sc_encoder* e, const PackedLayout* pk) {
    return pair_call(pk) || scored_call(pk) || (e->proj.mem && (!pk || pk->call.kind == PackedCall::TEXTS)) ? 0 : e->cfg.normalize;
}
static inline int out_width(const sc_encoder* e) { return e->proj.mem ? e->proj.E : e->cfg.hidden; }

struct Arena {
    char* base = nullptr;
    size_t used = 0;
    void* take(size_t bytes) { const size_t o = used; used += sc_align256(bytes); return base ? base + o : nullptr; }
    float* f32(size_t n) { return (float*)take(n * 4); }
    void* bf16(size_t n) { return take(n * 2); }
};

static inline bool ffn_gated(const sc_encoder_cfg& c) { return c.ffn_type == 1 || c.ffn_type == 2 || c.ffn_type == 4; }
static inline bool t5_stated_heads(const sc_encoder_cfg& c) { return c.arch == 3 && c.head_dim == 64; }
static inline int head_width(const sc_encoder_cfg& c) { return c.arch == 2 && c.head_dim == 128 ? 128 : 64; }
static inline int64_t attn_width(const sc_encoder_cfg& c) { return c.arch == 2 || t5_stated_heads(c) ? (int64_t)c.heads * head_width(c) : (int64_t)c.hidden; }
static inline int64_t kv_width(const sc_encoder_cfg& c) { return c.arch == 2 ? (int64_t)(c.kv_heads > 0 ? c.kv_heads : c.heads) * head_width(c) : attn_width(c); }
static inline bool layer_is_local(const sc_encoder_cfg& c, int l) { return c.arch == 1 && c.global_every > 1 && (l % c.global_every) != 0; }
static inline PlanBounds plan_bounds(const sc_encoder* e) {
    const sc_encoder_cfg& c = e->cfg;
    return PlanBounds{c.max_pos, c.pos_type, c.vocab, c.type_vocab, c.arch, c.global_every, c.local_window, MAXSIM_MAX_NQ};
}

sc_status ensure_ws(sc_encoder* e, int64_t rows, int64_t B);
sc_status forward_locked(sc_encoder* e, const int32_t* ids_dev, const int32_t* lens_dev, int32_t B, int32_t S, float* out_dev, const PackedLayout* pk = nullptr);
sc_status check_packed_offsets(sc_encoder* e, const int64_t* offsets, int32_t B, const char* who, int64_t* rows);
sc_status pin_slot_wait(sc_encoder::PinSlot& slot);
sc_status embed_packed_locked(sc_encoder* e, const int32_t* ids, const int64_t* offsets, int32_t B, int64_t used, sc_encoder::PinSlot& slot, const PackedCall& call,
                              const int64_t* index_rows = nullptr, const int64_t** rows_out = nullptr);

template <class Tail>
static sc_status packed_call_locked(sc_encoder* e, const int32_t* ids, const int64_t* offsets, int32_t B, int64_t used, const PackedCall& call,
                                    const int64_t* index_rows, bool in_flight, Tail&& tail) {
    SC_HIP(hipSetDevice(e->rt->device));
    sc_encoder::PinSlot& slot = e->pin[e->pin_next];
    sc_status st = pin_slot_wait(slot);
    if (st) return st;
    hipStream_t s = e->rt->stream;
    const int64_t* h_rows = nullptr;
    st = embed_packed_locked(e, ids, offsets, B, used, slot, call, index_rows, &h_rows);
    if (!st) st = tail(h_rows);
    if (st) {
        hipStreamSynchronize(s);
        return st;
    }
    if (!in_flight) {
        SC_HIP(hipStreamSynchronize(s));
        return SC_OK;
    }
    SC_HIP(hipEventRecord(slot.done, s));
    slot.busy = true;
    e->pin_next ^= 1;
    return SC_OK;
}
```

semcode_amd/csrc/sc_internal.h:

```cpp
#pragma once
#include <atomic>
#include <cstdlib>
#include <mutex>
#include <utility>
#include <vector>

#include "sc_common.h"

#define SC_PROF_SCAN 0
#define SC_PROF_MERGE 1
#define SC_PROF_GEMM 2
#define SC_PROF_ATTN 3
#define SC_PROF_CLASSES 4

sc_status sc_fail(sc_status code, const char* fmt, ...);

#define SC_HIP(expr)                                                                                  \
    do {                                                                                              \
        hipError_t _e = (expr);                                                                       \
        if (_e != hipSuccess) return sc_fail(SC_ERR_HIP, "%s failed: %s", #expr, hipGetErrorString(_e)); \
    } while (0)

struct sc_runtime {
    std::atomic<int> refs{1};
    int device = 0;
    hipStream_t stream = nullptr;
    bool own_stream = false;
    int profiling = 0;
    unsigned prof_seen[8] = {0, 0, 0, 0, 0, 0, 0, 0};
    char name[256] = {0};
    int cus = 256;
    int64_t hbm = 0;
    std::mutex mu;
    std::vector<std::pair<hipEvent_t, hipEvent_t>> prof[SC_PROF_CLASSES];
};

void sc_runtime_retain(sc_runtime* rt);
void sc_runtime_release(sc_runtime* rt);
void sc_prof_begin(sc_runtime* rt, int which, hipEvent_t* a, hipEvent_t* b);
void sc_prof_end(sc_runtime* rt, int which, hipEvent_t a, hipEvent_t b);
template <class F>
static inline void sc_with_prof(sc_runtime* rt, int which, F&& launch) {
    hipEvent_t a, b;
    sc_prof_begin(rt, which, &a, &b);
    launch();
    sc_prof_end(rt, which, a, b);
}

struct sc_buf {
    void* p = nullptr;
    size_t cap = 0;
    template <class T> T* as() const { return (T*)p; }
};

struct sc_devbuf {
    void* p = nullptr;
    ~sc_devbuf() { hipFree(p); }
    hipError_t alloc(size_t n) { return hipMalloc(&p, n ? n : 16); }
    template <class T> T* take() { T* q = (T*)p; p = nullptr; return q; }
};

struct sc_shadow {
    sc_buf arr[2];
    size_t row_bytes[2] = {0, 0};
    int64_t rows = 0;
    int64_t tail_pad = 0;
    unsigned* maxima = nullptr;
    std::vector<int64_t> dirty;
    int stat_bit = 0;
};

struct sc_index {
    sc_runtime* rt = nullptr;
    int dim = 0, ld = 0;
    sc_metric metric = SC_METRIC_IP;
    sc_index_kind kind = SC_INDEX_FLAT;
    int nlist = 0;
    int64_t row_base = 0;
    int64_t n = 0, capacity = 0;
    float* X = nullptr;
    float* xnorm = nullptr;
    bool trained = false;
    sc_buf stage, qpad, qnorm, partial, io;
    sc_shadow sh_b16;
    sc_shadow sh_i8;
    int coarse_mode = 0;
    bool i8_off = false;
    int last_coarse_bits = 0;
    int last_uncert_i8 = 0;
    bool wide_i8 = false;
    int last_wide = 0;
    bool i8_sticky = false;
    double cost_i8_first = 0.0;
    bool collect_off8 = false, collect_off16 = false;
    int last_collect_tried = 0, last_collect_resolved = 0;
    sc_buf bscratch;
    sc_buf fb, fb2;
    sc_buf tailbuf;
    int64_t last_tail_rows = 0;
    sc_buf mask_words, mask_cnt, mask_sel;
    int64_t last_mask_allowed = 0, last_mask_scanned = 0;
    int last_mask_gathered = 0;
    sc_buf groups, group_scratch;
    int64_t group_rows = -1;
    int last_group_width0 = 0, last_group_continued = 0, last_group_rounds = 0;
    int64_t last_group_scanned = 0;
    sc_buf mmr_scratch, mmr_stat;
    int last_mmr_fetch = 0;
    bool mmr_stat_pending = false;
    int64_t last_mmr_scanned = 0;
    sc_buf terms, lex_stat, lex_scratch;
    int64_t term_rows = -1, term_cap = 0;
    int term_T = 0;
    bool lex_stat_dirty = true;
    int64_t last_lex_rows = 0, last_lex_bytes = 0;
    int last_lex_passes = 0;
    sc_index* quant = nullptr;
    uint32_t* perm = nullptr;
    int64_t* list_off = nullptr;
    std::vector<uint32_t> inv_h;
    std::vector<int64_t> list_off_h;
    std::vector<int32_t> assign_h;
    int nlist_trained = 0;
    int64_t ivf_rows = 0;
    int64_t perm_rows = 0;
    std::vector<int64_t> dirty_rows;
    sc_buf ivf_scratch;
    sc_shadow sh_c8;
    sc_shadow* const shadows[3] = {&sh_b16, &sh_i8, &sh_c8};
    static constexpr int64_t SC_SHADOW_DIRTY_MAX = 8192;
    sc_buf ivfc_scratch;
    bool ivfc_off = false;
    int last_ivfc_uncertified = 0;
    int last_probed_lists = 0;
    int64_t last_unique_rows = 0, last_streamed_rows = 0;
    int last_groups = 0;
    int search_mode = 0;
    int last_path = 0;
    int last_uncertified = 0;
    int64_t last_del_rows_moved = 0, last_del_bytes_moved = 0;
    int last_del_kept = 0, last_del_dropped = 0;
    double uncert_frac = -1.0;
    std::mutex mu;
};

struct sc_index_buf { sc_buf sc_index::*buf; bool released; };
inline constexpr sc_index_buf SC_INDEX_BUFS[] = {
    {&sc_index::stage, true},   {&sc_index::partial, true},     {&sc_index::bscratch, true},     {&sc_index::fb, true},
    {&sc_index::fb2, true},     {&sc_index::tailbuf, true},     {&sc_index::ivf_scratch, true},  {&sc_index::ivfc_scratch, true},
    {&sc_index::mask_words, true}, {&sc_index::mask_cnt, true}, {&sc_index::mask_sel, true}, {&sc_index::group_scratch, true},
    {&sc_index::mmr_scratch, true}, {&sc_index::lex_scratch, true},
    {&sc_index::qpad, false},   {&sc_index::qnorm, false},      {&sc_index::io, false},          {&sc_index::groups, false},
    {&sc_index::mmr_stat, false},   {&sc_index::terms, false},      {&sc_index::lex_stat, false},
};

static inline int sc_ld8(const sc_index* ix) { return (ix->ld + 127) / 128 * 128; }
static inline size_t sc_ivfc_stats_words(int nlist_trained) { return (size_t)nlist_trained * 2 + 4; }
static inline unsigned* sc_ivfc_xmax_slot(const sc_index* ix) { return ix->sh_c8.maxima + (size_t)ix->nlist_trained * 2; }
static inline size_t sc_align256(size_t v) { return (v + 255) & ~(size_t)255; }
struct sc_carver {
    size_t off = 0;
    size_t operator()(size_t bytes) { const size_t o = off; off += sc_align256(bytes); return o; }
};
template <class T>
struct sc_scoped_set {
    T& ref;
    const T saved;
    sc_scoped_set(T& r, T v) : ref(r), saved(r) { r = v; }
    ~sc_scoped_set() { ref = saved; }
    sc_scoped_set(const sc_scoped_set&) = delete;
};
static inline int64_t sc_env_i64(const char* name, int64_t dflt) { const char* e = getenv(name); return e ? (int64_t)atoll(e) : dflt; }
static inline bool sc_env_flag(const char* name, bool dflt) { const char* e = getenv(name); return !e ? dflt : dflt ? e[0] != '0' : e[0] == '1'; }

sc_status sc_grow(sc_index* ix, sc_buf& b, size_t need);
void sc_buf_free(sc_buf& b);
void sc_shadow_invalidate(sc_shadow& sh);
void sc_shadow_release(sc_shadow& sh);
void sc_shadow_free_maxima(sc_shadow& sh);
void sc_invalidate_shadows(sc_index* ix);
void sc_shadow_note_overwritten(sc_shadow& sh, const int64_t* rows, const int64_t* pos, int64_t n, int64_t old_n);
sc_status sc_ensure_shadow_b16(sc_index* ix);
sc_status sc_ensure_shadow_i8(sc_index* ix);
sc_status sc_prep_queries(sc_index* ix, const float* q_dev, int32_t Q);
struct sc_subbatch { float* q; float* d; int64_t* r; int32_t* idx; int R; };
sc_status sc_subbatch_stage(sc_index* ix, sc_buf& buf, const float* q_dev, const std::vector<int>& which, int k, sc_subbatch* sb);
sc_status sc_subbatch_scatter(sc_index* ix, const sc_subbatch& sb, int k, float* out_dist, int64_t* out_rows);

sc_status sc_check_query_args(const char* who, bool any_null, int32_t Q, int32_t k, int32_t k_max);
sc_status sc_check_allow_null(const char* who, const void* allow, int64_t allow_words);
sc_status sc_check_allow_words(const char* who, const sc_index* ix, const void* allow, int64_t allow_words);
struct sc_host_io { float* q; float* dist; int64_t* rows; const uint32_t* allow; char* extra; };
sc_status sc_stage_host_locked(sc_index* ix, const float* q, int32_t Q, int32_t k, const uint32_t* allow, size_t extra_bytes, sc_host_io* io);
sc_status sc_fetch_host_locked(sc_index* ix, const sc_host_io& io, int32_t Q, int32_t k, float* out_dist, int64_t* out_rows);
sc_status sc_search_exhaustive_locked(sc_index* ix, const float* q_dev, int32_t Q, int32_t k, float* out_dist, int64_t* out_rows);
sc_status sc_candidates_locked(sc_index* ix, const float* q_dev, int32_t Q, int32_t W, const uint32_t* allow_dev, float* cand_dist, int64_t* cand_rows, int64_t* scanned,
                               int64_t* allowed);

sc_status sc_search_dev_locked(sc_index* ix, const float* q_dev, int32_t Q, int32_t k, int32_t nprobe, float* out_dist, int64_t* out_rows);
sc_status sc_search_flat_locked(sc_index* ix, const float* q_dev, int32_t Q, int32_t k, float* out_dist, int64_t* out_rows);
sc_status sc_ivf_search_locked(sc_index* ix, const float* q_dev, int32_t Q, int32_t k, int32_t nprobe, float* out_dist, int64_t* out_rows);
bool sc_ivf_listmajor_applicable(const sc_index* ix, int Q, int k, int nprobe, bool flat_is_batched);
sc_status sc_ivf_search_listmajor_locked(sc_index* ix, const float* q_dev, int32_t Q, int32_t k, int32_t nprobe, float* out_dist, int64_t* out_rows);
bool sc_ivf_coarse_applicable(const sc_index* ix, int Q, int k, int nprobe);
sc_status sc_ivf_search_coarse_locked(sc_index* ix, const float* q_dev, int32_t Q, int32_t k, int32_t nprobe, float* out_dist, int64_t* out_rows, int chunk = 0);
int sc_ivf_exact_probe_path(int ld, int R, int k, int nprobe, int cus);
sc_status sc_ivf_untrain_locked(sc_index* ix);
void sc_ivf_drop_lists_locked(sc_index* ix);
sc_status sc_ivf_cover_tail_locked(sc_index* ix);
sc_status sc_ivf_refresh_locked(sc_index* ix, bool keep_tail = false);
static inline int64_t sc_perm_entries(const sc_index* ix) { return ix->perm ? (ix->perm_rows > 0 ? ix->perm_rows : ix->ivf_rows) : 0; }
static inline int64_t sc_ivf_pos(const sc_index* ix, int64_t r) { return r < ix->ivf_rows ? (int64_t)ix->inv_h[(size_t)r] : r; }
sc_status sc_index_put_rows_locked(sc_index* ix, const float* vecs, bool vecs_on_device, const int64_t* rows, int64_t n, const char* who);
bool sc_ivf_applicable(const sc_index* ix, int Q, int nprobe);
sc_status sc_search_masked_locked(sc_index* ix, const float* q_dev, int32_t Q, int32_t k, const uint32_t* allow_dev, float* out_dist, int64_t* out_rows);
void sc_lex_drop_locked(sc_index* ix);
struct sc_ivf_probes { float* dist; int64_t* lists; char* extra; };
sc_status sc_ivf_probe_quantizer_locked(sc_index* ix, const float* q_dev, int Q, int nprobe, size_t extra_bytes, sc_ivf_probes* out,
                                        std::vector<int64_t>* host = nullptr);
struct IvfPlanParams;
bool sc_ivf_plan_params(int ld, int k, int nprobe, int cus, IvfPlanParams* pp, ScanPlan* plan = nullptr, ScanPlan* plan_res = nullptr);

void sc_ivf_set_refresh_nomem(int v);
void sc_ivf_set_refine_cap(int v);
void sc_ivf_set_coarse_nomem(int v);
void sc_set_collect_pass(int v);
void sc_set_tighten(int v);
void sc_set_wide_force(int v);
void sc_set_ivf_tail_rows(int v);
void sc_set_delete_chunk_rows(int v);
void sc_set_mask_gather(int v);
void sc_set_group_width0(int v);
void sc_set_group_width1(int v);
void sc_set_mmr_chunk_q(int v);
void sc_set_lex_chunk_q(int v);
void sc_encoder_set_rope_fused(int v);
void sc_encoder_set_cls_prune(int v);
```

Before: 22770 chunks/s.

## Split encoder batch into two halves run concurrently on two streams

The folded encoder forward now divides the batch into two halves, each with its own row-offset view of the workspace buffers, and issues every layer's kernels for both halves alternately on the main stream and a second non-blocking stream, joined with events. The aim is to let kernels of different kinds (attention, GEMMs, elementwise work) from the two halves overlap on the GPU and fill CUs left idle by individual launches. By default the split applies when the per-half tile count covers the device CUs; it can be forced on or off by option or environment variable. The trade-off is more kernel launches, smaller GEMMs per launch, and contention between concurrent kernels for cache and bandwidth. Profiling events are extended to record per-stream parts.

```diff
diff --git a/include/semcode_hip.h b/include/semcode_hip.h
--- a/include/semcode_hip.h
+++ b/include/semcode_hip.h
@@ -157,6 +157,8 @@
                            const float* stats_in, float eps, int32_t M, int32_t N, int32_t K, int32_t rope_S, float rope_theta,
                            int32_t rope_ncols, float* C, float* fin);
 int32_t sc_diag_gemm_strip(int32_t M, int32_t N, int32_t K, int32_t cus);
+int32_t sc_diag_enc_split(int32_t B, int32_t S, int32_t H, int32_t cus, int32_t by_options);
+int32_t sc_diag_enc_split_last(void);
 sc_status sc_diag_gemm_resln(sc_runtime* rt, int32_t flags, const float* A, const float* W, const float* bias, const float* gam, const float* R,
                              const float* fin, float eps, int32_t M, int32_t N, int32_t K, float* C, float* stats_out);
 sc_status sc_diag_attention_ex(sc_runtime* rt, const float* qkv, const int32_t* lens, int32_t B, int32_t S, int32_t heads, int32_t blocked_rows,
diff --git a/semcode_amd/_native.py b/semcode_amd/_native.py
--- a/semcode_amd/_native.py
+++ b/semcode_amd/_native.py
@@ -125,6 +125,8 @@
     "sc_diag_ffn_act": (C.c_int32, [C.c_void_p, C.c_int32, C.c_void_p, C.c_int32, C.c_int32, C.c_void_p]),
     "sc_diag_fold_ln": (C.c_int32, [C.c_void_p] * 5 + [C.c_int32, C.c_int32] + [C.c_void_p] * 3),
     "sc_diag_gemm_strip": (C.c_int32, [C.c_int32] * 4),
+    "sc_diag_enc_split": (C.c_int32, [C.c_int32] * 5),
+    "sc_diag_enc_split_last": (C.c_int32, []),
     "sc_diag_gemm_lna": (C.c_int32, [C.c_void_p, C.c_int32, C.c_int32] + [C.c_void_p] * 5 + [C.c_float, C.c_int32, C.c_int32, C.c_int32, C.c_int32,
                                      C.c_float, C.c_int32, C.c_void_p, C.c_void_p]),
     "sc_diag_gemm_resln": (C.c_int32, [C.c_void_p, C.c_int32] + [C.c_void_p] * 6 + [C.c_float, C.c_int32, C.c_int32, C.c_int32, C.c_void_p, C.c_void_p]),
@@ -1255,6 +1257,14 @@
     return int(lib().sc_diag_gemm_strip(int(M), int(N), int(K), int(cus)))
 
 
+def diag_enc_split(B: int, S: int, H: int, cus: int = 0, by_options: bool = True) -> int:
+    return int(lib().sc_diag_enc_split(int(B), int(S), int(H), int(cus), 1 if by_options else 0))
+
+
+def diag_enc_split_last() -> int:
+    return int(lib().sc_diag_enc_split_last())
+
+
 def diag_gemm_resln(rt: Runtime, A, W, bias, gam, R, fin, eps: float, a_blocked: bool = False):
     A, W, bias, gam, R, fin = _f32(A), _f32(W), _f32(bias), _f32(gam), _f32(R), _f32(fin)
     M, K = A.shape
diff --git a/semcode_amd/csrc/sc_api.cpp b/semcode_amd/csrc/sc_api.cpp
--- a/semcode_amd/csrc/sc_api.cpp
+++ b/semcode_amd/csrc/sc_api.cpp
@@ -68,10 +68,12 @@
 
 static void prof_clear(sc_runtime* rt) {
     for (int c = 0; c < SC_PROF_CLASSES; ++c) {
-        for (auto& p : rt->prof[c]) {
-            hipEventDestroy(p.first);
-            hipEventDestroy(p.second);
-        }
+        for (auto& p : rt->prof[c])
+            for (int i = 0; i < sc_prof_sample::MAX_PARTS; ++i)
+                if (p.a[i]) {
+                    hipEventDestroy(p.a[i]);
+                    hipEventDestroy(p.b[i]);
+                }
         rt->prof[c].clear();
     }
 }
@@ -126,19 +128,39 @@
     return SC_OK;
 }
 
-void sc_prof_begin(sc_runtime* rt, int which, hipEvent_t* a, hipEvent_t* b) {
-    *a = *b = nullptr;
+void sc_prof_open(sc_runtime* rt, int which, int parts, sc_prof_sample* p) {
+    *p = sc_prof_sample{};
     if (!rt->profiling || rt->prof[which].size() >= 8192) return;
     if (which >= SC_PROF_GEMM && rt->profiling > 1 && (rt->prof_seen[which]++ % (unsigned)rt->profiling) != 0) return;
-    if (hipEventCreate(a) != hipSuccess) { *a = nullptr; return; }
-    if (hipEventCreate(b) != hipSuccess) { hipEventDestroy(*a); *a = *b = nullptr; return; }
-    hipEventRecord(*a, rt->stream);
+    for (int i = 0; i < parts && i < sc_prof_sample::MAX_PARTS; ++i)
+        if (hipEventCreate(&p->a[i]) != hipSuccess || hipEventCreate(&p->b[i]) != hipSuccess) {
+            for (int j = 0; j <= i; ++j) {
+                if (p->a[j]) hipEventDestroy(p->a[j]);
+                if (p->b[j]) hipEventDestroy(p->b[j]);
+            }
+            *p = sc_prof_sample{};
+            return;
+        }
+}
+void sc_prof_close(sc_runtime* rt, int which, const sc_prof_sample& p) {
+    if (!p.a[0]) return;
+    std::lock_guard<std::mutex> g(rt->mu);
+    rt->prof[which].push_back(p);
+}
+void sc_prof_begin(sc_runtime* rt, int which, hipEvent_t* a, hipEvent_t* b) {
+    sc_prof_sample p;
+    sc_prof_open(rt, which, 1, &p);
+    *a = p.a[0];
+    *b = p.b[0];
+    if (*a) hipEventRecord(*a, rt->stream);
 }
 void sc_prof_end(sc_runtime* rt, int which, hipEvent_t a, hipEvent_t b) {
     if (!a) return;
     hipEventRecord(b, rt->stream);
-    std::lock_guard<std::mutex> g(rt->mu);
-    rt->prof[which].push_back({a, b});
+    sc_prof_sample p;
+    p.a[0] = a;
+    p.b[0] = b;
+    sc_prof_close(rt, which, p);
 }
 
 extern "C" sc_status sc_runtime_profile_read(sc_runtime* rt, int32_t which, double* total_ms, int64_t* launches) {
@@ -147,10 +169,11 @@
     SC_HIP(hipStreamSynchronize(rt->stream));
     double t = 0;
     std::lock_guard<std::mutex> g(rt->mu);
-    for (auto& p : rt->prof[which]) {
-        float ms = 0;
-        if (hipEventElapsedTime(&ms, p.first, p.second) == hipSuccess) t += ms;
-    }
+    for (auto& p : rt->prof[which])
+        for (int i = 0; i < sc_prof_sample::MAX_PARTS && p.a[i]; ++i) {
+            float ms = 0;
+            if (hipEventElapsedTime(&ms, p.a[i], p.b[i]) == hipSuccess) t += ms;
+        }
     if (total_ms) *total_ms = t;
     if (launches) *launches = (int64_t)rt->prof[which].size();
     return SC_OK;
@@ -189,7 +212,7 @@
         {"group_width0", sc_set_group_width0},                {"group_width1", sc_set_group_width1},
         {"mmr_chunk_q", sc_set_mmr_chunk_q},                  {"lex_chunk_q", sc_set_lex_chunk_q},
         {"gemm_strip", sc_gemm_set_strip},                    {"gemm_strip_n", sc_gemm_set_strip_n},
-        {"cls_prune", sc_encoder_set_cls_prune},
+        {"cls_prune", sc_encoder_set_cls_prune},              {"enc_split", sc_encoder_set_split},
     };
     for (const auto& o : options)
         if (!strcmp(name, o.name)) {
diff --git a/semcode_amd/csrc/sc_encoder_diag.cpp b/semcode_amd/csrc/sc_encoder_diag.cpp
--- a/semcode_amd/csrc/sc_encoder_diag.cpp
+++ b/semcode_amd/csrc/sc_encoder_diag.cpp
@@ -249,6 +249,15 @@
     if (M == 0) return sc_gemm_last_strip();
     return sc_gemm_strip_tiles(M, N, K, cus > 0 ? cus : sc_device_cus());
 }
+
+extern "C" int32_t sc_diag_enc_split(int32_t B, int32_t S, int32_t H, int32_t cus, int32_t by_options) {
+    if (cus <= 0) cus = sc_device_cus();
+    if (by_options) return sc_encoder_split_chunks(B, S, H, cus);
+    int B0 = 0;
+    sc_encoder_split_rule(B, S, H, cus, &B0);
+    return B0;
+}
+extern "C" int32_t sc_diag_enc_split_last(void) { return sc_encoder_split_last(); }
 
 extern "C" sc_status sc_diag_gemm_resln(sc_runtime* rt, int32_t flags, const float* A, const float* W, const float* bias, const float* gam, const float* R,
                                         const float* fin, float eps, int32_t M, int32_t N, int32_t K, float* C, float* stats_out) {
diff --git a/semcode_amd/csrc/sc_encoder_forward.cpp b/semcode_amd/csrc/sc_encoder_forward.cpp
--- a/semcode_amd/csrc/sc_encoder_forward.cpp
+++ b/semcode_amd/csrc/sc_encoder_forward.cpp
@@ -14,16 +14,19 @@
 static bool cls_prune_enabled() { return (g_cls_prune < 0 ? CLS_PRUNE_DEFAULT : g_cls_prune) != 0; }
 static bool ffn_blocked_enabled() { static const bool on = sc_env_flag("SC_FFN_BLOCKED", true); return on; }
 
-static void launch_rope(sc_encoder* e, int M, int S, const PackedLayout* pk, hipStream_t s, bool local = false) {
+static void launch_rope(sc_encoder* e, int M, int S, const PackedLayout* pk, hipStream_t s, bool local = false, void* qkv = nullptr) {
     const float *cos_t = local ? e->rope_cos_l : e->rope_cos, *sin_t = local ? e->rope_sin_l : e->rope_sin;
     const int nblocks = e->cfg.arch == 2 ? e->cfg.heads + e->cfg.kv_heads : 2 * e->cfg.heads;
-    if (pk) sc_launch_rope_qk_packed(e->qkv, M, nblocks, pk->pos, e->cfg.max_pos, cos_t, sin_t, s);
-    else sc_launch_rope_qk(e->qkv, M, nblocks, S, cos_t, sin_t, s);
-}
-static void launch_attention(sc_encoder* e, const int32_t* lens_dev, int B, int S, int M, const PackedLayout* pk, hipStream_t s) {
+    if (!qkv) qkv = e->qkv;
+    if (pk) sc_launch_rope_qk_packed(qkv, M, nblocks, pk->pos, e->cfg.max_pos, cos_t, sin_t, s);
+    else sc_launch_rope_qk(qkv, M, nblocks, S, cos_t, sin_t, s);
+}
+static void launch_attention(sc_encoder* e, const int32_t* lens_dev, int B, int S, int M, const PackedLayout* pk, hipStream_t s, const void* qkv = nullptr,
+                             void* ctx = nullptr) {
     const int hd = e->cfg.hidden / e->cfg.heads;
-    if (pk) sc_launch_attention_packed(e->qkv, pk->items, pk->nitems, e->cfg.hidden, e->slopes, e->ctx, s, M, hd);
-    else sc_launch_attention(e->qkv, lens_dev, B, S, e->cfg.hidden, e->slopes, e->ctx, s, M, hd);
+    if (!qkv) qkv = e->qkv, ctx = e->ctx;
+    if (pk) sc_launch_attention_packed(qkv, pk->items, pk->nitems, e->cfg.hidden, e->slopes, ctx, s, M, hd);
+    else sc_launch_attention(qkv, lens_dev, B, S, e->cfg.hidden, e->slopes, ctx, s, M, hd);
 }
 static void launch_norm(const sc_encoder_cfg& c, const void* in, int tokens, const float* g, const float* b, void* out, hipStream_t s) {
     if (c.arch >= 2) sc_launch_rmsnorm(in, tokens, c.hidden, g, c.ln_eps, out, s);
@@ -98,73 +101,142 @@
     else sc_launch_mean_pool(x, lens_dev, B, S, e->cfg.hidden, out_normalize(e, pk), out_dev, s);
 }
 
-static sc_status forward_folded_locked(sc_encoder* e, const int32_t* ids_dev, const int32_t* lens_dev, int32_t B, int32_t S, float* out_dev,
-                                       const PackedLayout* pk) {
+struct FoldView {
+    hipStream_t s;
+    const int32_t *ids, *lens;
+    float* out;
+    int B, tokens, M;
+    void *x, *x1, *y, *qkv, *ctx, *hm, *hg;
+    float *stat_a, *stat_b, *fin_a, *fin_b;
+};
+static FoldView fold_view(const sc_encoder* e, hipStream_t s, const int32_t* ids, const int32_t* lens, float* out, int b0, int B, int S, int tokens, int rows,
+                          int64_t row0) {
+    const sc_encoder_cfg& c = e->cfg;
+    const int64_t H = c.hidden, F = c.ffn, F1 = ffn_gated(c) ? 2 * F : F, slots = H / 256;
+    auto bf = [&](void* p, int64_t width) -> void* { return p ? (char*)p + row0 * width * 2 : nullptr; };
+    FoldView v;
+    v.s = s;
+    v.ids = ids + (int64_t)b0 * S;
+    v.lens = lens + b0;
+    v.out = out + (int64_t)b0 * H;
+    v.B = B, v.tokens = tokens, v.M = rows;
+    v.x = bf(e->x, H), v.x1 = bf(e->x1, H), v.y = bf(e->y, H), v.qkv = bf(e->qkv, 3 * H), v.ctx = bf(e->ctx, H), v.hm = bf(e->hm, F1), v.hg = bf(e->hg, F);
+    v.stat_a = e->stat_a + row0 * slots * 2, v.stat_b = e->stat_b + row0 * slots * 2;
+    v.fin_a = e->fin_a + row0 * 2, v.fin_b = e->fin_b + row0 * 2;
+    return v;
+}
+
+static int g_enc_split = -1, g_enc_split_last = 0;
+void sc_encoder_set_split(int v) { g_enc_split = v < 0 ? -1 : (v ? 1 : 0); }
+int sc_encoder_split_last(void) { return g_enc_split_last; }
+int sc_encoder_split_chunks(int B, int S, int H, int cus) {
+    static const int env = (int)sc_env_i64("SC_ENC_SPLIT", -1);
+    const int mode = g_enc_split >= 0 ? g_enc_split : env;
+    int B0 = 0;
+    if (mode == 0 || !sc_encoder_split_rule(B, S, H, cus, &B0, mode < 0)) return 0;
+    return B0;
+}
+static sc_status split_stream(sc_encoder* e) {
+    if (!e->split_stream) SC_HIP(hipStreamCreateWithFlags(&e->split_stream, hipStreamNonBlocking));
+    if (!e->split_fork) SC_HIP(hipEventCreateWithFlags(&e->split_fork, hipEventDisableTiming));
+    if (!e->split_join) SC_HIP(hipEventCreateWithFlags(&e->split_join, hipEventDisableTiming));
+    return SC_OK;
+}
+
+static sc_status folded_sequence(sc_encoder* e, const FoldView* views, int nv, int32_t S, const PackedLayout* pk) {
     const sc_encoder_cfg& c = e->cfg;
     sc_runtime* rt = e->rt;
-    hipStream_t s = rt->stream;
     const int H = c.hidden, F = c.ffn;
-    const int tokens = pk ? pk->rows : B * S;
-    const int M = (int)ceil256(tokens);
     const int slots = H / 256;
     const bool gated = ffn_gated(c);
     const bool ffn_blocked = !gated && ffn_blocked_enabled();
     const bool rope = c.pos_type == 2, rope_fused = rope && !pk && (g_rope_fused < 0 ? ROPE_FUSED_DEFAULT : g_rope_fused) != 0;
     const bool cls = cls_pooling(e, pk), prune = cls && cls_prune_enabled();
-    if (pair_call(pk))
-        sc_launch_embed_raw_pairs(ids_dev, pk->pos, pk->per_row, tokens, M, H, c.vocab, c.max_pos, c.type_vocab, e->wemb, e->pemb, e->temb, e->x, e->stat_b, slots, s);
-    else if (pk) sc_launch_embed_raw_packed(ids_dev, pk->pos, tokens, M, H, c.vocab, c.max_pos, e->wemb, e->pemb, e->temb, e->x, e->stat_b, slots, s);
-    else sc_launch_embed_raw(ids_dev, tokens, M, S, H, c.vocab, c.max_pos, e->wemb, e->pemb, e->temb, e->x, e->stat_b, slots, s);
+    auto each = [&](auto&& launch) {
+        for (int i = 0; i < nv; ++i) launch(views[i]);
+    };
+    auto timed = [&](int which, auto&& launch) {
+        sc_with_prof_parts(rt, which, nv, [&](int i) { return views[i].s; }, [&](int i) { launch(views[i]); });
+    };
+    each([&](const FoldView& v) {
+        if (pair_call(pk))
+            sc_launch_embed_raw_pairs(v.ids, pk->pos, pk->per_row, v.tokens, v.M, H, c.vocab, c.max_pos, c.type_vocab, e->wemb, e->pemb, e->temb, v.x, v.stat_b, slots, v.s);
+        else if (pk) sc_launch_embed_raw_packed(v.ids, pk->pos, v.tokens, v.M, H, c.vocab, c.max_pos, e->wemb, e->pemb, e->temb, v.x, v.stat_b, slots, v.s);
+        else sc_launch_embed_raw(v.ids, v.tokens, v.M, S, H, c.vocab, c.max_pos, e->wemb, e->pemb, e->temb, v.x, v.stat_b, slots, v.s);
+    });
     for (int l = 0; l < c.layers; ++l) {
         const LayerW& w = e->layers[l];
-        sc_with_prof(rt, SC_PROF_GEMM, [&] {
+        timed(SC_PROF_GEMM, [&](const FoldView& v) {
             if (rope_fused)
-                sc_launch_gemm_bf16_ln(EPI_LNA_BIAS_ROPE, e->x, H, w.wqkv_f, H, w.c2q, nullptr, 0, e->qkv, SC_LDC_BLOCKED64, M, 3 * H, H, s, w.c1q, e->stat_b, e->fin_b,
+                sc_launch_gemm_bf16_ln(EPI_LNA_BIAS_ROPE, v.x, H, w.wqkv_f, H, w.c2q, nullptr, 0, v.qkv, SC_LDC_BLOCKED64, v.M, 3 * H, H, v.s, w.c1q, v.stat_b, v.fin_b,
                                        nullptr, nullptr, c.ln_eps, e->rope_cos, e->rope_sin, S, 2 * H);
             else
-                sc_launch_gemm_bf16_ln(EPI_LNA_BIAS, e->x, H, w.wqkv_f, H, w.c2q, nullptr, 0, e->qkv, SC_LDC_BLOCKED64, M, 3 * H, H, s, w.c1q, e->stat_b, e->fin_b, nullptr,
+                sc_launch_gemm_bf16_ln(EPI_LNA_BIAS, v.x, H, w.wqkv_f, H, w.c2q, nullptr, 0, v.qkv, SC_LDC_BLOCKED64, v.M, 3 * H, H, v.s, w.c1q, v.stat_b, v.fin_b, nullptr,
                                        nullptr, c.ln_eps);
         });
-        if (rope && !rope_fused) launch_rope(e, M, S, pk, s);
+        if (rope && !rope_fused) each([&](const FoldView& v) { launch_rope(e, v.M, S, pk, v.s, false, v.qkv); });
         if (prune && l == c.layers - 1)
-            return cls_last_layer(e, w, lens_dev, B, S, M, pk, w.g_prev, l == 0 ? e->embb : e->layers[l - 1].ln2b, out_dev);
-        sc_with_prof(rt, SC_PROF_ATTN, [&] { launch_attention(e, lens_dev, B, S, M, pk, s); });
-        sc_with_prof(rt, SC_PROF_GEMM, [&] {
-            sc_launch_gemm_bf16_ln(EPI_RESLN_STATS, e->ctx, H, w.wo, H, w.bb_o, e->x, H, e->y, H, M, H, H, s, nullptr, nullptr, e->fin_b, w.g_prev, e->stat_a, c.ln_eps);
-        });
-        const void* ffn_in = e->hm;
-        sc_with_prof(rt, SC_PROF_GEMM, [&] {
+            return cls_last_layer(e, w, views[0].lens, views[0].B, S, views[0].M, pk, w.g_prev, l == 0 ? e->embb : e->layers[l - 1].ln2b, views[0].out);
+        timed(SC_PROF_ATTN, [&](const FoldView& v) { launch_attention(e, v.lens, v.B, S, v.M, pk, v.s, v.qkv, v.ctx); });
+        timed(SC_PROF_GEMM, [&](const FoldView& v) {
+            sc_launch_gemm_bf16_ln(EPI_RESLN_STATS, v.ctx, H, w.wo, H, w.bb_o, v.x, H, v.y, H, v.M, H, H, v.s, nullptr, nullptr, v.fin_b, w.g_prev, v.stat_a, c.ln_eps);
+        });
+        timed(SC_PROF_GEMM, [&](const FoldView& v) {
             if (gated)
-                sc_launch_gemm_bf16_ln(EPI_LNA_BIAS, e->y, H, w.w1_f, H, w.c2f, nullptr, 0, e->hm, 2 * F, M, 2 * F, H, s, w.c1f, e->stat_a, e->fin_a, nullptr, nullptr, c.ln_eps);
+                sc_launch_gemm_bf16_ln(EPI_LNA_BIAS, v.y, H, w.w1_f, H, w.c2f, nullptr, 0, v.hm, 2 * F, v.M, 2 * F, H, v.s, w.c1f, v.stat_a, v.fin_a, nullptr, nullptr, c.ln_eps);
             else
-                sc_launch_gemm_bf16_ln(EPI_LNA_GELU, e->y, H, w.w1_f, H, w.c2f, nullptr, 0, e->hm, ffn_blocked ? SC_LDC_BLOCKED64 : F, M, F, H, s, w.c1f, e->stat_a,
-                                       e->fin_a, nullptr, nullptr, c.ln_eps);
-        });
-        if (gated) {
-            launch_gate(c, e->hm, M, F, e->hg, s);
-            ffn_in = e->hg;
-        }
-        sc_with_prof(rt, SC_PROF_GEMM, [&] {
-            sc_launch_gemm_bf16_ln(EPI_RESLN_STATS, ffn_in, ffn_blocked ? SC_LDC_BLOCKED64 : F, w.w2, F, w.bb_2, e->y, H, e->x, H, M, H, F, s, nullptr,
-                                   nullptr, e->fin_a, w.ln1g, e->stat_b, c.ln_eps);
+                sc_launch_gemm_bf16_ln(EPI_LNA_GELU, v.y, H, w.w1_f, H, w.c2f, nullptr, 0, v.hm, ffn_blocked ? SC_LDC_BLOCKED64 : F, v.M, F, H, v.s, w.c1f, v.stat_a,
+                                       v.fin_a, nullptr, nullptr, c.ln_eps);
+        });
+        if (gated) each([&](const FoldView& v) { launch_gate(c, v.hm, v.M, F, v.hg, v.s); });
+        timed(SC_PROF_GEMM, [&](const FoldView& v) {
+            sc_launch_gemm_bf16_ln(EPI_RESLN_STATS, gated ? v.hg : v.hm, ffn_blocked ? SC_LDC_BLOCKED64 : F, w.w2, F, w.bb_2, v.y, H, v.x, H, v.M, H, F, v.s, nullptr,
+                                   nullptr, v.fin_a, w.ln1g, v.stat_b, c.ln_eps);
         });
     }
     const LayerW& last = e->layers[c.layers - 1];
     if (token_call(pk)) {
-        sc_launch_layernorm(e->x, tokens, H, last.ln2g, last.ln2b, c.ln_eps, e->x1, s);
-        return launch_token_head(e, e->x1, pk, s);
-    }
-    if (cls) {
-        sc_launch_cls_pool(e->x, pk ? pk->starts : nullptr, B, S, H, last.ln2g, last.ln2b, c.ln_eps, out_normalize(e, pk), out_dev, s);
-    } else if (out_normalize(e, pk)) {
-        sc_launch_layernorm(e->x, tokens, H, last.ln2g, last.ln2b, c.ln_eps, e->x1, s);
-        launch_mean_pool(e, e->x1, lens_dev, B, S, pk, out_dev, s);
-    } else if (pk) {
-        sc_launch_mean_pool_ln_packed(e->x, e->stat_b, slots, M, last.ln2g, last.ln2b, c.ln_eps, pk->starts, lens_dev, B, H, out_dev, s);
-    } else {
-        sc_launch_mean_pool_ln(e->x, e->stat_b, slots, M, last.ln2g, last.ln2b, c.ln_eps, lens_dev, B, S, H, out_dev, s);
-    }
-    SC_HIP(hipGetLastError());
+        sc_launch_layernorm(views[0].x, views[0].tokens, H, last.ln2g, last.ln2b, c.ln_eps, views[0].x1, views[0].s);
+        return launch_token_head(e, views[0].x1, pk, views[0].s);
+    }
+    each([&](const FoldView& v) {
+        if (cls) {
+            sc_launch_cls_pool(v.x, pk ? pk->starts : nullptr, v.B, S, H, last.ln2g, last.ln2b, c.ln_eps, out_normalize(e, pk), v.out, v.s);
+        } else if (out_normalize(e, pk)) {
+            sc_launch_layernorm(v.x, v.tokens, H, last.ln2g, last.ln2b, c.ln_eps, v.x1, v.s);
+            launch_mean_pool(e, v.x1, v.lens, v.B, S, pk, v.out, v.s);
+        } else if (pk) {
+            sc_launch_mean_pool_ln_packed(v.x, v.stat_b, slots, v.M, last.ln2g, last.ln2b, c.ln_eps, pk->starts, v.lens, v.B, H, v.out, v.s);
+        } else {
+            sc_launch_mean_pool_ln(v.x, v.stat_b, slots, v.M, last.ln2g, last.ln2b, c.ln_eps, v.lens, v.B, S, H, v.out, v.s);
+        }
+    });
+    SC_HIP(hipGetLastError());
+    return SC_OK;
+}
+
+static sc_status forward_folded_locked(sc_encoder* e, const int32_t* ids_dev, const int32_t* lens_dev, int32_t B, int32_t S, float* out_dev,
+                                       const PackedLayout* pk) {
+    hipStream_t s = e->rt->stream;
+    const int H = e->cfg.hidden;
+    const int tokens = pk ? pk->rows : B * S;
+    const int B0 = !pk && e->pooling == 0 ? sc_encoder_split_chunks(B, S, H, e->rt->cus) : 0;
+    g_enc_split_last = B0 > 0;
+    if (!B0) {
+        const FoldView whole = fold_view(e, s, ids_dev, lens_dev, out_dev, 0, B, S, tokens, (int)ceil256(tokens), 0);
+        return folded_sequence(e, &whole, 1, S, pk);
+    }
+    if (sc_status st = split_stream(e)) return st;
+    SC_HIP(hipEventRecord(e->split_fork, s));
+    SC_HIP(hipStreamWaitEvent(e->split_stream, e->split_fork, 0));
+    const FoldView halves[2] = {fold_view(e, s, ids_dev, lens_dev, out_dev, 0, B0, S, B0 * S, B0 * S, 0),
+                                fold_view(e, e->split_stream, ids_dev, lens_dev, out_dev, B0, B - B0, S, (B - B0) * S, (B - B0) * S, (int64_t)B0 * S)};
+    const sc_status st = folded_sequence(e, halves, 2, S, nullptr);
+    hipError_t he = hipEventRecord(e->split_join, e->split_stream);
+    if (he == hipSuccess) he = hipStreamWaitEvent(s, e->split_join, 0);
+    if (he != hipSuccess) hipStreamSynchronize(e->split_stream);
+    if (st) return st;
+    SC_HIP(he);
     return SC_OK;
 }
 
diff --git a/semcode_amd/csrc/sc_encoder_model.cpp b/semcode_amd/csrc/sc_encoder_model.cpp
--- a/semcode_amd/csrc/sc_encoder_model.cpp
+++ b/semcode_amd/csrc/sc_encoder_model.cpp
@@ -297,6 +297,12 @@
     if (!e) return SC_OK;
     hipSetDevice(e->rt->device);
     hipStreamSynchronize(e->rt->stream);
+    if (e->split_stream) {
+        hipStreamSynchronize(e->split_stream);
+        hipStreamDestroy(e->split_stream);
+    }
+    if (e->split_fork) hipEventDestroy(e->split_fork);
+    if (e->split_join) hipEventDestroy(e->split_join);
     hipFree(e->params);
     hipFree(e->ws);
     hipFree(e->splitk);
diff --git a/semcode_amd/csrc/sc_encoder_plan.cpp b/semcode_amd/csrc/sc_encoder_plan.cpp
--- a/semcode_amd/csrc/sc_encoder_plan.cpp
+++ b/semcode_amd/csrc/sc_encoder_plan.cpp
@@ -1,6 +1,16 @@
 #include "sc_encoder_plan.h"
 
 #include <cstring>
+
+bool sc_encoder_split_rule(int B, int S, int H, int cus, int* B0, bool use_cus) {
+    *B0 = 0;
+    const int64_t b0 = B / 2, b1 = B - b0;
+    if (b0 < 1 || S < 1 || H < 256 || (H % 256)) return false;
+    if ((b0 * S) % 256 || (b1 * S) % 256) return false;
+    if (use_cus && (b0 * S / 256) * (H / 256) < (int64_t)cus) return false;
+    *B0 = (int)b0;
+    return true;
+}
 
 void sc_packed_items(const int32_t* starts, const int32_t* lens, int64_t B, int32_t* items, int nitems[3]) {
     int32_t* w = items;
diff --git a/semcode_amd/csrc/sc_encoder_plan.h b/semcode_amd/csrc/sc_encoder_plan.h
--- a/semcode_amd/csrc/sc_encoder_plan.h
+++ b/semcode_amd/csrc/sc_encoder_plan.h
@@ -9,6 +9,8 @@
 
 static inline int64_t ceil32(int64_t v) { return (v + 31) & ~(int64_t)31; }
 static inline int64_t ceil256(int64_t v) { return (v + 255) & ~(int64_t)255; }
+
+bool sc_encoder_split_rule(int B, int S, int H, int cus, int* B0, bool use_cus = true);
 
 struct PackedCall {
     enum Kind {
diff --git a/semcode_amd/csrc/sc_encoder_state.h b/semcode_amd/csrc/sc_encoder_state.h
--- a/semcode_amd/csrc/sc_encoder_state.h
+++ b/semcode_amd/csrc/sc_encoder_state.h
@@ -73,6 +73,8 @@
     bool foldable = false;
     int path = 0;
     int pooling = 0;
+    hipStream_t split_stream = nullptr;
+    hipEvent_t split_fork = nullptr, split_join = nullptr;
     void* splitk = nullptr;
     static constexpr size_t SPLITK_BYTES = 64u << 20;
     struct PinSlot {
diff --git a/semcode_amd/csrc/sc_internal.h b/semcode_amd/csrc/sc_internal.h
--- a/semcode_amd/csrc/sc_internal.h
+++ b/semcode_amd/csrc/sc_internal.h
@@ -20,6 +20,11 @@
         hipError_t _e = (expr);                                                                       \
         if (_e != hipSuccess) return sc_fail(SC_ERR_HIP, "%s failed: %s", #expr, hipGetErrorString(_e)); \
     } while (0)
+
+struct sc_prof_sample {
+    static constexpr int MAX_PARTS = 2;
+    hipEvent_t a[MAX_PARTS] = {nullptr, nullptr}, b[MAX_PARTS] = {nullptr, nullptr};
+};
 
 struct sc_runtime {
     std::atomic<int> refs{1};
@@ -32,7 +37,7 @@
     int cus = 256;
     int64_t hbm = 0;
     std::mutex mu;
-    std::vector<std::pair<hipEvent_t, hipEvent_t>> prof[SC_PROF_CLASSES];
+    std::vector<sc_prof_sample> prof[SC_PROF_CLASSES];
 };
 
 void sc_runtime_retain(sc_runtime* rt);
@@ -45,6 +50,19 @@
     sc_prof_begin(rt, which, &a, &b);
     launch();
     sc_prof_end(rt, which, a, b);
+}
+void sc_prof_open(sc_runtime* rt, int which, int parts, sc_prof_sample* p);
+void sc_prof_close(sc_runtime* rt, int which, const sc_prof_sample& p);
+template <class S, class F>
+static inline void sc_with_prof_parts(sc_runtime* rt, int which, int parts, S&& stream_of, F&& launch) {
+    sc_prof_sample p;
+    sc_prof_open(rt, which, parts, &p);
+    for (int i = 0; i < parts; ++i) {
+        if (p.a[i]) hipEventRecord(p.a[i], stream_of(i));
+        launch(i);
+        if (p.b[i]) hipEventRecord(p.b[i], stream_of(i));
+    }
+    sc_prof_close(rt, which, p);
 }
 
 struct sc_buf {
@@ -236,3 +254,6 @@
 void sc_set_lex_chunk_q(int v);
 void sc_encoder_set_rope_fused(int v);
 void sc_encoder_set_cls_prune(int v);
+void sc_encoder_set_split(int v);
+int sc_encoder_split_chunks(int B, int S, int H, int cus);
+int sc_encoder_split_last(void);
```

Result: faster. 23240 chunks/s, median of 6 (+2.1%).
